# wildsonbbl/gnnepcsaft

Hardware: AMD Instinct MI355X
Metric: molecular graphs/sec (fwd+bwd) (higher is better)
Workload: dtype f32; 1 GPU; BASELINE configs[1]: PNA hidden=128 L=6 towers=1 pre=2 post=4, 4096 graphs/GPU (81920 atoms, 163840 directed bonds), fwd+loss+bwd incl. CSR packing; graphs_per_gpu=4096, parallelism=dp1, hip_graph=False, launch=auto, grad_allreduce_bytes=0, grad_exchange=none (1 rank)

## Files before the change

gnnepcsaft_amd/_lib.py:

```python
from __future__ import annotations

import ctypes as C
from pathlib import Path
from typing import Dict, Optional

import torch

_LIB_PATH = Path(__file__).resolve().parent / "libgnnepcsaft_hip.so"

ABI_VERSION = 7
GNX_OK, GNX_E_INVALID, GNX_E_HIP, GNX_E_RANGE, GNX_E_WORKSPACE = 0, -1, -2, -3, -4
OPT_GEMM_SPLIT, OPT_WGRAD_WGS, OPT_EMBED_BWD_MFMA, OPT_STD_BWD_CENTERED, OPT_GEMM_PIPE, OPT_WGRAD_PIPE, OPT_GEMM_AS, \
    OPT_GEMM_WS_FAST, OPT_GEMM_TILE_ROWS, OPT_GEMM_MID = range(10)
GEMM_RELU, GEMM_ACCUMULATE, GEMM_B_TRANS, GEMM_SPLIT_ONLY, GEMM_PRESPLIT = 1, 2, 4, 8, 16
GEMM_KERNEL_NAMES = ("none", "k_gemm<vec>", "k_gemm<generic>", "k_gemm_ws", "k_gemm_ws3", "k_gemm_ws3<fast,8>",
                     "k_gemm_ws3<fast,4>", "k_gemm3", "k_gemm3p<96>", "k_gemm3p<128>", "k_gemm_as3", "k_gemm_mid",
                     "k_gemm_small_batched")
WGRAD_KERNEL_NAMES = ("none", "k_gemm_wgrad<true,true>", "k_gemm_wgrad<false,true>", "k_gemm_wgrad3<true>",
                      "k_gemm_wgrad3p_grouped")
POOL_ADD, POOL_MEAN, POOL_MAX = 0, 1, 2
K_NONE, K_PNA_AGG_FWD, K_PNA_AGG_BWD, K_GEMM_WS, K_GEMM_WGRAD, K_GINE_AGG_FWD, K_GINE_AGG_BWD, K_EDGE_COMBINE_FWD, \
    K_EDGE_COMBINE_BWD, K_BN_FWD, K_BN_BWD, K_GEMM_TILED, K_GEMM_SMALL, K_GEMM_WGRAD_BATCHED, K_KEY_SEGMENT_SUM, \
    K_EMBED, K_PNA_EDGE_FWD, K_PNA_EDGE_BWD, K_ATTN_FWD, K_ATTN_BWD, K_PCSAFT_RHO, K_PCSAFT_VP, \
    K_PCSAFT_MIX_STATE, K_PCSAFT_MIX_RHO, K_PCSAFT_MIX_LNPHI_STATE, K_PCSAFT_MIX_LNPHI = range(26)
K_COUNT = 26
KERNEL_GROUPS = {K_PNA_AGG_FWD: "pna_aggregate_fwd", K_PNA_AGG_BWD: "pna_aggregate_bwd", K_GEMM_WS: "gemm_weights_stationary",
                 K_GEMM_WGRAD: "weight_gradient", K_GINE_AGG_FWD: "gine_aggregate_fwd", K_GINE_AGG_BWD: "gine_aggregate_bwd",
                 K_EDGE_COMBINE_FWD: "edge_combine_fwd", K_EDGE_COMBINE_BWD: "edge_combine_bwd", K_BN_FWD: "batchnorm_fwd",
                 K_BN_BWD: "batchnorm_bwd", K_GEMM_TILED: "gemm_tiled", K_GEMM_SMALL: "gemm_small",
                 K_GEMM_WGRAD_BATCHED: "weight_gradient_batched", K_KEY_SEGMENT_SUM: "key_segment_sum", K_EMBED: "embedding",
                 K_PNA_EDGE_FWD: "pna_edge_fused_fwd", K_PNA_EDGE_BWD: "pna_edge_fused_bwd",
                 K_ATTN_FWD: "transformer_attn_fwd", K_ATTN_BWD: "transformer_attn_bwd",
                 K_PCSAFT_RHO: "pcsaft_density", K_PCSAFT_VP: "pcsaft_vapor_pressure",
                 K_PCSAFT_MIX_STATE: "pcsaft_mix_state", K_PCSAFT_MIX_RHO: "pcsaft_mix_density",
                 K_PCSAFT_MIX_LNPHI_STATE: "pcsaft_mix_lnphi_state", K_PCSAFT_MIX_LNPHI: "pcsaft_mix_lnphi"}


class GnxError(RuntimeError):
    def __init__(self, status: int, msg: str):
        super().__init__(f"gnx status {status}: {msg}")
        self.status = status


class GemmSeg(C.Structure):
    _fields_ = [("a", C.c_void_p), ("lda", C.c_int64), ("rowscale", C.c_void_p), ("b", C.c_void_p),
                ("ldb", C.c_int64), ("k", C.c_int32), ("_pad", C.c_int32)]


class GemmPlanInfo(C.Structure):
    _fields_ = [("kernel", C.c_int32), ("tile_rows", C.c_int32), ("grid_x", C.c_uint32), ("grid_y", C.c_uint32),
                ("block", C.c_uint32), ("runs_split", C.c_int32), ("image_bytes", C.c_size_t)]


class WgradGroupedPlanInfo(C.Structure):
    _fields_ = [("kernel", C.c_int32), ("ranges", C.c_int32), ("chunks_per_range", C.c_int32), ("grid_x", C.c_uint32),
                ("grid_y", C.c_uint32), ("grid_z", C.c_uint32), ("block", C.c_uint32)]


class WgradProb(C.Structure):
    _fields_ = [("dC", C.c_void_p), ("lddc", C.c_int64), ("A", C.c_void_p), ("lda", C.c_int64),
                ("rowscale", C.c_void_p), ("dW", C.c_void_p), ("lddw", C.c_int64), ("dbias", C.c_void_p),
                ("M", C.c_int64), ("N", C.c_int32), ("K", C.c_int32)]


_vp, _i32, _i64, _f32, _sz = C.c_void_p, C.c_int32, C.c_int64, C.c_float, C.c_size_t

PNA_MAX_LAYERS, PNA_MAX_TOWERS = 8, 8
PNA_BWD_DEFER_SMALL, PNA_BWD_LAST_OF_PASS = 1, 2


class PnaFwdArgs(C.Structure):
    _fields_ = [("N", _i64), ("E", _i64), ("T", _i32), ("F", _i32), ("pre_layers", _i32), ("post_layers", _i32),
                ("D", _i32), ("merged", _i32),
                ("rowptr", _vp), ("src", _vp), ("dst", _vp), ("code", _vp), ("dperm", _vp), ("tiles", _vp), ("ntiles", _vp),
                ("max_tiles", _i64), ("x", _vp), ("Te", _vp), ("weff", _vp * PNA_MAX_TOWERS), ("Wm", _vp), ("bm", _vp),
                ("params", C.POINTER(_vp)), ("P", _vp), ("Q", _vp), ("A", _vp), ("hs", _vp * PNA_MAX_LAYERS),
                ("zs", _vp * PNA_MAX_LAYERS), ("ws", _vp), ("ws_bytes", _sz), ("out", _vp), ("etile_info", _vp),
                ("etile_w", _i32), ("tile_rows", _i32)]


class PnaBwdArgs(C.Structure):
    _fields_ = [("N", _i64), ("E", _i64), ("T", _i32), ("F", _i32), ("pre_layers", _i32), ("post_layers", _i32),
                ("R", _i32), ("D", _i32), ("avg_deg_log", _f32), ("merged", _i32), ("acc_first", _i32),
                ("use_side_streams", _i32), ("n_h", _i32), ("n_z", _i32),
                ("rowptr", _vp), ("colptr", _vp), ("cpos", _vp), ("code", _vp), ("code_pos", _vp), ("dperm", _vp),
                ("tiles", _vp), ("ntiles", _vp), ("chunks", _vp), ("nchunks", _vp),
                ("max_tiles", _i64), ("max_chunks", _i64),
                ("x", _vp), ("BE", _vp), ("EE", _vp), ("A", _vp),
                ("hs", _vp * PNA_MAX_LAYERS), ("zs", _vp * PNA_MAX_LAYERS), ("weff", _vp * PNA_MAX_TOWERS), ("Wm", _vp),
                ("params", C.POINTER(_vp)), ("grads", C.POINTER(_vp)), ("dout", _vp),
                ("gbuf", _vp * PNA_MAX_LAYERS), ("dA", _vp), ("gebuf", _vp * PNA_MAX_LAYERS), ("dP", _vp), ("dQ", _vp),
                ("dTe", _vp), ("dEE", _vp), ("dWm", _vp), ("dbm", _vp), ("dWeff", _vp), ("ws", _vp), ("ws_bytes", _sz),
                ("acc_buf", _vp), ("dx", _vp), ("flags", _i32), ("etile_w", _i32), ("etile_info", _vp)]


PACK_MAX_AVG = 4
PACK_CLASSES, PACK_CODE_INDEX, PACK_EDGE_TILES, PACK_TILED_SCAN = 1, 2, 4, 256


class PackBatchArgs(C.Structure):
    _fields_ = [("edge_index", _vp), ("edge_attr", _vp), ("batch", _vp), ("N", _i64), ("E", _i64), ("B", _i64),
                ("K", _i32), ("bond_dims", _i32 * 16), ("max_degree", _i32), ("R", _i32), ("n_avg", _i32),
                ("avg_deg_log", _f32 * PACK_MAX_AVG), ("tile_rows", _i32 * 3), ("edge_tile_w", _i32),
                ("parts", C.c_uint32), ("_pad", _i32),
                ("rowptr", _vp), ("perm", _vp), ("src", _vp), ("dst", _vp), ("colptr", _vp), ("cpos", _vp),
                ("code", _vp), ("graph_ptr", _vp), ("amp", _vp * PACK_MAX_AVG), ("att", _vp * PACK_MAX_AVG),
                ("dperm", _vp), ("cls_ptr", _vp), ("tiles", _vp * 3), ("ntiles", _vp * 3), ("code_pos", _vp),
                ("code_ptr", _vp), ("edge_tiles", _vp), ("ws", _vp), ("ws_bytes", _sz)]


class GemmImage(C.Structure):
    _fields_ = [("image_bytes", C.c_uint64), ("classes", _i32), ("Npad", _i32), ("Kpad", _i32), ("koff", _i32 * 5),
                ("frag", _i32), ("bt", _i32)]


class PnaLayerImages(C.Structure):
    _fields_ = [("post0", _vp * PNA_MAX_TOWERS), ("dA", _vp * PNA_MAX_TOWERS), ("dx", _vp * PNA_MAX_TOWERS),
                ("post0_rec", GemmImage * PNA_MAX_TOWERS), ("dA_rec", GemmImage * PNA_MAX_TOWERS),
                ("dx_rec", GemmImage * PNA_MAX_TOWERS)]


class PnaFinishArgs(C.Structure):
    _fields_ = [("L", _i32), ("T", _i32), ("F", _i32), ("pre_layers", _i32), ("post_layers", _i32), ("R", _i32), ("D", _i32),
                ("merged", _i32), ("use_side_streams", _i32), ("_pad", _i32),
                ("BE", _vp), ("acc_buf", _vp), ("ones", _vp), ("avg_deg_log", C.POINTER(_f32)),
                ("params", C.POINTER(_vp)), ("grads", C.POINTER(_vp)), ("EE", C.POINTER(_vp)), ("dTe", C.POINTER(_vp)),
                ("dEE", C.POINTER(_vp)), ("dWm", C.POINTER(_vp)), ("dbm", C.POINTER(_vp)), ("dWeff", C.POINTER(_vp))]


class SmallProb(C.Structure):
    _fields_ = [("A", _vp), ("lda", _i64), ("B", _vp), ("ldb", _i64), ("bias", _vp), ("C", _vp), ("ldc", _i64),
                ("M", _i32), ("N", _i32), ("K", _i32), ("flags", _i32)]


SB_A_TRANS, SB_B_TRANS, SB_ACCUMULATE, SB_ATOMIC, SB_RELU = 1, 2, 4, 8, 16

SIGNATURES = {
    "gnx_create": (_i32, [C.POINTER(_vp), _i32]),
    "gnx_destroy": (_i32, [_vp]),
    "gnx_set_stream": (_i32, [_vp, _vp]),
    "gnx_last_error": (C.c_char_p, []),
    "gnx_abi_version": (_i32, []),
    "gnx_set_option": (_i32, [_vp, _i32, _i32]),
    "gnx_get_option": (_i32, [_vp, _i32, C.POINTER(_i32)]),
    "gnx_prof_begin": (_i32, [_vp, C.c_uint32]),
    "gnx_prof_read": (_i32, [_vp, _i32, C.POINTER(_i64), C.POINTER(C.c_double), C.POINTER(C.c_double),
                             C.POINTER(C.c_double), C.POINTER(C.c_double)]),
    "gnx_prof_end": (_i32, [_vp]),
    "gnx_pack_csr_workspace_bytes": (_sz, [_i64, _i64]),
    "gnx_pack_csr": (_i32, [_vp, _vp, _i64, _i64, _vp, _vp, _vp, _vp, _vp, _vp, _vp, _sz]),
    "gnx_feature_code": (_i32, [_vp, _vp, _i64, _i32, C.POINTER(_i32), _vp, _vp, _vp, _sz]),
    "gnx_graph_ptr": (_i32, [_vp, _vp, _i64, _i64, _vp, _vp, _sz]),
    "gnx_degree_scalers": (_i32, [_vp, _vp, _i64, _f32, _vp, _vp]),
    "gnx_embed_sum_fwd": (_i32, [_vp, _vp, _i64, _i32, C.POINTER(_i32), _vp, _i32, _vp]),
    "gnx_table_scatter_workspace_bytes": (_sz, [_i64, _i32, _i32]),
    "gnx_embed_sum_bwd": (_i32, [_vp, _vp, _i64, _i32, C.POINTER(_i32), _i32, _vp, _i32, _vp, _vp, _sz]),
    "gnx_check_range": (_i32, [_vp]),
    "gnx_collate_ptr": (_i32, [_vp, _vp, _vp, _i64, _vp, _i64, _vp, _vp]),
    "gnx_collate_gather": (_i32, [_vp, _vp, _vp, _i64, _vp, _vp, _vp, _i64, _vp, _i64, _vp, _vp, _i64, _i64, _vp, _vp,
                                  _vp, _vp]),
    "gnx_collate_rows": (_i32, [_vp, _vp, _i64, _vp, _i64, _i32, _i32, _vp]),
    "gnx_gemm_workspace_bytes": (_sz, [_vp, _i32, C.POINTER(GemmSeg), C.POINTER(_i64), _i32, _i64, _i32, _vp, _i32,
                                       _i32]),
    "gnx_gemm": (_i32, [_vp, _i32, C.POINTER(GemmSeg), _i64, _i32, _vp, _vp, _i64, _vp, _i64, _i32, _vp, _sz]),
    "gnx_gemm_wgrad": (_i32, [_vp, _vp, _i64, _vp, _i64, _vp, _i64, _i32, _i32, _vp, _i64, _vp]),
    "gnx_gemm_wgrad_batched": (_i32, [_vp, _i32, C.POINTER(WgradProb)]),
    "gnx_degree_max": (_i32, [_vp, _vp, _i64, C.POINTER(_i32)]),
    "gnx_degree_classes_workspace_bytes": (_sz, [_i64, _i32]),
    "gnx_degree_classes": (_i32, [_vp, _vp, _i64, _i32, _vp, _vp, _vp, _sz]),
    "gnx_class_tiles": (_i32, [_vp, _vp, _i32, _i32, _vp, _vp]),
    "gnx_gemm_grouped": (_i32, [_vp, _i32, C.POINTER(GemmSeg), C.POINTER(_i64), _i32, _i64, _i32, _vp, _vp, _i64, _vp,
                                _i64, _i32, _vp, _vp, _vp, _i64, _vp, _sz]),
    "gnx_gemm_tile_rows": (_i32, [_vp, _i64, _i32]),
    "gnx_gemm_grouped_rows": (_i32, [_vp, _i32, C.POINTER(GemmSeg), C.POINTER(_i64), _i32, _i64, _i32, _vp, _vp, _i64, _vp,
                                     _i64, _i32, _vp, _vp, _vp, _i64, _vp, _sz, _i32]),
    "gnx_gemm_plan": (_i32, [_vp, _i32, C.POINTER(GemmSeg), C.POINTER(_i64), _i32, _i64, _i32, _vp, _vp, _i64, _vp, _i64, _i32,
                             _vp, _vp, _vp, _i64, _vp, _sz, _i32, C.POINTER(GemmPlanInfo)]),
    "gnx_gemm_wgrad_grouped": (_i32, [_vp, _vp, _i64, _vp, _i64, _i64, _i32, _i32, _vp, _i64, _i64, _vp, _vp, _vp,
                                      _i64]),
    "gnx_gemm_wgrad_grouped_plan": (_i32, [_vp, _i64, _i64, _vp, _vp, _i64, _i32, _i32, _i64,
                                           C.POINTER(WgradGroupedPlanInfo)]),
    "gnx_pna_weff": (_i32, [_vp, _vp, _i64, _i32, _i32, _f32, _vp]),
    "gnx_pna_weff_bwd": (_i32, [_vp, _vp, _i32, _i32, _f32, _vp, _i64]),
    "gnx_group_by_small_key": (_i32, [_vp, _vp, _i64, _i32, _vp, _vp, _vp, _sz]),
    "gnx_key_segment_sum": (_i32, [_vp, _vp, _vp, _vp, _i64, _i32, _vp]),
    "gnx_edge_combine_fwd": (_i32, [_vp, _vp, _vp, _vp, _vp, _vp, _vp, _i64, _i32, _i32, _vp]),
    "gnx_edge_combine_bwd": (_i32, [_vp, _vp, _vp, _vp, _vp, _vp, _i64, _i64, _i32, _i32, _vp, _vp, _vp, _vp, _sz]),
    "gnx_pna_aggregate_fwd": (_i32, [_vp, _vp, _vp, _i64, _i64, _i32, _i32, _vp]),
    "gnx_pna_aggregate_bwd": (_i32, [_vp, _vp, _vp, _vp, _vp, _i64, _i64, _i32, _i32, _vp]),
    "gnx_edge_tiles_count": (_i32, [_i64, _i32]),
    "gnx_edge_tiles": (_i32, [_vp, _vp, _i64, _i64, _i32, _vp]),
    "gnx_pack_batch_workspace_bytes": (_sz, [_i64, _i64, _i32, _i32]),
    "gnx_pack_batch": (_i32, [_vp, C.POINTER(PackBatchArgs)]),
    "gnx_pack_batch_scan_chunk": (_i64, []),
    "gnx_pack_batch_scan_bound": (_i64, []),
    "gnx_pna_edge_fwd": (_i32, [_vp, _vp, _vp, _vp, _vp, _vp, _vp, _vp, _vp, _i32, _i64, _i64, _i32, _i32, C.POINTER(_vp),
                                C.POINTER(_vp), _vp, _vp, _vp]),
    "gnx_pna_edge_bwd": (_i32, [_vp, _vp, _vp, _vp, _vp, _vp, _i32, _i64, _i64, _i32, _i32, _i32, C.POINTER(_vp), _vp, _vp,
                                _vp]),
    "gnx_gine_aggregate_fwd": (_i32, [_vp, _vp, _vp, _vp, _vp, _vp, _i64, _i64, _i32, _f32, _vp]),
    "gnx_gine_aggregate_bwd": (_i32, [_vp, _vp, _vp, _vp, _vp, _vp, _vp, _vp, _vp, _vp, _i64, _i64, _i32, _i32, _f32,
                                      _vp, _vp]),
    "gnx_gine_dle": (_i32, [_vp, _vp, _vp, _vp, _vp, _vp, _vp, _vp, _i64, _i32, _i32, _vp]),
    "gnx_transformer_attn_fwd": (_i32, [_vp, _vp, _vp, _vp, _vp, _vp, _i64, _i64, _i32, _i32, _f32, C.c_uint64,
                                        C.c_uint64, _vp, _vp, _vp]),
    "gnx_transformer_attn_bwd": (_i32, [_vp, _vp, _vp, _vp, _vp, _vp, _vp, _vp, _vp, _vp, _vp, _vp, _i64, _i64, _i32,
                                        _i32, _i32, _f32, C.c_uint64, C.c_uint64, _vp, _vp, _vp]),
    "gnx_transformer_attn_dle": (_i32, [_vp, _vp, _vp, _vp, _vp, _vp, _vp, _i64, _i32, _i32, _i32, _vp]),
    "gnx_pcsaft_density": (_i32, [_vp, _vp, _i64, _vp, _vp, _vp, _i64, _vp, _vp]),
    "gnx_pcsaft_vapor_pressure": (_i32, [_vp, _vp, _i64, _vp, _vp, _i64, _vp, _vp, _vp, _vp]),
    "gnx_pcsaft_mix_state": (_i32, [_vp, _vp, _i64, _vp, _vp, _vp, _i64, _i32, _vp, _vp, _vp, _vp, _i64, _vp, _vp, _vp,
                                    _vp]),
    "gnx_pcsaft_mix_density": (_i32, [_vp, _vp, _i64, _vp, _vp, _vp, _i64, _i32, _vp, _vp, _vp, _vp, _i64, _vp, _vp]),
    "gnx_pcsaft_mix_lnphi_state": (_i32, [_vp, _vp, _i64, _vp, _vp, _vp, _i64, _i32, _vp, _vp, _vp, _vp, _i64, _vp, _vp,
                                          _vp]),
    "gnx_pcsaft_mix_lnphi": (_i32, [_vp, _vp, _i64, _vp, _vp, _vp, _i64, _i32, _vp, _vp, _vp, _vp, _i64, _vp, _vp, _vp,
                                    _vp]),
    "gnx_pcsaft_mix_bubble": (_i32, [_vp, _vp, _i64, _vp, _vp, _vp, _i64, _i32, _vp, _vp, _vp, _i64, _vp, _vp, _vp, _vp,
                                     _vp]),
    "gnx_pcsaft_mix_dew": (_i32, [_vp, _vp, _i64, _vp, _vp, _vp, _i64, _i32, _vp, _vp, _vp, _i64, _vp, _vp, _vp, _vp,
                                  _vp]),
    "gnx_pcsaft_mix_bubble_t": (_i32, [_vp, _vp, _i64, _vp, _vp, _vp, _i64, _i32, _vp, _vp, _vp, _vp, _i64, _vp, _vp, _vp,
                                       _vp, _vp]),
    "gnx_pcsaft_mix_dew_t": (_i32, [_vp, _vp, _i64, _vp, _vp, _vp, _i64, _i32, _vp, _vp, _vp, _vp, _i64, _vp, _vp, _vp,
                                    _vp, _vp]),
    "gnx_pcsaft_mix_flash": (_i32, [_vp, _vp, _i64, _vp, _vp, _vp, _i64, _i32, _vp, _vp, _vp, _vp, _i64, _vp, _vp, _vp, _vp,
                                    _vp, _vp]),
    "gnx_pcsaft_mix_stability": (_i32, [_vp, _vp, _i64, _vp, _vp, _vp, _i64, _i32, _vp, _vp, _vp, _vp, _vp, _i64, _vp, _vp,
                                        _vp, _vp, _vp]),
    "gnx_pcsaft_mix_lle": (_i32, [_vp, _vp, _i64, _vp, _vp, _vp, _i64, _i32, _vp, _vp, _vp, _vp, _vp, _i64, _vp, _vp, _vp,
                                  _vp, _vp, _vp]),
    "gnx_segment_pool_fwd": (_i32, [_vp, _vp, _vp, _i64, _i32, _i32, _vp]),
    "gnx_segment_pool_bwd": (_i32, [_vp, _vp, _vp, _vp, _vp, _i64, _i32, _i32, _vp]),
    "gnx_batchnorm_workspace_bytes": (_sz, [_i64, _i32]),
    "gnx_batchnorm_fwd": (_i32, [_vp, _vp, _i64, _i32, _vp, _vp, _vp, _vp, _vp, _f32, _f32, _i32, _i32, _vp, _vp, _vp,
                                 _vp, _sz]),
    "gnx_batchnorm_bwd": (_i32, [_vp, _vp, _vp, _vp, _i64, _i32, _vp, _vp, _vp, _i32, _vp, _vp, _vp, _vp, _sz]),
    "gnx_batchnorm_bwd_x": (_i32, [_vp, _vp, _vp, _i64, _i32, _vp, _vp, _vp, _vp, _i32, _vp, _vp, _vp, _vp, _sz]),
    "gnx_dropout": (_i32, [_vp, _vp, _i64, _f32, C.c_uint64, C.c_uint64, _vp]),
    "gnx_huber_ape": (_i32, [_vp, _vp, _vp, _i64, _f32, _vp, _vp]),
    "gnx_adamw_amsgrad": (_i32, [_vp, _vp, _vp, _vp, _vp, _vp, _i64, _f32, _f32, _f32, _f32, _f32, _i64]),
    "gnx_sgd": (_i32, [_vp, _vp, _vp, _i64, _f32]),
    "gnx_pna_weight_only": (_i32, [_vp, _vp, _i32, _i32, _i32, _i32, _i32, _i32, _f32, C.POINTER(_vp), _i32, _vp, _vp,
                                   C.POINTER(_vp), _vp, _vp]),
    "gnx_pna_conv_fwd": (_i32, [_vp, C.POINTER(PnaFwdArgs)]),
    "gnx_pna_split_all_bytes": (_sz, [_vp, _i32, _i32, _i32, _i32, _i32, _i32, _i64, _i32]),
    "gnx_pna_split_all": (_i32, [_vp, _i32, _i32, _i32, _i32, _i32, _i32, _i64, _i32, C.POINTER(_vp), C.POINTER(_vp), _vp, _sz,
                                 C.POINTER(PnaLayerImages)]),
    "gnx_gemm_split_counts": (_i32, [_vp, C.POINTER(_i64), C.POINTER(_i64)]),
    "gnx_pna_conv_fwd_images": (_i32, [_vp, C.POINTER(PnaFwdArgs), C.POINTER(PnaLayerImages)]),
    "gnx_pna_conv_bwd_images": (_i32, [_vp, C.POINTER(PnaBwdArgs), C.POINTER(PnaLayerImages)]),
    "gnx_pna_weight_only_all": (_i32, [_vp, _i32, _vp, _i32, _i32, _i32, _i32, _i32, _i32, C.POINTER(_f32), C.POINTER(_vp),
                                       _i32, C.POINTER(_vp), C.POINTER(_vp), C.POINTER(_vp), C.POINTER(_vp), C.POINTER(_vp)]),
    "gnx_pna_stack_finish": (_i32, [_vp, C.POINTER(PnaFinishArgs)]),
    "gnx_gemm_small_batched": (_i32, [_vp, _i32, C.POINTER(SmallProb)]),
    "gnx_pna_weff_batched": (_i32, [_vp, _i32, C.POINTER(_vp), _i64, _i32, _i32, C.POINTER(_f32), C.POINTER(_vp)]),
    "gnx_pna_weff_bwd_batched": (_i32, [_vp, _i32, C.POINTER(_vp), _i32, _i32, C.POINTER(_f32), C.POINTER(_vp), _i64]),
    "gnx_pna_conv_bwd_workspace_bytes": (_sz, [_i32, _i32, _i32]),
    "gnx_pna_conv_bwd": (_i32, [_vp, C.POINTER(PnaBwdArgs)]),
    "gnx_fill": (_i32, [_vp, _vp, _i64, _f32]),
    "gnx_scale": (_i32, [_vp, _vp, _i64, _f32]),
    "gnx_axpy": (_i32, [_vp, _vp, _vp, _i64, _f32]),
    "gnx_side_stream": (_i32, [_vp, C.POINTER(_vp)]),
    "gnx_side_begin": (_i32, [_vp]),
    "gnx_side_end": (_i32, [_vp]),
    "gnx_side_join": (_i32, [_vp]),
    "gnx_side_stream_n": (_i32, [_vp, _i32, C.POINTER(_vp)]),
    "gnx_side_begin_n": (_i32, [_vp, _i32]),
    "gnx_side_join_n": (_i32, [_vp, _i32]),
    "gnx_clip_rows": (_i32, [_vp, _vp, _i64, _i32, _vp, _vp, _vp]),
}

_lib: Optional[C.CDLL] = None
_handles: Dict[int, int] = {}


def lib_path() -> Path:
    return _LIB_PATH


def load() -> C.CDLL:
    global _lib
    if _lib is not None:
        return _lib
    if not _LIB_PATH.exists():
        raise ImportError(f"{_LIB_PATH} is missing: build it with `python -m gnnepcsaft_amd.build` "
                          "(hipcc --offload-arch=gfx950). There is no CPU fallback.")
    lib = C.CDLL(str(_LIB_PATH))
    for name, (res, args) in SIGNATURES.items():
        fn = getattr(lib, name)
        fn.restype = res
        fn.argtypes = args
    if lib.gnx_abi_version() != ABI_VERSION:
        raise ImportError(f"ABI version mismatch: library {lib.gnx_abi_version()} != binding {ABI_VERSION}")
    _lib = lib
    return lib


def last_error() -> str:
    return load().gnx_last_error().decode(errors="replace")


def check(status: int) -> None:
    if status != GNX_OK:
        raise GnxError(status, last_error())


_bound_stream: dict = {}
try:
    _raw_stream = torch._C._cuda_getCurrentRawStream
except AttributeError:
    def _raw_stream(idx: int) -> int:
        return torch.cuda.current_stream(idx).cuda_stream


def handle(device: torch.device) -> int:
    if device.type != "cuda":
        raise GnxError(GNX_E_INVALID, f"gnnepcsaft_amd kernels need a HIP device tensor, got {device}; there is no CPU "
                                      "fallback")
    idx = device.index if device.index is not None else torch.cuda.current_device()
    lib = load()
    h = _handles.get(idx)
    if h is None:
        out = _vp()
        check(lib.gnx_create(C.byref(out), idx))
        h = out.value
        _handles[idx] = h
    stream = _raw_stream(idx)
    if _bound_stream.get(idx) != stream:
        check(lib.gnx_set_stream(h, stream))
        _bound_stream[idx] = stream
    return h
```

gnnepcsaft_amd/csrc/gnx_aggregate.hip:

```cpp
#include "gnx_common.hpp"

#include <cmath>
#include <cstdlib>

int32_t gnx_code_scatter_add(gnx_handle* h, const int32_t* code, int64_t E, int R, const float* g, int H,
                             float* dtable, void* ws, size_t ws_bytes);

template <int VEC>
struct vec_t;
template <>
struct vec_t<4> {
  typedef f32x4 type;
};
template <>
struct vec_t<1> {
  typedef float type;
};

template <int VEC>
__device__ __forceinline__ void vload(float (&r)[VEC], const float* p) {
  if constexpr (VEC == 4) {
    f32x4 v = *reinterpret_cast<const f32x4*>(p);
    r[0] = v.x;
    r[1] = v.y;
    r[2] = v.z;
    r[3] = v.w;
  } else {
    r[0] = p[0];
  }
}
template <int VEC>
__device__ __forceinline__ void vstore(float* p, const float (&r)[VEC]) {
  if constexpr (VEC == 4) {
    f32x4 v = {r[0], r[1], r[2], r[3]};
    *reinterpret_cast<f32x4*>(p) = v;
  } else {
    p[0] = r[0];
  }
}

__device__ __forceinline__ float relu_keep_nan(float r) { return (r < 0.f) ? 0.f : r; }
__device__ __forceinline__ float max_keep_nan(float s, float a) { return (a > s || a != a) ? a : s; }

#define STD_VAR_MIN 1e-5f
#define STD_MASK_AT 0.0031622776601683794f

template <int VEC>
__global__ void __launch_bounds__(256) k_pna_agg_fwd(const float* __restrict__ m, const int* __restrict__ rowptr,
                                                     int64_t N, int T, int F, float* __restrict__ A) {
  const int H = T * F;
  const int G = H / VEC;
  int64_t t = (int64_t)blockIdx.x * blockDim.x + threadIdx.x;
  if (t >= N * G) return;
  int64_t n = t / G;
  int c = (int)(t % G) * VEC;
  int p0 = rowptr[n], p1 = rowptr[n + 1];
  float s[VEC], s2[VEC], mn[VEC], mx[VEC];
#pragma unroll
  for (int v = 0; v < VEC; ++v) {
    s[v] = 0.f;
    s2[v] = 0.f;
    mn[v] = INFINITY;
    mx[v] = -INFINITY;
  }
  const float* mp = m + (int64_t)p0 * H + c;
  int p = p0;
  for (; p + 1 < p1; p += 2, mp += 2 * (int64_t)H) {
    float a[VEC], b[VEC];
    vload<VEC>(a, mp);
    vload<VEC>(b, mp + H);
#pragma unroll
    for (int v = 0; v < VEC; ++v) {
      s[v] = __fadd_rn(__fadd_rn(s[v], a[v]), b[v]);
      s2[v] = __fadd_rn(__fadd_rn(s2[v], __fmul_rn(a[v], a[v])), __fmul_rn(b[v], b[v]));
      mn[v] = fminf(mn[v], fminf(a[v], b[v]));
      mx[v] = fmaxf(mx[v], fmaxf(a[v], b[v]));
    }
  }
  if (p < p1) {
    float a[VEC];
    vload<VEC>(a, mp);
#pragma unroll
    for (int v = 0; v < VEC; ++v) {
      s[v] = __fadd_rn(s[v], a[v]);
      s2[v] = __fadd_rn(s2[v], __fmul_rn(a[v], a[v]));
      mn[v] = fminf(mn[v], a[v]);
      mx[v] = fmaxf(mx[v], a[v]);
    }
  }
  const int d = p1 - p0;
  const float cnt = (float)(d > 0 ? d : 1);
  float mean[VEC], sd[VEC];
#pragma unroll
  for (int v = 0; v < VEC; ++v) {
    mean[v] = __fdiv_rn(s[v], cnt);
    float mean2 = __fdiv_rn(s2[v], cnt);
    float var = __fsub_rn(mean2, __fmul_rn(mean[v], mean[v]));
    float o = __fsqrt_rn(fmaxf(var, STD_VAR_MIN));
    sd[v] = (o <= STD_MASK_AT) ? 0.f : o;
    if (d == 0) {
      mn[v] = 0.f;
      mx[v] = 0.f;
    }
  }
  int tw = c / F, f = c % F;
  float* o = A + (n * T + tw) * (int64_t)(4 * F) + f;
  vstore<VEC>(o, mean);
  vstore<VEC>(o + F, mn);
  vstore<VEC>(o + 2 * F, mx);
  vstore<VEC>(o + 3 * F, sd);
}

extern "C" int32_t gnx_pna_aggregate_fwd(gnx_handle* h, const float* m, const int32_t* rowptr, int64_t N, int64_t E,
                                         int32_t T, int32_t F, float* A) {
  GNX_CHECK_ARG(h && rowptr && T > 0 && F > 0 && N >= 0 && E >= 0, "gnx_pna_aggregate_fwd: bad argument");
  GNX_CHECK_ARG(N == 0 || A, "gnx_pna_aggregate_fwd: A is NULL");
  if (N == 0) return GNX_OK;
  gnx_prof_scope prof(h, GNX_K_PNA_AGG_FWD, 4.0 * E * T * F + 4.0 * E + 16.0 * N * T * F, 0.0, 0.0, true);
  if (F % 4 == 0) {
    int64_t th = N * (T * F / 4);
    GNX_LAUNCH_TIMED(prof, k_pna_agg_fwd<4>, dim3((unsigned)gnx_cdiv(th, 256)), dim3(256), 0, h->stream, m, rowptr, N,
                     (int)T, (int)F, A);
  } else {
    int64_t th = N * (T * F);
    GNX_LAUNCH_TIMED(prof, k_pna_agg_fwd<1>, dim3((unsigned)gnx_cdiv(th, 256)), dim3(256), 0, h->stream, m, rowptr, N,
                     (int)T, (int)F, A);
  }
  GNX_LAUNCH_CHECK();
  return GNX_OK;
}

template <int VEC>
__global__ void __launch_bounds__(256) k_pna_agg_bwd_rc(const float* __restrict__ dA, const float* __restrict__ m,
                                                        const int* __restrict__ rowptr, int64_t N, int T, int F,
                                                        float* __restrict__ dm, int centered) {
  const int H = T * F;
  const int G = H / VEC;
  int64_t t = (int64_t)blockIdx.x * blockDim.x + threadIdx.x;
  if (t >= N * G) return;
  int64_t n = t / G;
  int c = (int)(t % G) * VEC;
  int p0 = rowptr[n], p1 = rowptr[n + 1];
  if (p1 <= p0) return;
  int tw = c / F, f = c % F;
  int64_t ao = (n * T + tw) * (int64_t)(4 * F) + f;
  float gmean[VEC], gmn[VEC], gmx[VEC], gsd[VEC];
  vload<VEC>(gmean, dA + ao);
  vload<VEC>(gmn, dA + ao + F);
  vload<VEC>(gmx, dA + ao + 2 * F);
  vload<VEC>(gsd, dA + ao + 3 * F);
  float s[VEC], s2[VEC], mn[VEC], mx[VEC];
#pragma unroll
  for (int v = 0; v < VEC; ++v) {
    s[v] = 0.f;
    s2[v] = 0.f;
    mn[v] = INFINITY;
    mx[v] = -INFINITY;
  }
  if (p1 - p0 <= 4) {
    const int deg = p1 - p0;
    float a[4][VEC];
#pragma unroll
    for (int e = 0; e < 4; ++e) vload<VEC>(a[e], m + (int64_t)(p0 + (e < deg ? e : 0)) * H + c);
#pragma unroll
    for (int e = 0; e < 4; ++e)
      if (e < deg) {
#pragma unroll
        for (int v = 0; v < VEC; ++v) {
          s[v] = __fadd_rn(s[v], a[e][v]);
          s2[v] = __fadd_rn(s2[v], __fmul_rn(a[e][v], a[e][v]));
          mn[v] = fminf(mn[v], a[e][v]);
          mx[v] = fmaxf(mx[v], a[e][v]);
        }
      }
    const float cnt = (float)deg;
    float mean[VEC], sd[VEC], nmn[VEC], nmx[VEC], c2[VEC];
#pragma unroll
    for (int v = 0; v < VEC; ++v) {
      c2[v] = 0.f;
      mean[v] = __fdiv_rn(s[v], cnt);
      float mean2 = __fdiv_rn(s2[v], cnt);
      float var = __fsub_rn(mean2, __fmul_rn(mean[v], mean[v]));
      float o = __fsqrt_rn(fmaxf(var, STD_VAR_MIN));
      sd[v] = (o <= STD_MASK_AT) ? 0.f : o;
      nmn[v] = (mn[v] == 0.f) ? 1.f : 0.f;
      nmx[v] = (mx[v] == 0.f) ? 1.f : 0.f;
    }
#pragma unroll
    for (int e = 0; e < 4; ++e)
      if (e < deg) {
#pragma unroll
        for (int v = 0; v < VEC; ++v) {
          nmn[v] += (a[e][v] == mn[v]) ? 1.f : 0.f;
          nmx[v] += (a[e][v] == mx[v]) ? 1.f : 0.f;
          const float dv = a[e][v] - mean[v];
          c2[v] = fmaf(dv, dv, c2[v]);
        }
      }
    float k_mean[VEC], k_mn[VEC], k_mx[VEC], k_sd[VEC];
#pragma unroll
    for (int v = 0; v < VEC; ++v) {
      k_mean[v] = gmean[v] / cnt;
      k_mn[v] = gmn[v] / nmn[v];
      k_mx[v] = gmx[v] / nmx[v];
      const float sdiv = (centered && c2[v] > 0.f) ? sqrtf(c2[v] / cnt) : sd[v];
      k_sd[v] = (sd[v] > 0.f) ? gsd[v] / (cnt * sdiv) : 0.f;
    }
    float* dp = dm + (int64_t)p0 * H + c;
#pragma unroll
    for (int e = 0; e < 4; ++e)
      if (e < deg) {
        float o[VEC];
#pragma unroll
        for (int v = 0; v < VEC; ++v) {
          float r = k_mean[v] + k_sd[v] * (a[e][v] - mean[v]);
          r += (a[e][v] == mn[v]) ? k_mn[v] : 0.f;
          r += (a[e][v] == mx[v]) ? k_mx[v] : 0.f;
          o[v] = r;
        }
        vstore<VEC>(dp + (int64_t)e * H, o);
      }
    return;
  }
  const float* mp = m + (int64_t)p0 * H + c;
  for (int p = p0; p < p1; ++p, mp += H) {
    float a[VEC];
    vload<VEC>(a, mp);
#pragma unroll
    for (int v = 0; v < VEC; ++v) {
      s[v] = __fadd_rn(s[v], a[v]);
      s2[v] = __fadd_rn(s2[v], __fmul_rn(a[v], a[v]));
      mn[v] = fminf(mn[v], a[v]);
      mx[v] = fmaxf(mx[v], a[v]);
    }
  }
  const float cnt = (float)(p1 - p0);
  float mean[VEC], sd[VEC], nmn[VEC], nmx[VEC], c2[VEC];
#pragma unroll
  for (int v = 0; v < VEC; ++v) {
    c2[v] = 0.f;
    mean[v] = __fdiv_rn(s[v], cnt);
    float mean2 = __fdiv_rn(s2[v], cnt);
    float var = __fsub_rn(mean2, __fmul_rn(mean[v], mean[v]));
    float o = __fsqrt_rn(fmaxf(var, STD_VAR_MIN));
    sd[v] = (o <= STD_MASK_AT) ? 0.f : o;
    nmn[v] = (mn[v] == 0.f) ? 1.f : 0.f;
    nmx[v] = (mx[v] == 0.f) ? 1.f : 0.f;
  }
  mp = m + (int64_t)p0 * H + c;
  for (int p = p0; p < p1; ++p, mp += H) {
    float a[VEC];
    vload<VEC>(a, mp);
#pragma unroll
    for (int v = 0; v < VEC; ++v) {
      nmn[v] += (a[v] == mn[v]) ? 1.f : 0.f;
      nmx[v] += (a[v] == mx[v]) ? 1.f : 0.f;
      const float dv = a[v] - mean[v];
      c2[v] = fmaf(dv, dv, c2[v]);
    }
  }
  float k_mean[VEC], k_mn[VEC], k_mx[VEC], k_sd[VEC];
#pragma unroll
  for (int v = 0; v < VEC; ++v) {
    k_mean[v] = gmean[v] / cnt;
    k_mn[v] = gmn[v] / nmn[v];
    k_mx[v] = gmx[v] / nmx[v];
    const float sdiv = (centered && c2[v] > 0.f) ? sqrtf(c2[v] / cnt) : sd[v];
    k_sd[v] = (sd[v] > 0.f) ? gsd[v] / (cnt * sdiv) : 0.f;
  }
  mp = m + (int64_t)p0 * H + c;
  float* dp = dm + (int64_t)p0 * H + c;
  for (int p = p0; p < p1; ++p, mp += H, dp += H) {
    float a[VEC], o[VEC];
    vload<VEC>(a, mp);
#pragma unroll
    for (int v = 0; v < VEC; ++v) {
      float r = k_mean[v] + k_sd[v] * (a[v] - mean[v]);
      r += (a[v] == mn[v]) ? k_mn[v] : 0.f;
      r += (a[v] == mx[v]) ? k_mx[v] : 0.f;
      o[v] = r;
    }
    vstore<VEC>(dp, o);
  }
}

extern "C" int32_t gnx_pna_aggregate_bwd(gnx_handle* h, const float* dA, const float* m, const float* A,
                                         const int32_t* rowptr, int64_t N, int64_t E, int32_t T, int32_t F, float* dm) {
  GNX_CHECK_ARG(h && rowptr && T > 0 && F > 0 && N >= 0 && E >= 0, "gnx_pna_aggregate_bwd: bad argument");
  GNX_CHECK_ARG(N == 0 || (dA && A), "gnx_pna_aggregate_bwd: NULL argument");
  if (N == 0) return GNX_OK;
  gnx_prof_scope prof(h, GNX_K_PNA_AGG_BWD, 16.0 * N * T * F + 8.0 * E * T * F + 4.0 * E, 0.0, 0.0, true);
  if (F % 4 == 0)
    GNX_LAUNCH_TIMED(prof, k_pna_agg_bwd_rc<4>, dim3((unsigned)gnx_cdiv(N * (T * F / 4), 256)), dim3(256), 0, h->stream, dA, m,
                     rowptr, N, (int)T, (int)F, dm, h->opt[GNX_OPT_STD_BWD_CENTERED]);
  else
    GNX_LAUNCH_TIMED(prof, k_pna_agg_bwd_rc<1>, dim3((unsigned)gnx_cdiv(N * (int64_t)(T * F), 256)), dim3(256), 0, h->stream, dA,
                     m, rowptr, N, (int)T, (int)F, dm, h->opt[GNX_OPT_STD_BWD_CENTERED]);
  GNX_LAUNCH_CHECK();
  return GNX_OK;
}

template <int VEC>
__global__ void __launch_bounds__(256) k_edge_combine_fwd(const float* __restrict__ P, const float* __restrict__ Q,
                                                          const float* __restrict__ Te, const int* __restrict__ src,
                                                          const int* __restrict__ dst, const int* __restrict__ code,
                                                          int64_t E, int H, int relu, float* __restrict__ h1) {
  const int G = H / VEC;
  int64_t t = (int64_t)blockIdx.x * blockDim.x + threadIdx.x;
  if (t >= E * G) return;
  int64_t p = t / G;
  int c = (int)(t % G) * VEC;
  float a[VEC], b[VEC], e[VEC], o[VEC];
  vload<VEC>(a, P + (int64_t)dst[p] * H + c);
  vload<VEC>(b, Q + (int64_t)src[p] * H + c);
  vload<VEC>(e, Te + (int64_t)code[p] * H + c);
#pragma unroll
  for (int v = 0; v < VEC; ++v) {
    float r = (a[v] + b[v]) + e[v];
    o[v] = relu ? relu_keep_nan(r) : r;
  }
  vstore<VEC>(h1 + p * H + c, o);
}

extern "C" int32_t gnx_edge_combine_fwd(gnx_handle* h, const float* P, const float* Q, const float* Te,
                                        const int32_t* src, const int32_t* dst, const int32_t* code, int64_t E,
                                        int32_t H, int32_t relu, float* h1) {
  GNX_CHECK_ARG(h && H > 0 && E >= 0, "gnx_edge_combine_fwd: bad argument");
  if (E == 0) return GNX_OK;
  GNX_CHECK_ARG(P && Q && Te && src && dst && code && h1, "gnx_edge_combine_fwd: NULL argument");
  gnx_prof_scope prof(h, GNX_K_EDGE_COMBINE_FWD, 12.0 * E * H + 12.0 * E);
  if (H % 4 == 0)
    hipLaunchKernelGGL(k_edge_combine_fwd<4>, dim3((unsigned)gnx_cdiv(E * (H / 4), 256)), dim3(256), 0, h->stream, P, Q,
                       Te, src, dst, code, E, (int)H, (int)relu, h1);
  else
    hipLaunchKernelGGL(k_edge_combine_fwd<1>, dim3((unsigned)gnx_cdiv(E * H, 256)), dim3(256), 0, h->stream, P, Q, Te,
                       src, dst, code, E, (int)H, (int)relu, h1);
  GNX_LAUNCH_CHECK();
  return GNX_OK;
}

template <int VEC>
__global__ void __launch_bounds__(256) k_edge_combine_bwd(const float* __restrict__ g, const int* __restrict__ rowptr,
                                                          const int* __restrict__ colptr, const int* __restrict__ cpos,
                                                          int64_t N, int H, float* __restrict__ dP,
                                                          float* __restrict__ dQ) {
  const int G = H / VEC;
  int64_t t = (int64_t)blockIdx.x * blockDim.x + threadIdx.x;
  if (t >= N * G) return;
  int64_t n = t / G;
  int c = (int)(t % G) * VEC;
  float s[VEC], q[VEC];
#pragma unroll
  for (int v = 0; v < VEC; ++v) {
    s[v] = 0.f;
    q[v] = 0.f;
  }
  if (dP != nullptr) {
    int p0 = rowptr[n], p1 = rowptr[n + 1];
    for (int p = p0; p < p1; ++p) {
      float a[VEC];
      vload<VEC>(a, g + (int64_t)p * H + c);
#pragma unroll
      for (int v = 0; v < VEC; ++v) s[v] += a[v];
    }
  }
  int c0 = colptr[n], c1 = colptr[n + 1];
  for (int k = c0; k < c1; ++k) {
    float a[VEC];
    vload<VEC>(a, g + (int64_t)cpos[k] * H + c);
#pragma unroll
    for (int v = 0; v < VEC; ++v) q[v] += a[v];
  }
  if (dP != nullptr) vstore<VEC>(dP + n * H + c, s);
  vstore<VEC>(dQ + n * H + c, q);
}

extern "C" int32_t gnx_edge_combine_bwd(gnx_handle* h, const float* g, const int32_t* rowptr, const int32_t* colptr,
                                        const int32_t* cpos, const int32_t* code, int64_t N, int64_t E, int32_t H,
                                        int32_t R, float* dP, float* dQ, float* dTe, void* ws, size_t ws_bytes) {
  GNX_CHECK_ARG(h && H > 0 && N >= 0 && E >= 0, "gnx_edge_combine_bwd: bad argument");
  if (N == 0) return GNX_OK;
  GNX_CHECK_ARG(rowptr && colptr && dQ && (E == 0 || (g && cpos)), "gnx_edge_combine_bwd: NULL argument");
  gnx_prof_scope prof(h, GNX_K_EDGE_COMBINE_BWD, 4.0 * E * H + (dP ? 8.0 : 4.0) * N * H + 4.0 * E + 8.0 * N);
  if (H % 4 == 0)
    hipLaunchKernelGGL(k_edge_combine_bwd<4>, dim3((unsigned)gnx_cdiv(N * (H / 4), 256)), dim3(256), 0, h->stream, g,
                       rowptr, colptr, cpos, N, (int)H, dP, dQ);
  else
    hipLaunchKernelGGL(k_edge_combine_bwd<1>, dim3((unsigned)gnx_cdiv(N * H, 256)), dim3(256), 0, h->stream, g, rowptr,
                       colptr, cpos, N, (int)H, dP, dQ);
  GNX_LAUNCH_CHECK();
  if (dTe != nullptr && E > 0) {
    GNX_CHECK_ARG(code && R > 0, "gnx_edge_combine_bwd: code/R missing for dTe");
    return gnx_code_scatter_add(h, code, E, R, g, H, dTe, ws, ws_bytes);
  }
  return GNX_OK;
}


#define SEG_CHUNK 128

template <int VEC>
__global__ void __launch_bounds__(256) k_key_segment_sum(const float* __restrict__ g, const int* __restrict__ pos,
                                                         const int* __restrict__ key, int64_t E, int H,
                                                         float* __restrict__ dtable) {
  const int G = H / VEC;
  const int lanes = 256 / G > 0 ? 256 / G : 1;
  const int cg = threadIdx.x % G, rl = threadIdx.x / G;
  if (rl >= lanes) return;
  const int c = cg * VEC;
  const int64_t i0 = (int64_t)blockIdx.x * SEG_CHUNK;
  int64_t i1 = i0 + SEG_CHUNK;
  if (i1 > E) i1 = E;
  const int64_t per = (i1 - i0 + lanes - 1) / lanes;
  int64_t a = i0 + (int64_t)rl * per, b = a + per;
  if (b > i1) b = i1;
  if (a >= b) return;
  float acc[VEC];
#pragma unroll
  for (int v = 0; v < VEC; ++v) acc[v] = 0.f;
  int cur = key[pos[a]];
  constexpr int UN = 4;
  for (int64_t i = a; i < b; i += UN) {
    int p[UN], k[UN];
    float r[UN][VEC];
#pragma unroll
    for (int j = 0; j < UN; ++j) p[j] = pos[(i + j < b) ? i + j : b - 1];
#pragma unroll
    for (int j = 0; j < UN; ++j) k[j] = key[p[j]];
#pragma unroll
    for (int j = 0; j < UN; ++j) vload<VEC>(r[j], g + (int64_t)p[j] * H + c);
#pragma unroll
    for (int j = 0; j < UN; ++j) {
      if (i + j < b) {
        if (k[j] != cur) {
#pragma unroll
          for (int v = 0; v < VEC; ++v) atomicAdd(&dtable[(int64_t)cur * H + c + v], acc[v]);
// ... 366 lines not shown
```

gnnepcsaft_amd/csrc/gnx_api.hip:

```cpp
#include "gnx_common.hpp"

#include <cstdlib>
#include <cstring>

static thread_local char g_err[512] = "";

void gnx_set_error(const char* fmt, ...) {
  va_list ap;
  va_start(ap, fmt);
  vsnprintf(g_err, sizeof(g_err), fmt, ap);
  va_end(ap);
}

extern "C" const char* gnx_last_error(void) { return g_err; }
extern "C" int32_t gnx_abi_version(void) { return GNX_ABI_VERSION; }

extern "C" int32_t gnx_create(gnx_handle** out, int32_t device) {
  GNX_CHECK_ARG(out != nullptr, "gnx_create: out is NULL");
  int count = 0;
  GNX_HIP(hipGetDeviceCount(&count));
  GNX_CHECK_ARG(device >= 0 && device < count, "gnx_create: device %d not in [0,%d)", device, count);
  GNX_HIP(hipSetDevice(device));
  gnx_handle* h = new gnx_handle();
  h->device = device;
  {
    hipDeviceProp_t prop;
    if (hipGetDeviceProperties(&prop, device) == hipSuccess) h->num_cus = prop.multiProcessorCount;
  }
  hipError_t e = hipMalloc(&h->d_flag, 256);
  if (e == hipSuccess) e = hipMalloc(&h->d_scratch, 4096);
  if (e == hipSuccess) e = hipMemset(h->d_flag, 0, 256);
  if (e == hipSuccess) e = hipMalloc(&h->d_zero, 256);
  if (e == hipSuccess) e = hipMemset(h->d_zero, 0, 256);
  if (e != hipSuccess) {
    gnx_set_error("gnx_create: %s", hipGetErrorString(e));
    delete h;
    return GNX_E_HIP;
  }
  static const struct {
    int id;
    const char* env;
    int def;
  } opts[] = {{GNX_OPT_GEMM_SPLIT, "GNX_GEMM_SPLIT", 1},         {GNX_OPT_WGRAD_WGS, "GNX_WGRAD_WGS", 0},
              {GNX_OPT_EMBED_BWD_MFMA, "GNX_EMBED_BWD_MFMA", 1}, {GNX_OPT_STD_BWD_CENTERED, "GNX_STD_BWD_CENTERED", 1},
              {GNX_OPT_GEMM_PIPE, "GNX_GEMM_PIPE", 1},           {GNX_OPT_WGRAD_PIPE, "GNX_WGRAD_PIPE", 1},
              {GNX_OPT_GEMM_AS, "GNX_GEMM_AS", 1},               {GNX_OPT_GEMM_WS_FAST, "GNX_GEMM_WS_FAST", 2},
              {GNX_OPT_GEMM_TILE_ROWS, "GNX_GEMM_TILE_ROWS", 0}, {GNX_OPT_GEMM_MID, "GNX_GEMM_MID", 1}};
  for (const auto& o : opts) {
    const char* e = getenv(o.env);
    h->opt[o.id] = e ? atoi(e) : o.def;
  }
  *out = h;
  return GNX_OK;
}

extern "C" int32_t gnx_set_option(gnx_handle* h, int32_t opt, int32_t value) {
  GNX_CHECK_ARG(h != nullptr && opt >= 0 && opt < GNX_OPT_COUNT, "gnx_set_option: bad handle or option %d", opt);
  h->opt[opt] = value;
  return GNX_OK;
}

extern "C" int32_t gnx_get_option(gnx_handle* h, int32_t opt, int32_t* value) {
  GNX_CHECK_ARG(h != nullptr && value != nullptr && opt >= 0 && opt < GNX_OPT_COUNT, "gnx_get_option: bad argument");
  *value = h->opt[opt];
  return GNX_OK;
}

extern "C" int32_t gnx_destroy(gnx_handle* h) {
  if (!h) return GNX_OK;
  for (hipEvent_t e : h->ev) (void)hipEventDestroy(e);
  (void)hipFree(h->d_flag);
  (void)hipFree(h->d_scratch);
  (void)hipFree(h->d_zero);
  for (int i = 0; i < gnx_handle::kSideStreams; ++i) {
    if (h->side_fork[i]) (void)hipEventDestroy(h->side_fork[i]);
    if (h->side_done[i]) (void)hipEventDestroy(h->side_done[i]);
    if (h->side[i]) (void)hipStreamDestroy(h->side[i]);
  }
  delete h;
  return GNX_OK;
}

extern "C" int32_t gnx_set_stream(gnx_handle* h, void* hip_stream) {
  GNX_CHECK_ARG(h != nullptr, "gnx_set_stream: handle is NULL");
  GNX_CHECK_ARG(!h->on_side, "gnx_set_stream: between gnx_side_begin and gnx_side_end");
  h->stream = reinterpret_cast<hipStream_t>(hip_stream);
  return GNX_OK;
}

static int32_t side_ensure(gnx_handle* h, int which) {
  GNX_CHECK_ARG(h != nullptr, "gnx_side_*: handle is NULL");
  GNX_CHECK_ARG(which >= 0 && which < gnx_handle::kSideStreams, "gnx_side_*: stream %d not in [0,%d)", which,
                gnx_handle::kSideStreams);
  if (h->side[which] == nullptr) {
    GNX_HIP(hipSetDevice(h->device));
    GNX_HIP(hipStreamCreateWithFlags(&h->side[which], hipStreamNonBlocking));
    GNX_HIP(hipEventCreateWithFlags(&h->side_fork[which], hipEventDisableTiming));
    GNX_HIP(hipEventCreateWithFlags(&h->side_done[which], hipEventDisableTiming));
  }
  return GNX_OK;
}

extern "C" int32_t gnx_side_begin_n(gnx_handle* h, int32_t which) {
  const int32_t st = side_ensure(h, which);
  if (st != GNX_OK) return st;
  GNX_CHECK_ARG(!h->on_side, "gnx_side_begin: already on a side stream");
  GNX_HIP(hipEventRecord(h->side_fork[which], h->stream));
  GNX_HIP(hipStreamWaitEvent(h->side[which], h->side_fork[which], 0));
  h->main_saved = h->stream;
  h->stream = h->side[which];
  h->on_side = true;
  return GNX_OK;
}

extern "C" int32_t gnx_side_begin(gnx_handle* h) { return gnx_side_begin_n(h, 0); }

extern "C" int32_t gnx_side_stream_n(gnx_handle* h, int32_t which, void** hip_stream) {
  GNX_CHECK_ARG(hip_stream != nullptr, "gnx_side_stream: NULL argument");
  const int32_t st = side_ensure(h, which);
  if (st != GNX_OK) return st;
  *hip_stream = reinterpret_cast<void*>(h->side[which]);
  return GNX_OK;
}

extern "C" int32_t gnx_side_stream(gnx_handle* h, void** hip_stream) { return gnx_side_stream_n(h, 0, hip_stream); }

extern "C" int32_t gnx_side_end(gnx_handle* h) {
  GNX_CHECK_ARG(h != nullptr, "gnx_side_end: handle is NULL");
  if (h->on_side) {
    h->stream = h->main_saved;
    h->on_side = false;
  }
  return GNX_OK;
}

extern "C" int32_t gnx_side_join_n(gnx_handle* h, int32_t which) {
  GNX_CHECK_ARG(h != nullptr, "gnx_side_join: handle is NULL");
  GNX_CHECK_ARG(which >= 0 && which < gnx_handle::kSideStreams, "gnx_side_join: bad stream %d", which);
  GNX_CHECK_ARG(!h->on_side, "gnx_side_join: between gnx_side_begin and gnx_side_end");
  if (h->side[which] == nullptr) return GNX_OK;
  GNX_HIP(hipEventRecord(h->side_done[which], h->side[which]));
  GNX_HIP(hipStreamWaitEvent(h->stream, h->side_done[which], 0));
  return GNX_OK;
}

extern "C" int32_t gnx_side_join(gnx_handle* h) { return gnx_side_join_n(h, 0); }

int32_t gnx_read_flag(gnx_handle* h, int* value) {
  int v = 0;
  GNX_HIP(hipMemcpyAsync(&v, h->d_flag, sizeof(int), hipMemcpyDeviceToHost, h->stream));
  GNX_HIP(hipStreamSynchronize(h->stream));
  if (v != 0) GNX_HIP(hipMemsetAsync(h->d_flag, 0, sizeof(int), h->stream));
  *value = v;
  return GNX_OK;
}

extern "C" int32_t gnx_check_range(gnx_handle* h) {
  GNX_CHECK_ARG(h != nullptr, "gnx_check_range: handle is NULL");
  int v = 0;
  int32_t st = gnx_read_flag(h, &v);
  if (st != GNX_OK) return st;
  if (v != 0) {
    gnx_set_error("integer input out of range:%s%s%s%s%s%s%s", (v & 32) ? " an in-degree (or bond code) exceeds the caller's hint;" : "",
                  (v & 1) ? " edge_index holds a node id outside [0,N);" : "",
                  (v & 2) ? " edge/node feature outside its vocabulary;" : "",
                  (v & 4) ? " batch holds a graph id outside [0,B);" : "", (v & 8) ? " batch is not sorted;" : "",
                  (v & 16) ? " embedding index outside its table;" : "",
                  (v & 128) ? " batch index outside the device dataset;" : "");
    return GNX_E_RANGE;
  }
  return GNX_OK;
}

extern "C" int32_t gnx_prof_begin(gnx_handle* h, uint32_t kernel_mask) {
  GNX_CHECK_ARG(h != nullptr, "gnx_prof_begin: handle is NULL");
  GNX_CHECK_ARG((kernel_mask >> GNX_K_COUNT) == 0, "gnx_prof_begin: bad kernel mask 0x%x", kernel_mask);
  h->prof_mask = kernel_mask & ~1u;
  h->ev_used = 0;
  return GNX_OK;
}

extern "C" int32_t gnx_prof_read(gnx_handle* h, int32_t kid, int64_t* launches, double* total_ms, double* alg_bytes,
                                 double* alg_flops, double* mfma_bf16_flops) {
  GNX_CHECK_ARG(h != nullptr && launches != nullptr && total_ms != nullptr, "gnx_prof_read: NULL argument");
  GNX_CHECK_ARG(kid > 0 && kid < GNX_K_COUNT, "gnx_prof_read: bad kernel id %d", kid);
  GNX_HIP(hipStreamSynchronize(h->stream));
  double tot = 0.0, w[3] = {0.0, 0.0, 0.0};
  int64_t n = 0;
  for (size_t i = 0; i + 1 < h->ev_used; i += 2) {
    if (h->ev_kid[i / 2] != kid) continue;
    float ms = 0.f;
    GNX_HIP(hipEventElapsedTime(&ms, h->ev[i], h->ev[i + 1]));
    tot += ms;
    for (int q = 0; q < 3; ++q) w[q] += h->ev_work[3 * (i / 2) + q];
    ++n;
  }
  *launches = n;
  *total_ms = tot;
  if (alg_bytes) *alg_bytes = w[0];
  if (alg_flops) *alg_flops = w[1];
// ... 106 lines not shown
```

gnnepcsaft_amd/csrc/gnx_gemm.hip:

```cpp
#include "gnx_gemm_plan.hpp"
#include "gnx_split.hpp"

#include <cstdlib>
#include <type_traits>

#define MAX_SEGS 4

enum { EPI_PLAIN = 0, EPI_ACCUM = 1, EPI_MASK = 2 };

template <typename F>
static auto epi_dispatch(bool bt, int epi, F&& f) {
  auto with_bt = [&](auto BT) {
    if (epi == EPI_MASK) return f(BT, std::integral_constant<int, EPI_MASK>{});
    if (epi == EPI_ACCUM) return f(BT, std::integral_constant<int, EPI_ACCUM>{});
    return f(BT, std::integral_constant<int, EPI_PLAIN>{});
  };
  return bt ? with_bt(std::true_type{}) : with_bt(std::false_type{});
}

struct seg_dev {
  const float* a;
  const float* rs;
  const float* b;
  int64_t lda;
  int64_t ldb;
  int64_t cls_stride;
  int k;
  int vec_a;
  int vec_b;
};

struct gemm_args {
  seg_dev seg[MAX_SEGS];
  int nseg;
  int64_t M;
  int N;
  const float* bias;
  const float* mask;
  int64_t ldmask;
  float* C;
  int64_t ldc;
  int relu;
  const int* row_index;
  const int* tile_info;
  const int* ntiles;
  int ny;
  const __bf16* bsplit;
  int Npad, Kpad;
  int koff[MAX_SEGS];
  int steps;
};

template <int EPI>
__device__ __forceinline__ void epilogue_tile(const f32x16& acc, const int (&rows)[16], int gc, int N, float bv,
                                              int relu, const float* __restrict__ mask, int64_t ldmask,
                                              float* __restrict__ C, int64_t ldc) {
  const bool col_ok = gc < N;
  const int gcc = col_ok ? gc : 0;
  float extra[16];
  if constexpr (EPI != EPI_PLAIN) {
#pragma unroll
    for (int r = 0; r < 16; ++r) {
      const int64_t gr = rows[r] < 0 ? 0 : rows[r];
      extra[r] = (EPI == EPI_MASK) ? mask[gr * ldmask + gcc] : C[gr * ldc + gcc];
    }
  }
#pragma unroll
  for (int r = 0; r < 16; ++r) {
    float v = acc[r] + bv;
    if constexpr (EPI == EPI_ACCUM) v += extra[r];
    v = relu ? fmaxf(v, 0.f) : v;
    if constexpr (EPI == EPI_MASK) v = (extra[r] > 0.f) ? v : 0.f;
    if (col_ok && rows[r] >= 0) C[(int64_t)rows[r] * ldc + gc] = v;
  }
}

template <bool B_TRANS, int EPI, bool VEC>
__global__ void __launch_bounds__(256, 2) k_gemm(gemm_args g) {
  __shared__ __attribute__((aligned(16))) float As[BM * LDK];
  __shared__ __attribute__((aligned(16))) float Bs[B_TRANS ? BN * LDK : BK * LDN];
  __shared__ int rid[BM];

  const int tid = threadIdx.x;
  const int lane = tid & 63;
  const int wave = tid >> 6;
  const int wm = wave >> 1, wn = wave & 1;
  const int li = lane & 31, lh = lane >> 5;
  const int n0 = blockIdx.y * BN;
  int cls = 0;
  if (g.tile_info != nullptr) {
    if ((int)blockIdx.x >= g.ntiles[0]) return;
    const int p0 = g.tile_info[3 * blockIdx.x], pr = g.tile_info[3 * blockIdx.x + 1];
    cls = g.tile_info[3 * blockIdx.x + 2];
    if (tid < BM) rid[tid] = (tid < pr) ? g.row_index[p0 + tid] : -1;
  } else {
    const int64_t m0 = (int64_t)blockIdx.x * BM;
    if (tid < BM) rid[tid] = (m0 + tid < g.M) ? (int)(m0 + tid) : -1;
  }
  __syncthreads();

  f32x16 acc[2][2];
#pragma unroll
  for (int i = 0; i < 2; ++i)
#pragma unroll
    for (int j = 0; j < 2; ++j)
#pragma unroll
      for (int r = 0; r < 16; ++r) acc[i][j][r] = 0.f;

  f32x4 ra[4], rb[4];

  const int lr = tid >> 3;
  const int lk = (tid & 7) * 4;
  const int br = tid >> 5;
  const int bc = (tid & 31) * 4;
  int grow[4];
#pragma unroll
  for (int i = 0; i < 4; ++i) grow[i] = rid[lr + 32 * i];
  int okmask = 0;
  float rsv[4] = {1.f, 1.f, 1.f, 1.f};

  auto load_tile = [&](const seg_dev& s, int k0) {
    const float* sb = s.b + (int64_t)cls * s.cls_stride;
    if constexpr (VEC) {
      const int kcol = k0 + lk;
      const bool k_ok = kcol < s.k;
      const int kc = k_ok ? kcol : 0;
      okmask = 0;
#pragma unroll
      for (int i = 0; i < 4; ++i) {
        const int64_t row = grow[i] >= 0 ? grow[i] : 0;
        ra[i] = *reinterpret_cast<const f32x4*>(s.a + row * s.lda + kc);
        rsv[i] = *(s.rs != nullptr ? s.rs + row : &c_one);
        okmask |= (k_ok && grow[i] >= 0) ? (1 << i) : 0;
      }
      if (B_TRANS) {
#pragma unroll
        for (int i = 0; i < 4; ++i) {
          const int gn = n0 + lr + 32 * i;
          rb[i] = *reinterpret_cast<const f32x4*>(sb + (int64_t)(gn < g.N ? gn : 0) * s.ldb + kc);
          okmask |= (k_ok && gn < g.N) ? (16 << i) : 0;
        }
      } else {
        const int nn = n0 + bc;
        const bool n_ok = nn < g.N;
        const int nc = n_ok ? nn : 0;
#pragma unroll
        for (int i = 0; i < 4; ++i) {
          const int kr = k0 + br + 8 * i;
          rb[i] = *reinterpret_cast<const f32x4*>(sb + (int64_t)(kr < s.k ? kr : 0) * s.ldb + nc);
          okmask |= (n_ok && kr < s.k) ? (16 << i) : 0;
        }
      }
      return;
// ... 1189 lines not shown
  const bool k_ok = k4 < s.k;
  int grow[8];
#pragma unroll
  for (int q = 0; q < 8; ++q) {
    const int r = lr + 8 * q;
    const int idx = p0 + (r < pr ? r : pr - 1);
    grow[q] = grouped ? g.row_index[idx] : idx;
  }
  int my_row = 0;
  if (tid < AS_BM) {
    const int idx = p0 + (tid < pr ? tid : pr - 1);
    my_row = grouped ? g.row_index[idx] : idx;
  }
  f32x4 ra[8];
#pragma unroll
  for (int q = 0; q < 8; ++q) ra[q] = *reinterpret_cast<const f32x4*>(s.a + (int64_t)grow[q] * s.lda + (k_ok ? k4 : 0));

  const int total_kt = NT * 4;
  const __bf16* const bbase = g.bsplit + ((int64_t)cls * NT * 4 * 3) * (BN * BK) + (wave * 64 + lane) * 8;
  bf16x8 bq[2][2][3];
  auto load_b = [&](int slot, int sl, int j) {
    const __bf16* p = bbase + (int64_t)(j < total_kt ? j : total_kt - 1) * (3 * BN * BK);
#pragma unroll
    for (int pc = 0; pc < 3; ++pc) bq[slot][sl][pc] = *reinterpret_cast<const bf16x8*>(p + ((sl * 3 + pc) * 4 * 64) * 8);
  };
  load_b(0, 0, 0);
  load_b(0, 1, 0);
  AS_AT(0);

  typedef __attribute__((ext_vector_type(2))) float f32x2;
  if (tid < AS_BM) {
    roff[tid] = (unsigned)my_row * (unsigned)g.ldc;
    moff[tid] = (unsigned)my_row * (unsigned)g.ldmask;
  }
#pragma unroll
  for (int q = 0; q < 8; q += 2) {
    float xa[8];
#pragma unroll
    for (int j = 0; j < 4; ++j) {
      xa[j] = k_ok ? ra[q][j] : 0.f;
      xa[4 + j] = k_ok ? ra[q + 1][j] : 0.f;
    }
    bf16x8 pc[3];
    split3(xa, pc[0], pc[1], pc[2]);
#pragma unroll
    for (int p = 0; p < 3; ++p) {
      const f32x4 w = *reinterpret_cast<const f32x4*>(&pc[p]);
      unsigned char* qa = A3 + p * AS_PIECE + (lr + 8 * q) * AS_LDA + k4 * 2;
      *reinterpret_cast<f32x2*>(qa) = f32x2{w.x, w.y};
      *reinterpret_cast<f32x2*>(qa + 8 * AS_LDA) = f32x2{w.z, w.w};
    }
  }
  load_b(1, 0, 1);
  load_b(1, 1, 1);
  AS_AT(1);
  __syncthreads();
  AS_AT(2);

  int afrag = li * AS_LDA + 16 * lh;
  bf16x8 af[2][2][3];
  auto read_a = [&](int slot, int off, int ks) {
    const unsigned char* base = A3 + off;
#pragma unroll
    for (int mi = 0; mi < 2; ++mi)
#pragma unroll
      for (int p = 0; p < 3; ++p)
        af[slot][mi][p] = *reinterpret_cast<const bf16x8*>(base + p * AS_PIECE + mi * 32 * AS_LDA + ks * 32);
  };
  read_a(0, afrag, 0);

  const int qj = li & 3;
  const unsigned lc = (unsigned)(wave * 32 + (li >> 2) * 4);
  unsigned ro[2][4], mo[2][4];
#pragma unroll
  for (int mi = 0; mi < 2; ++mi)
#pragma unroll
    for (int gq = 0; gq < 4; ++gq) {
      ro[mi][gq] = roff[mi * 32 + 8 * gq + 4 * lh + qj] + lc;
      mo[mi][gq] = moff[mi * 32 + 8 * gq + 4 * lh + qj] + lc;
    }
  const float* const bias_p = g.bias != nullptr ? g.bias : c_zero4;
  const int bias_on = g.bias != nullptr ? 1 : 0;
  auto bias_at = [&](int nt_) { return *reinterpret_cast<const f32x4*>(bias_p + (bias_on ? nt_ * BN + (int)lc : 0)); };
  f32x4 bv = bias_at(0);
  const float floor_v = g.relu ? 0.f : -__builtin_inff();
  asm volatile("" ::"v"(bv));
  auto quad_swap = [&](float& x, float& y, auto CTRL, bool hi) {
    const float send = hi ? x : y;
    const float got = __builtin_bit_cast(float, __builtin_amdgcn_mov_dpp(__builtin_bit_cast(int, send), decltype(CTRL)::value, 0xf, 0xf, true));
    x = hi ? got : x;
    y = hi ? y : got;
  };
  using XOR1 = std::integral_constant<int, 0xB1>;
  using XOR2 = std::integral_constant<int, 0x4E>;

  for (int nt = 0; nt < NT; ++nt) {
    asm volatile("" : "+v"(afrag));
    f32x16 acc[2];
#pragma unroll
    for (int mi = 0; mi < 2; ++mi)
#pragma unroll
      for (int r = 0; r < 16; ++r) acc[mi][r] = 0.f;
    const f32x4 bv_next = bias_at(nt + 1 < NT ? nt + 1 : nt);
#pragma unroll
    for (int ks = 0; ks < 8; ++ks) {
      const int kt = ks >> 1, sl = ks & 1;
      read_a((ks + 1) & 1, afrag, (ks + 1) & 7);
      __builtin_amdgcn_sched_barrier(0);
#pragma unroll
      for (int mi = 0; mi < 2; ++mi) mfma_3x3(acc[mi], af[ks & 1][mi], bq[kt & 1][sl]);
      load_b(kt & 1, sl, nt * 4 + kt + 2);
      __builtin_amdgcn_sched_barrier(0);
    }
    asm volatile("" ::"v"(bv_next));
    AS_AT(3);
    float* const cbase = g.C + nt * BN;
    const float* const mbase = (EPI == EPI_MASK ? g.mask : g.C) + nt * BN;
    f32x4 extra[2][4];
    if constexpr (EPI != EPI_PLAIN) {
#pragma unroll
      for (int mi = 0; mi < 2; ++mi)
#pragma unroll
        for (int gq = 0; gq < 4; ++gq)
          extra[mi][gq] = *reinterpret_cast<const f32x4*>(mbase + (EPI == EPI_MASK ? mo[mi][gq] : ro[mi][gq]));
    }
#pragma unroll
    for (int mi = 0; mi < 2; ++mi)
#pragma unroll
      for (int gq = 0; gq < 4; ++gq) {
        float c0 = acc[mi][4 * gq], c1 = acc[mi][4 * gq + 1], c2 = acc[mi][4 * gq + 2], c3 = acc[mi][4 * gq + 3];
        quad_swap(c0, c1, XOR1{}, (qj & 1) != 0);
        quad_swap(c2, c3, XOR1{}, (qj & 1) != 0);
        quad_swap(c0, c2, XOR2{}, (qj & 2) != 0);
        quad_swap(c1, c3, XOR2{}, (qj & 2) != 0);
        f32x4 v = {c0 + bv.x, c1 + bv.y, c2 + bv.z, c3 + bv.w};
        if constexpr (EPI == EPI_ACCUM) v += extra[mi][gq];
#pragma unroll
        for (int e = 0; e < 4; ++e) v[e] = fmaxf(v[e], floor_v);
        if constexpr (EPI == EPI_MASK)
#pragma unroll
          for (int e = 0; e < 4; ++e) v[e] = (extra[mi][gq][e] > 0.f) ? v[e] : 0.f;
        *reinterpret_cast<f32x4*>(cbase + ro[mi][gq]) = v;
      }
    bv = bv_next;
    AS_AT(4);
  }
#ifdef AS_STAMP
  if (tid == 0 && as_stamp_buf != nullptr) {
    for (int i = 0; i < 5; ++i) as_stamp_buf[(size_t)blockIdx.x * 8 + i] = tacc[i];
    as_stamp_buf[(size_t)blockIdx.x * 8 + 5] = tstart;
    as_stamp_buf[(size_t)blockIdx.x * 8 + 6] = clock64();
  }
#endif
}

#define MID_T 16
#define MID_KC 128
#define MID_LD (MID_KC + 4)

template <bool B_TRANS, int EPI>
__global__ void __launch_bounds__(256) k_gemm_mid(gemm_args g) {
  __shared__ __attribute__((aligned(16))) float As[MID_T][MID_LD];
  __shared__ __attribute__((aligned(16))) float Bs[MID_T][MID_LD];
  __shared__ int rid[MID_T];
  const int tid = threadIdx.x;
  const int tx = tid & 15, ty = tid >> 4;
  const int n0 = blockIdx.y * MID_T;
  int cls = 0;
  if (g.tile_info != nullptr) {
    const int t = blockIdx.x >> 3, sub = blockIdx.x & 7;
    if (t >= g.ntiles[0]) return;
    const int p0 = g.tile_info[3 * t] + MID_T * sub, pr = g.tile_info[3 * t + 1] - MID_T * sub;
    cls = g.tile_info[3 * t + 2];
    if (pr <= 0) return;
    if (tid < MID_T) rid[tid] = tid < pr ? g.row_index[p0 + tid] : -1;
  } else {
    const int64_t m0 = (int64_t)blockIdx.x * MID_T;
    if (tid < MID_T) rid[tid] = (m0 + tid < g.M) ? (int)(m0 + tid) : -1;
  }
  __syncthreads();

  f32x4 ra[2], rb[2];
  auto fetch = [&](int si, int k0) {
    const seg_dev& s = g.seg[si];
    const float* __restrict__ sb = s.b + (int64_t)cls * s.cls_stride;
    const bool va = s.vec_a && (s.k % 4 == 0), vb = s.vec_b && (B_TRANS ? (s.k % 4 == 0) : (g.N % 4 == 0));
    const int kc = (s.k - k0) < MID_KC ? (s.k - k0) : MID_KC;
#pragma unroll
    for (int j = 0; j < 2; ++j) {
      const int gi = tid + 256 * j, r = gi >> 5, k4 = (gi & 31) * 4;
      const int row = rid[r];
      f32x4 v = {0.f, 0.f, 0.f, 0.f};
      if (row >= 0 && k4 < kc) {
        const float* ap = s.a + (int64_t)row * s.lda + k0 + k4;
        if (va) {
          v = *reinterpret_cast<const f32x4*>(ap);
        } else {
#pragma unroll
          for (int e = 0; e < 4; ++e) v[e] = (k4 + e < kc) ? ap[e] : 0.f;
        }
        if (s.rs != nullptr) {
          const float rs = s.rs[row];
#pragma unroll
          for (int e = 0; e < 4; ++e) v[e] = rs * v[e];
        }
      }
      ra[j] = v;
    }
    if (B_TRANS) {
#pragma unroll
      for (int j = 0; j < 2; ++j) {
        const int gi = tid + 256 * j, r = gi >> 5, k4 = (gi & 31) * 4;
        f32x4 v = {0.f, 0.f, 0.f, 0.f};
        if (n0 + r < g.N && k4 < kc) {
          const float* bp = sb + (int64_t)(n0 + r) * s.ldb + k0 + k4;
          if (vb) {
            v = *reinterpret_cast<const f32x4*>(bp);
          } else {
#pragma unroll
            for (int e = 0; e < 4; ++e) v[e] = (k4 + e < kc) ? bp[e] : 0.f;
          }
        }
        rb[j] = v;
      }
    } else {
#pragma unroll
      for (int j = 0; j < 2; ++j) {
        const int gi = tid + 256 * j, k = gi >> 2, c4 = (gi & 3) * 4;
        f32x4 v = {0.f, 0.f, 0.f, 0.f};
        if (k < kc && n0 + c4 < g.N) {
          const float* bp = sb + (int64_t)(k0 + k) * s.ldb + n0 + c4;
          if (vb) {
            v = *reinterpret_cast<const f32x4*>(bp);
          } else {
#pragma unroll
            for (int e = 0; e < 4; ++e) v[e] = (n0 + c4 + e < g.N) ? bp[e] : 0.f;
          }
        }
        rb[j] = v;
      }
    }
  };
  auto stage = [&]() {
#pragma unroll
    for (int j = 0; j < 2; ++j) {
      const int gi = tid + 256 * j;
      *reinterpret_cast<f32x4*>(&As[gi >> 5][(gi & 31) * 4]) = ra[j];
      if (B_TRANS) {
        *reinterpret_cast<f32x4*>(&Bs[gi >> 5][(gi & 31) * 4]) = rb[j];
      } else {
        const int k = gi >> 2, c4 = (gi & 3) * 4;
#pragma unroll
        for (int e = 0; e < 4; ++e) Bs[c4 + e][k] = rb[j][e];
      }
    }
  };

  float acc = 0.f;
  int si = 0, k0 = 0;
  fetch(0, 0);
  while (true) {
    stage();
    __syncthreads();
    const int kc = (g.seg[si].k - k0) < MID_KC ? (g.seg[si].k - k0) : MID_KC;
    int sn = si, kn = k0 + MID_KC;
    if (kn >= g.seg[si].k) {
      ++sn;
      kn = 0;
    }
    const bool more = sn < g.nseg;
    if (more) fetch(sn, kn);
    const int kend = (kc + 3) & ~3;
    for (int k = 0; k < kend; k += 4) {
      const f32x4 a = *reinterpret_cast<const f32x4*>(&As[ty][k]);
      const f32x4 b = *reinterpret_cast<const f32x4*>(&Bs[tx][k]);
      acc = fmaf(a.x, b.x, acc);
      acc = fmaf(a.y, b.y, acc);
      acc = fmaf(a.z, b.z, acc);
      acc = fmaf(a.w, b.w, acc);
    }
    if (!more) break;
    __syncthreads();
    si = sn;
    k0 = kn;
  }
  const int gm = rid[ty], gn = n0 + tx;
  if (gm >= 0 && gn < g.N) {
    float v = acc + (g.bias != nullptr ? g.bias[gn] : 0.f);
    float* cp = g.C + (int64_t)gm * g.ldc + gn;
    if constexpr (EPI == EPI_ACCUM) v += *cp;
    v = g.relu ? fmaxf(v, 0.f) : v;
    if constexpr (EPI == EPI_MASK) v = (g.mask[(int64_t)gm * g.ldmask + gn] > 0.f) ? v : 0.f;
    *cp = v;
  }
}

#define SM_T 16
#define SM_KC 128

struct small_batch_args {
  gnx_small_prob p[GNX_SMALL_BATCH];
  int n;
};

__global__ void __launch_bounds__(256) k_gemm_small_batched(small_batch_args b) {
  __shared__ float As[SM_T][SM_KC + 1];
// ... 141 lines not shown

  gnx_prof_scope prof(h, p.prof_id, p.bytes, p.flops, p.mfma);
  if (p.run_split) {
    const dim3 gs((unsigned)gnx_cdiv((int64_t)sa.D * sa.Npad * (sa.Kpad / 8), 256));
    if (p.bt)
      hipLaunchKernelGGL(k_split_weights<true>, gs, dim3(256), 0, h->stream, sa);
    else
      hipLaunchKernelGGL(k_split_weights<false>, gs, dim3(256), 0, h->stream, sa);
    ++h->split_launches;
  }
  if (p.stop_after_split || p.kernel == GNX_GEMM_KERNEL_NONE) {
    GNX_LAUNCH_CHECK();
    return GNX_OK;
  }
  const dim3 grid(p.grid_x, p.grid_y), block(p.block);
#define GEMM_CASE(KIND, COND, KERNEL, ARGS, LDS_LIMIT)                                               \
  case KIND:                                                                                         \
    if constexpr (COND) {                                                                            \
      if constexpr ((LDS_LIMIT) > 0)                                                                 \
        if (const hipError_t e = gnx_raise_lds_limit<&KERNEL>(LDS_LIMIT); e != hipSuccess) return e; \
      hipLaunchKernelGGL((KERNEL), grid, block, p.lds, h->stream, ARGS);                             \
    }                                                                                                \
    return hipSuccess
  const hipError_t lds_limit = epi_dispatch(p.bt, p.epi, [&](auto BT, auto EPI) -> hipError_t {
    constexpr bool no_rmw = EPI != EPI_ACCUM;
    switch (p.kernel) {
      GEMM_CASE(GNX_GEMM_KERNEL_WS, true, (k_gemm_ws<BT, EPI>), w, 160 * 1024);
      GEMM_CASE(GNX_GEMM_KERNEL_WS3, true, (k_gemm_ws3<BT, EPI, false, 8>), w, 160 * 1024);
      GEMM_CASE(GNX_GEMM_KERNEL_WS3_FAST8, no_rmw, (k_gemm_ws3<BT, EPI, true, 8>), w, 160 * 1024);
      GEMM_CASE(GNX_GEMM_KERNEL_WS3_FAST4, no_rmw, (k_gemm_ws3<BT, EPI, true, 4>), w, 64 * 1024);
      GEMM_CASE(GNX_GEMM_KERNEL_MID, true, (k_gemm_mid<BT, EPI>), g, 0);
      GEMM_CASE(GNX_GEMM_KERNEL_AS3, true, (k_gemm_as3<EPI>), g, (int)AS_LDS);
      GEMM_CASE(GNX_GEMM_KERNEL_GEMM3P_96, true, (k_gemm3p<EPI, 3>), g, 0);
      GEMM_CASE(GNX_GEMM_KERNEL_GEMM3P_128, true, (k_gemm3p<EPI, 4>), g, 0);
      GEMM_CASE(GNX_GEMM_KERNEL_GEMM3, true, (k_gemm3<EPI>), g, 0);
      GEMM_CASE(GNX_GEMM_KERNEL_TILED_VEC, true, (k_gemm<BT, EPI, true>), g, 0);
      GEMM_CASE(GNX_GEMM_KERNEL_TILED_GENERIC, true, (k_gemm<BT, EPI, false>), g, 0);
      default: {
        small_batch_args b;
        for (int i = 0; i < GNX_SMALL_BATCH; ++i)
          b.p[i] = {w.A, w.lda, w.B, w.ldb, bias, C, ldc, (int32_t)M, N, w.K,
                    (p.bt ? GNX_SB_B_TRANS : 0) | (relu ? GNX_SB_RELU : 0) | ((flags & GNX_GEMM_ACCUMULATE) ? GNX_SB_ACCUMULATE : 0)};
        b.n = 1;
        hipLaunchKernelGGL(k_gemm_small_batched, grid, block, 0, h->stream, b);
        return hipSuccess;
      }
    }
  });
#undef GEMM_CASE
  GNX_HIP(lds_limit);
  GNX_LAUNCH_CHECK();
  return GNX_OK;
}

int32_t gnx_split_weights_batched(gnx_handle* h, int32_t n, const gemm_split_problem* probs) {
  GNX_CHECK_ARG(h && (n == 0 || probs) && n >= 0, "gnx_split_weights_batched: bad argument");
  double bytes = 0.0;
  for (int i = 0; i < n; ++i) {
    const gemm_split_problem& q = probs[i];
    GNX_CHECK_ARG(q.nseg >= 1 && q.nseg <= MAX_SEGS && q.N > 0 && q.classes >= 1 && q.out && aligned16(q.out),
                  "gnx_split_weights_batched: problem %d: bad shape or image address", i);
    for (int s = 0; s < q.nseg; ++s)
      GNX_CHECK_ARG(q.b[s] && q.k[s] > 0 && q.ldb[s] > 0 && q.ldb[s] <= INT32_MAX,
                    "gnx_split_weights_batched: problem %d, segment %d: NULL weights, k <= 0 or ldb out of range", i, s);
  }
  for (int i0 = 0; i0 < n; i0 += SPLIT_MAX_BATCH) {
    split_batch_args b = {};
    b.n = n - i0 < SPLIT_MAX_BATCH ? n - i0 : SPLIT_MAX_BATCH;
    int64_t widest = 0;
    for (int i = 0; i < b.n; ++i) {
      const gemm_split_problem& q = probs[i0 + i];
      split_batch_prob& d = b.p[i];
      int64_t kpad = 0;
      for (int s = 0; s < q.nseg; ++s) {
        d.seg[s] = split_batch_seg{q.b[s], q.cls_stride[s], (int32_t)q.ldb[s], q.k[s]};
        kpad += plan_kpad(q.k[s]);
      }
      d.out = reinterpret_cast<__bf16*>(q.out);
      d.N = q.N;
      d.D = q.classes;
      d.nseg = q.nseg;
      d.layout = (q.bt ? 1 : 0) | (q.frag ? 2 : 0);
      const int64_t items = (int64_t)q.classes * (gnx_cdiv(q.N, BN) * BN) * (kpad / 8);
      widest = items > widest ? items : widest;
      bytes += 6.0 * items * 8 + 4.0 * q.classes * q.N * kpad;
    }
    gnx_prof_scope prof(h, GNX_K_GEMM_TILED, bytes, 0.0, 0.0);
    hipLaunchKernelGGL(k_split_weights_batched, dim3((unsigned)gnx_cdiv(widest, 256), (unsigned)b.n), dim3(256), 0, h->stream, b);
    ++h->split_batched_launches;
    bytes = 0.0;
  }
  GNX_LAUNCH_CHECK();
  return GNX_OK;
}

extern "C" int32_t gnx_gemm(gnx_handle* h, int32_t nseg, const gnx_gemm_seg* segs, int64_t M, int32_t N,
                            const float* bias, const float* mask, int64_t ldmask, float* C, int64_t ldc, int32_t flags,
                            void* ws, size_t ws_bytes) {
  return gemm_launch(h, nseg, segs, nullptr, 1, M, N, bias, mask, ldmask, C, ldc, flags, nullptr, nullptr, nullptr, 0,
                     ws, ws_bytes);
}

extern "C" size_t gnx_gemm_workspace_bytes(gnx_handle* h, int32_t nseg, const gnx_gemm_seg* segs,
                                           const int64_t* cls_strides, int32_t num_classes, int64_t M, int32_t N,
                                           const float* mask, int32_t flags, int32_t grouped) {
  if (h == nullptr || segs == nullptr || nseg < 1 || nseg > MAX_SEGS || M < 0 || N <= 0) return 0;
  static const int32_t a_table = 0;
  return gemm_plan_of(nseg, segs, cls_strides, num_classes, M, N, nullptr, mask, N, nullptr, N, flags, grouped ? &a_table : nullptr,
                      1, nullptr, 0, h->opt, h->num_cus)
      .image_bytes;
}

extern "C" int32_t gnx_gemm_split_counts(gnx_handle* h, int64_t* per_call, int64_t* batched) {
  GNX_CHECK_ARG(h && per_call && batched, "gnx_gemm_split_counts: NULL argument");
  *per_call = h->split_launches;
  *batched = h->split_batched_launches;
  return GNX_OK;
}

extern "C" int32_t gnx_gemm_tile_rows(gnx_handle* h, int64_t M, int32_t N) {
  if (h == nullptr || M <= 0 || N <= 0) return 128;
  return gemm_plan_tile_rows(M, N, h->opt[GNX_OPT_GEMM_TILE_ROWS], h->num_cus > 0 ? h->num_cus : 256);
}

extern "C" int32_t gnx_gemm_plan(gnx_handle* h, int32_t nseg, const gnx_gemm_seg* segs, const int64_t* cls_strides,
                                 int32_t num_classes, int64_t M, int32_t N, const float* bias, const float* mask, int64_t ldmask,
                                 float* C, int64_t ldc, int32_t flags, const int32_t* row_index, const int32_t* tile_info,
                                 const int32_t* ntiles, int64_t max_tiles, void* ws, size_t ws_bytes, int32_t tile_rows,
                                 gnx_gemm_plan_info* out) {
  GNX_CHECK_ARG(out, "gnx_gemm_plan: NULL argument");
  const bool grouped = cls_strides || row_index || tile_info || ntiles;
  GNX_CHECK_ARG(!grouped || (cls_strides && row_index && tile_info && ntiles && max_tiles > 0 && num_classes >= 1 && num_classes <= 4096),
                "gnx_gemm_plan: grouped call with a NULL array, max_tiles <= 0 or num_classes not in [1,4096]");
  const int32_t st = gemm_check(h, nseg, segs, M, N, mask, ldmask, C, ldc, flags, tile_rows);
  if (st != GNX_OK) return st;
  (void)ws_bytes;
  const gemm_plan p = gemm_plan_of(nseg, segs, cls_strides, grouped ? num_classes : 1, M, N, bias, mask, ldmask, C, ldc, flags,
                                   tile_info, max_tiles, ws, tile_rows, h->opt, h->num_cus);
  *out = gnx_gemm_plan_info{p.kernel, p.tile_rows, p.grid_x, p.grid_y, p.block, p.run_split ? 1 : 0, p.image_bytes};
  return GNX_OK;
}

extern "C" int32_t gnx_gemm_grouped(gnx_handle* h, int32_t nseg, const gnx_gemm_seg* segs, const int64_t* cls_strides,
                                    int32_t num_classes, int64_t M, int32_t N, const float* bias, const float* mask,
                                    int64_t ldmask, float* C, int64_t ldc, int32_t flags, const int32_t* row_index,
                                    const int32_t* tile_info, const int32_t* ntiles, int64_t max_tiles, void* ws,
                                    size_t ws_bytes) {
  GNX_CHECK_ARG(cls_strides && row_index && tile_info && ntiles && max_tiles > 0, "gnx_gemm_grouped: NULL argument");
  GNX_CHECK_ARG(num_classes >= 1 && num_classes <= 4096, "gnx_gemm_grouped: num_classes=%d not in [1,4096]", num_classes);
  return gemm_launch(h, nseg, segs, cls_strides, num_classes, M, N, bias, mask, ldmask, C, ldc, flags, row_index,
                     tile_info, ntiles, max_tiles, ws, ws_bytes);
}

extern "C" int32_t gnx_gemm_grouped_rows(gnx_handle* h, int32_t nseg, const gnx_gemm_seg* segs, const int64_t* cls_strides,
                                         int32_t num_classes, int64_t M, int32_t N, const float* bias, const float* mask,
                                         int64_t ldmask, float* C, int64_t ldc, int32_t flags, const int32_t* row_index,
                                         const int32_t* tile_info, const int32_t* ntiles, int64_t max_tiles, void* ws,
                                         size_t ws_bytes, int32_t tile_rows) {
  GNX_CHECK_ARG(cls_strides && row_index && tile_info && ntiles && max_tiles > 0, "gnx_gemm_grouped_rows: NULL argument");
  GNX_CHECK_ARG(num_classes >= 1 && num_classes <= 4096, "gnx_gemm_grouped_rows: num_classes=%d not in [1,4096]", num_classes);
  GNX_CHECK_ARG(tile_rows == 96 || tile_rows == 128, "gnx_gemm_grouped_rows: tile_rows=%d not in {96, 128}", tile_rows);
  return gemm_launch(h, nseg, segs, cls_strides, num_classes, M, N, bias, mask, ldmask, C, ldc, flags, row_index,
                     tile_info, ntiles, max_tiles, ws, ws_bytes, tile_rows);
}
```

gnnepcsaft_amd/csrc/gnx_gemm_plan.hpp:

```cpp
#pragma once
#include <cstddef>
#include <cstdint>

#include "gnx.h"

constexpr int PLAN_MAX_SEGS = 4;
constexpr int PLAN_BM = 128, PLAN_BN = 128, PLAN_BK = 32;
constexpr int PLAN_WS_BM = 64;
constexpr size_t PLAN_WS_LDS = 4 * (128 * 132 + 2 * 64 * 132);
constexpr size_t PLAN_WS3_LDS8 = 2 * 3 * 64 * 272;
constexpr size_t PLAN_WS3_LDS4 = 64 * 1024;
constexpr int PLAN_G3P_MIN_KTILES = 8;
constexpr size_t plan_g3p_lds(int mi) { return (size_t)(2 * 3 * 32 * mi * 80 + 2 * 32 * mi * 4); }
constexpr int PLAN_AS_BM = 64;
constexpr size_t PLAN_AS_LDS = 3 * 64 * 272 + 2 * 64 * 4;
constexpr int PLAN_PATCH = 16;
constexpr int PLAN_WGS_PER_CU = 2;
constexpr int64_t PLAN_SPLIT_MIN_ROWS = 4096, PLAN_WS_MIN_ROWS = 8192;

enum { PLAN_EPI_PLAIN = 0, PLAN_EPI_ACCUM = 1, PLAN_EPI_MASK = 2 };

struct gemm_plan {
  int kernel = GNX_GEMM_KERNEL_NONE;
  bool bt = false;
// ... 154 lines not shown
  r.classes = p.classes;
  r.Npad = p.Npad;
  r.Kpad = p.Kpad;
  for (int s = 0; s <= PLAN_MAX_SEGS; ++s) r.koff[s] = p.koff[s];
  r.frag = p.frag;
  r.bt = p.bt ? 1 : 0;
  return r;
}
static inline bool gemm_image_equal(const gnx_gemm_image& a, const gnx_gemm_image& b) {
  bool eq = a.image_bytes == b.image_bytes && a.classes == b.classes && a.Npad == b.Npad && a.Kpad == b.Kpad && a.frag == b.frag &&
            a.bt == b.bt;
  for (int s = 0; s <= PLAN_MAX_SEGS; ++s) eq = eq && a.koff[s] == b.koff[s];
  return eq;
}

struct gemm_split_problem {
  const float* b[PLAN_MAX_SEGS];
  int64_t ldb[PLAN_MAX_SEGS], cls_stride[PLAN_MAX_SEGS];
  int32_t k[PLAN_MAX_SEGS];
  int32_t nseg, N, classes, frag, bt;
  void* out;
};
static inline gemm_split_problem gemm_split_problem_of(const gemm_plan& p, int32_t nseg, const gnx_gemm_seg* segs,
                                                       const int64_t* cls_strides, int32_t N, void* out) {
  gemm_split_problem q = {};
  for (int s = 0; s < nseg; ++s) {
    q.b[s] = segs[s].b;
    q.ldb[s] = segs[s].ldb;
    q.cls_stride[s] = cls_strides ? cls_strides[s] : 0;
    q.k[s] = segs[s].k;
  }
  q.nseg = nseg;
  q.N = N;
  q.classes = p.classes;
  q.frag = p.frag;
  q.bt = p.bt ? 1 : 0;
  q.out = out;
  return q;
}

struct pna_product {
  int32_t nseg = 0;
  gnx_gemm_seg seg[3] = {};
  int64_t stride[3] = {0, 0, 0};
  bool grouped = false;
  int32_t classes = 1, N = 0, flags = 0, tile_rows = 0;
  const float* bias = nullptr;
  float* C = nullptr;
  int64_t ldc = 0;
};

static inline gnx_gemm_seg pna_seg(const float* a, int64_t lda, const float* b, int64_t ldb, int32_t k) {
  gnx_gemm_seg s;
  s.a = a;
  s.lda = lda;
  s.rowscale = nullptr;
  s.b = b;
  s.ldb = ldb;
  s.k = k;
  s._pad = 0;
  return s;
}

static inline float* pna_stand_in() { return reinterpret_cast<float*>(static_cast<uintptr_t>(1) << 20); }

static inline pna_product pna_post0_product(const float* const* P, const float* weff_t, int T, int F, int pre, int post, int D,
                                            int t, const float* x, const float* A, float* z0, int tile_rows) {
  const int H = T * F, k = 4 + t * 2 * (pre + post) + 2 * pre;
  pna_product q;
  q.nseg = 2;
  q.seg[0] = pna_seg(x + t * F, H, P[k], 13 * F, F);
  q.seg[1] = pna_seg(A + (int64_t)t * 4 * F, (int64_t)T * 4 * F, weff_t, 4 * F, 4 * F);
  q.stride[1] = (int64_t)4 * F * F;
  q.grouped = true;
  q.classes = D;
  q.N = F;
  q.flags = GNX_GEMM_B_TRANS | (post > 1 ? GNX_GEMM_RELU : 0);
  q.tile_rows = tile_rows == 96 ? 96 : 128;
  q.bias = P[k + 1];
  q.C = z0 + t * F;
  q.ldc = H;
  return q;
}

static inline pna_product pna_dA_product(const float* weff_t, int T, int F, int D, int t, const float* g, float* dA) {
  pna_product q;
  q.nseg = 1;
  q.seg[0] = pna_seg(g + t * F, (int64_t)T * F, weff_t, 4 * F, F);
  q.stride[0] = (int64_t)4 * F * F;
  q.grouped = true;
  q.classes = D;
  q.N = 4 * F;
  q.C = dA + (int64_t)t * 4 * F;
  q.ldc = (int64_t)T * 4 * F;
  return q;
}

static inline pna_product pna_dx_product(const float* const* P, int T, int F, int pre, int post, int t, const float* g_post0,
                                         const float* dP, const float* dQ, float* dx) {
  const int H = T * F, k0 = 4 + t * 2 * (pre + post), kp = k0 + 2 * pre;
  pna_product q;
  q.nseg = 3;
  q.seg[0] = pna_seg(g_post0 + t * F, H, P[kp], 13 * F, F);
  q.seg[1] = pna_seg(dP + t * F, H, P[k0], 3 * F, F);
  q.seg[2] = pna_seg(dQ + t * F, H, P[k0] + F, 3 * F, F);
  q.N = F;
  q.C = dx + t * F;
  q.ldc = H;
  return q;
}

static inline gemm_plan pna_product_plan(const pna_product& q, int64_t M, int32_t extra_flags, const void* ws, int64_t max_tiles,
                                         const int* opt, int num_cus) {
  static const int32_t a_table = 0;
  return gemm_plan_of(q.nseg, q.seg, q.grouped ? q.stride : nullptr, q.grouped ? q.classes : 1, M, q.N, q.bias, nullptr, 0, q.C,
                      q.ldc, q.flags | extra_flags, q.grouped ? &a_table : nullptr, max_tiles, ws, q.grouped ? q.tile_rows : 0, opt,
                      num_cus);
}

static inline size_t pna_images_layout(int L, int T, int F, int pre, int post, int D, int64_t N, int tile_rows,
                                       const float* const* params, const float* const* weff, const int* opt, int num_cus,
                                       void* slab, gnx_pna_layer_images* out, gemm_split_problem* probs, int* nprobs) {
  const int np = 4 + T * 2 * (pre + post);
  const uintptr_t base = reinterpret_cast<uintptr_t>(slab);
  float* const act = pna_stand_in();
  size_t off = 0;
  int n = 0;
  for (int l = 0; l < L; ++l) {
    const float* const* P = params + (size_t)l * np;
    gnx_pna_layer_images li = {};
    for (int t = 0; t < T; ++t) {
      const float* w = weff[(size_t)l * T + t];
      const pna_product prod[3] = {pna_post0_product(P, w, T, F, pre, post, D, t, act, act, act, tile_rows),
                                   pna_dA_product(w, T, F, D, t, act, act), pna_dx_product(P, T, F, pre, post, t, act, act, act, act)};
      void** const ptr[3] = {&li.post0[t], &li.dA[t], &li.dx[t]};
      gnx_gemm_image* const rec[3] = {&li.post0_rec[t], &li.dA_rec[t], &li.dx_rec[t]};
      for (int i = 0; i < 3; ++i) {
        const pna_product& q = prod[i];
        const gemm_plan p = pna_product_plan(q, N, GNX_GEMM_SPLIT_ONLY, act, 1, opt, num_cus);
        if (!p.images || !p.run_split) continue;
        *rec[i] = gemm_image_of(p);
        void* const image = reinterpret_cast<void*>(base + off);
        *ptr[i] = image;
        if (probs) probs[n] = gemm_split_problem_of(p, q.nseg, q.seg, q.grouped ? q.stride : nullptr, q.N, image);
        ++n;
        off += p.image_bytes;
      }
    }
    if (out) out[l] = li;
  }
  if (nprobs) *nprobs = n;
  return off;
}
```

gnnepcsaft_amd/csrc/gnx_layer.hip:

```cpp
#include "gnx_common.hpp"
#include "gnx_gemm_plan.hpp"

#include <algorithm>
#include <vector>

namespace {

inline gnx_gemm_seg seg(const float* a, int64_t lda, const float* b, int64_t ldb, int32_t k) { return pna_seg(a, lda, b, ldb, k); }

inline bool a16(const void* p) { return (reinterpret_cast<uintptr_t>(p) & 15) == 0; }

struct WgradQueue {
  std::vector<gnx_wgrad_prob> q;
  void add(const float* dC, int64_t lddc, const float* A, int64_t lda, int64_t M, int32_t N, int32_t K, float* dW,
           int64_t lddw, float* dbias) {
    if (M <= 0) return;
    gnx_wgrad_prob p;
    p.dC = dC;
    p.lddc = lddc;
    p.A = A;
    p.lda = lda;
    p.rowscale = nullptr;
    p.dW = dW;
    p.lddw = lddw;
    p.dbias = dbias;
    p.M = M;
    p.N = N;
    p.K = K;
    q.push_back(p);
  }
  int32_t flush(gnx_handle* h) {
    std::stable_sort(q.begin(), q.end(), [](const gnx_wgrad_prob& a, const gnx_wgrad_prob& b) { return a.M > b.M; });
    for (size_t i = 0; i < q.size(); i += 8) {
      const int32_t n = (int32_t)std::min<size_t>(8, q.size() - i);
      const int32_t st = gnx_gemm_wgrad_batched(h, n, q.data() + i);
      if (st != GNX_OK) return st;
    }
    q.clear();
    return GNX_OK;
  }
};

#define GNX_TRY(call)                 \
  do {                                \
    const int32_t st_ = (call);       \
    if (st_ != GNX_OK) return st_;    \
  } while (0)

template <class F>
int32_t on_side(gnx_handle* h, int which, bool enabled, F body) {
  if (!enabled) return body();
  GNX_TRY(gnx_side_begin_n(h, which));
  const int32_t st = body();
  (void)gnx_side_end(h);
  return st;
}

struct class_tiles {
  const int32_t *dperm, *tiles, *ntiles;
  int64_t max_tiles;
};

int32_t run_product(gnx_handle* h, const pna_product& q, int64_t M, const class_tiles& ct, int32_t extra_flags, void* ws,
                    size_t ws_bytes) {
  if (!q.grouped) return gnx_gemm(h, q.nseg, q.seg, M, q.N, q.bias, nullptr, 0, q.C, q.ldc, q.flags | extra_flags, ws, ws_bytes);
  if (q.tile_rows)
    return gnx_gemm_grouped_rows(h, q.nseg, q.seg, q.stride, q.classes, M, q.N, q.bias, nullptr, 0, q.C, q.ldc, q.flags | extra_flags,
                                 ct.dperm, ct.tiles, ct.ntiles, ct.max_tiles, ws, ws_bytes, q.tile_rows);
  return gnx_gemm_grouped(h, q.nseg, q.seg, q.stride, q.classes, M, q.N, q.bias, nullptr, 0, q.C, q.ldc, q.flags | extra_flags, ct.dperm,
                          ct.tiles, ct.ntiles, ct.max_tiles, ws, ws_bytes);
}

int32_t run_with_image(gnx_handle* h, const pna_product& q, int64_t M, const class_tiles& ct, void* image,
                       const gnx_gemm_image* rec, void* scratch, size_t scratch_bytes) {
  if (image != nullptr && rec != nullptr && rec->image_bytes > 0) {
    const gemm_plan p = pna_product_plan(q, M, GNX_GEMM_PRESPLIT, image, ct.max_tiles, h->opt, h->num_cus);
    if (p.images && gemm_image_equal(gemm_image_of(p), *rec))
      return run_product(h, q, M, ct, GNX_GEMM_PRESPLIT, image, (size_t)rec->image_bytes);
  }
  return run_product(h, q, M, ct, 0, scratch, scratch_bytes);
}

}

static size_t align256(size_t v) { return (v + 255) / 256 * 256; }

extern "C" size_t gnx_pna_conv_bwd_workspace_bytes(int32_t T, int32_t F, int32_t D) {
  const int64_t H = (int64_t)T * F;
  const size_t grouped = gemm_plan_image_bytes(D, 4 * (int64_t)F, plan_kpad(F));
  const size_t dx = gemm_plan_image_bytes(1, F, 3 * plan_kpad(F));
  const size_t lin = gemm_plan_image_bytes(1, H, plan_kpad(H));
  const size_t post0 = gemm_plan_image_bytes(D, F, plan_kpad(F) + plan_kpad(4 * (int64_t)F));
  return align256(std::max(std::max(grouped, post0), std::max(dx, lin)) + 256);
}

extern "C" int32_t gnx_pna_conv_bwd(gnx_handle* h, const gnx_pna_bwd_args* a) { return gnx_pna_conv_bwd_images(h, a, nullptr); }

extern "C" int32_t gnx_pna_conv_bwd_images(gnx_handle* h, const gnx_pna_bwd_args* a, const gnx_pna_layer_images* im) {
  GNX_CHECK_ARG(h && a, "gnx_pna_conv_bwd: NULL argument");
  const int T = a->T, F = a->F, pre = a->pre_layers, post = a->post_layers, R = a->R, D = a->D;
  const int64_t N = a->N, E = a->E;
  const int H = T * F;
  GNX_CHECK_ARG(T >= 1 && F >= 1 && pre >= 1 && pre <= GNX_PNA_MAX_LAYERS && post >= 1 && post <= GNX_PNA_MAX_LAYERS &&
                    T <= GNX_PNA_MAX_TOWERS && D >= 1 && R >= 1,
                "gnx_pna_conv_bwd: bad layer shape T=%d F=%d pre=%d post=%d D=%d R=%d", T, F, pre, post, D, R);
  GNX_CHECK_ARG(a->params && a->grads && a->dout && a->x && a->A && a->dx && a->acc_buf, "gnx_pna_conv_bwd: NULL array");
  const bool side = a->use_side_streams != 0;
  const int per = 2 * (pre + post);
  auto pidx = [&](int t, bool is_pre, int i) { return 4 + t * per + 2 * (is_pre ? i : pre + i); };
  const float* const* P = a->params;
  float* const* G = a->grads;
  const float* lin_w = P[2];
  WgradQueue wq;

  const class_tiles ct = {a->dperm, a->tiles, a->ntiles, a->max_tiles};

  int gi = 0;
  float* g = a->gbuf[gi];
  const float* z_last = a->zs[a->n_z - 1];
  int last_hidden;
  const bool tail = (a->flags & GNX_PNA_BWD_LAST_OF_PASS) != 0;
  const bool defer = (a->flags & GNX_PNA_BWD_DEFER_SMALL) != 0;
  std::vector<std::function<int32_t()>> class_wgrads;
  if (a->merged) {
    if (!defer) {
      GNX_TRY(gnx_fill(h, a->dWm, (int64_t)H * H, 0.f));
      GNX_TRY(gnx_fill(h, a->dbm, H, 0.f));
    }
    wq.add(a->dout, H, z_last, H, N, H, H, a->dWm, H, a->dbm);
    gnx_gemm_seg s = seg(a->dout, H, a->Wm, H, H);
    GNX_TRY(gnx_gemm(h, 1, &s, N, H, nullptr, z_last, H, g, H, 0, a->ws, a->ws_bytes));
    last_hidden = post - 2;
  } else {
    wq.add(a->dout, H, z_last, H, N, H, H, G[2], H, G[3]);
    gnx_gemm_seg s = seg(a->dout, H, lin_w, H, H);
    GNX_TRY(gnx_gemm(h, 1, &s, N, H, nullptr, nullptr, 0, g, H, 0, a->ws, a->ws_bytes));
    last_hidden = post - 1;
  }
  for (int i = last_hidden; i >= 1; --i) {
    const float* a_prev = a->zs[i - 1];
    for (int t = 0; t < T; ++t) {
      const int k = pidx(t, false, i);
      wq.add(g + t * F, H, a_prev + t * F, H, N, F, F, G[k], F, G[k + 1]);
      gnx_gemm_seg s = seg(g + t * F, H, P[k], F, F);
      GNX_TRY(gnx_gemm(h, 1, &s, N, F, nullptr, a_prev + t * F, H, a->gbuf[gi + 1] + t * F, H, 0, a->ws, a->ws_bytes));
    }
    g = a->gbuf[++gi];
  }
  for (int t = 0; t < T; ++t) {
    const int k = pidx(t, false, 0);
    const float* gt = g + t * F;
    const float* At = a->A + (int64_t)t * 4 * F;
    float* dWp = G[k];
    wq.add(gt, H, a->x + t * F, H, N, F, F, dWp, 13 * F, G[k + 1]);
    float* dWeff = a->dWeff + (int64_t)t * D * F * 4 * F;
    if (!defer) GNX_TRY(gnx_fill(h, dWeff, (int64_t)D * F * 4 * F, 0.f));
    auto class_wgrad = [&, gt, At, dWeff, dWp]() -> int32_t {
      GNX_TRY(gnx_gemm_wgrad_grouped(h, gt, H, At, (int64_t)T * 4 * F, N, F, 4 * F, dWeff, 4 * F, (int64_t)F * 4 * F, a->dperm,
                                     a->chunks, a->nchunks, a->max_chunks));
      return defer ? GNX_OK : gnx_pna_weff_bwd(h, dWeff, F, D, a->avg_deg_log, dWp, 13 * F);
    };
    if (side)
      class_wgrads.push_back(class_wgrad);
    else
      GNX_TRY(class_wgrad());
    GNX_TRY(run_with_image(h, pna_dA_product(a->weff[t], T, F, D, t, g, a->dA), N, ct, im ? im->dA[t] : nullptr,
                           im ? &im->dA_rec[t] : nullptr, a->ws, a->ws_bytes));
  }
  const float* g_post0 = g;
  int ei = 0;
  float* ge = a->gebuf[ei];
  GNX_TRY(gnx_pna_aggregate_bwd(h, a->dA, a->hs[a->n_h - 1], a->A, a->rowptr, N, E, T, F, ge));
  for (auto& fn : class_wgrads) GNX_TRY(on_side(h, 0, side, fn));
  bool fused_bwd = pre == 2 && a->etile_info != nullptr && E > 0 && F % 4 == 0 && F <= 128 &&
                   R <= 64 && a16(ge) && a16(a->hs[0]) && a16(a->gebuf[1]) && a16(a->dP) && a16(a->dTe);
  for (int t = 0; t < T && fused_bwd; ++t) fused_bwd = a16(P[pidx(t, true, 1)]);
  if (fused_bwd) {
    const float* W1[GNX_PNA_MAX_TOWERS];
    for (int t = 0; t < T; ++t) {
      const int k = pidx(t, true, 1);
      W1[t] = P[k];
      wq.add(ge + t * F, H, a->hs[0] + t * F, H, E, F, F, G[k], F, G[k + 1]);
    }
    if (!defer) GNX_TRY(gnx_fill(h, a->dTe, (int64_t)R * H, 0.f));
    GNX_TRY(gnx_pna_edge_bwd(h, ge, a->hs[0], a->code, a->rowptr, a->etile_info, a->etile_w, N, E, T, F, R, W1, a->gebuf[1], a->dP,
                             a->dTe));
    ge = a->gebuf[++ei];
    GNX_TRY(gnx_edge_combine_bwd(h, ge, a->rowptr, a->colptr, a->cpos, a->code, N, E, H, 0, nullptr, a->dQ, nullptr, nullptr, 0));
  } else {
    for (int i = pre - 1; i >= 1; --i) {
      const float* h_prev = a->hs[i - 1];
      for (int t = 0; t < T; ++t) {
        const int k = pidx(t, true, i);
        wq.add(ge + t * F, H, h_prev + t * F, H, E, F, F, G[k], F, G[k + 1]);
        gnx_gemm_seg s = seg(ge + t * F, H, P[k], F, F);
        GNX_TRY(gnx_gemm(h, 1, &s, E, F, nullptr, h_prev + t * F, H, a->gebuf[ei + 1] + t * F, H, 0, a->ws, a->ws_bytes));
      }
      ge = a->gebuf[++ei];
    }
    GNX_TRY(gnx_edge_combine_bwd(h, ge, a->rowptr, a->colptr, a->cpos, a->code, N, E, H, 0, a->dP, a->dQ, nullptr, nullptr, 0));
  }
  for (int t = 0; t < T; ++t) {
    float* dW0 = G[pidx(t, true, 0)];
    wq.add(a->dP + t * F, H, a->x + t * F, H, N, F, F, dW0, 3 * F, nullptr);
    wq.add(a->dQ + t * F, H, a->x + t * F, H, N, F, F, dW0 + F, 3 * F, nullptr);
  }
  auto flush_batched = [&]() -> int32_t {
    const int wgs_saved = h->opt[GNX_OPT_WGRAD_WGS];
    if (tail && wgs_saved == 0) h->opt[GNX_OPT_WGRAD_WGS] = h->num_cus > 0 ? h->num_cus : 256;
    const int32_t fst = wq.flush(h);
    h->opt[GNX_OPT_WGRAD_WGS] = wgs_saved;
    return fst;
  };
  const bool flush_before_dx = side && !tail;
  if (flush_before_dx) GNX_TRY(on_side(h, 0, side, flush_batched));
  for (int t = 0; t < T; ++t)
    GNX_TRY(run_with_image(h, pna_dx_product(P, T, F, pre, post, t, g_post0, a->dP, a->dQ, a->dx), N, ct, im ? im->dx[t] : nullptr,
                           im ? &im->dx_rec[t] : nullptr, a->ws, a->ws_bytes));
  GNX_TRY(on_side(h, 1, side, [&]() -> int32_t {
    if (!fused_bwd) {
      if (!defer) GNX_TRY(gnx_fill(h, a->dTe, (int64_t)R * H, 0.f));
      if (E > 0) GNX_TRY(gnx_key_segment_sum(h, ge, a->code_pos, a->code, E, H, a->dTe));
    }
    if (defer) return GNX_OK;
    for (int t = 0; t < T; ++t) {
      const int k0 = pidx(t, true, 0);
      GNX_TRY(gnx_gemm_wgrad(h, a->dTe + t * F, H, a->EE, F, nullptr, R, F, F, G[k0] + 2 * F, 3 * F, G[k0 + 1]));
      gnx_gemm_seg s = seg(a->dTe + t * F, H, P[k0] + 2 * F, 3 * F, F);
      GNX_TRY(gnx_gemm(h, 1, &s, R, F, nullptr, nullptr, 0, a->dEE, F, t > 0 ? GNX_GEMM_ACCUMULATE : 0, nullptr, 0));
    }
    GNX_TRY(gnx_gemm_wgrad(h, a->dEE, F, a->BE, H, nullptr, R, F, H, G[0], H, G[1]));
    if (a->acc_first) GNX_TRY(gnx_fill(h, a->acc_buf, (int64_t)R * H, 0.f));
    gnx_gemm_seg s = seg(a->dEE, F, P[0], H, F);
    return gnx_gemm(h, 1, &s, R, H, nullptr, nullptr, 0, a->acc_buf, H, GNX_GEMM_ACCUMULATE, nullptr, 0);
  }));
  GNX_TRY(on_side(h, 0, side, [&]() -> int32_t {
    if (!flush_before_dx) GNX_TRY(flush_batched());
    if (!a->merged || defer) return GNX_OK;
    const float* dbm = a->dbm;
    for (int t = 0; t < T; ++t) {
      const int k = pidx(t, false, post - 1);
      const float* Wt = P[k];
      const float* bt = P[k + 1];
      gnx_gemm_seg s1 = seg(a->dWm + t * F, H, Wt, F, F);
      GNX_TRY(gnx_gemm(h, 1, &s1, H, F, nullptr, nullptr, 0, G[2] + t * F, H, GNX_GEMM_ACCUMULATE | GNX_GEMM_B_TRANS, nullptr, 0));
      gnx_gemm_seg s2 = seg(dbm, 1, bt, 1, 1);
      GNX_TRY(gnx_gemm(h, 1, &s2, H, F, nullptr, nullptr, 0, G[2] + t * F, H, GNX_GEMM_ACCUMULATE | GNX_GEMM_B_TRANS, nullptr, 0));
      GNX_TRY(gnx_gemm_wgrad(h, lin_w + t * F, H, a->dWm + t * F, H, nullptr, H, F, F, G[k], F, nullptr));
      gnx_gemm_seg s3 = seg(dbm, H, lin_w + t * F, H, H);
      GNX_TRY(gnx_gemm(h, 1, &s3, 1, F, nullptr, nullptr, 0, G[k + 1], F, GNX_GEMM_ACCUMULATE, nullptr, 0));
    }
    return gnx_axpy(h, G[3], dbm, H, 1.0f);
  }));
  return GNX_OK;
}

struct weff_batch_args {
  const float* W[GNX_SMALL_BATCH];
  float* out[GNX_SMALL_BATCH];
  float avg_log[GNX_SMALL_BATCH];
  int64_t ldw;
  int F, D;
};

#define WEFF_BLOCK 256
#define WEFF_CLS (WEFF_BLOCK / 4 + 2)
__global__ void __launch_bounds__(WEFF_BLOCK) k_pna_weff_batched(weff_batch_args a) {
  __shared__ float s_amp[WEFF_CLS], s_att[WEFF_CLS];
  const int b = blockIdx.y;
  const int F = a.F;
  const int64_t first = (int64_t)blockIdx.x * WEFF_BLOCK;
  int64_t i = first + threadIdx.x;
  int64_t per = (int64_t)F * 4 * F;
  const int d0 = (int)(first / per);
  if (threadIdx.x < WEFF_CLS) {
    const double dd = (double)(d0 + (int)threadIdx.x), avg = (double)a.avg_log[b];
    s_amp[threadIdx.x] = (float)(log(dd + 1.0) / avg);
    s_att[threadIdx.x] = (float)(avg / log(fmax(dd, 1.0) + 1.0));
  }
  __syncthreads();
  if (i >= per * a.D) return;
  int d = (int)(i / per);
  int o = (int)((i % per) / (4 * F)), j = (int)(i % (4 * F));
  const float amp = s_amp[d - d0], att = s_att[d - d0];
  const float* w = a.W[b] + (int64_t)o * a.ldw;
  a.out[b][i] = w[F + j] + amp * w[5 * F + j] + att * w[9 * F + j];
}

struct weff_bwd_batch_args {
  const float* dWeff[GNX_SMALL_BATCH];
  float* dW[GNX_SMALL_BATCH];
  float avg_log[GNX_SMALL_BATCH];
  int64_t lddw;
  int F, D;
};

__global__ void k_pna_weff_bwd_batched(weff_bwd_batch_args a) {
  const int b = blockIdx.y;
  const int F = a.F;
  int64_t i = (int64_t)blockIdx.x * blockDim.x + threadIdx.x;
  int64_t per = (int64_t)F * 4 * F;
  if (i >= per) return;
  int o = (int)(i / (4 * F)), j = (int)(i % (4 * F));
  float s1 = 0.f, s2 = 0.f, s3 = 0.f;
  const float avg_log = a.avg_log[b];
  const float* dWeff = a.dWeff[b];
  for (int d = 0; d < a.D; ++d) {
    float dd = (float)d;
    float amp = logf(dd + 1.0f) / avg_log;
    float att = avg_log / logf(fmaxf(dd, 1.0f) + 1.0f);
    float v = dWeff[(int64_t)d * per + i];
    s1 += v;
    s2 += amp * v;
    s3 += att * v;
  }
  float* w = a.dW[b] + (int64_t)o * a.lddw;
  w[F + j] += s1;
  w[5 * F + j] += s2;
  w[9 * F + j] += s3;
}

extern "C" int32_t gnx_pna_weff_bwd_batched(gnx_handle* h, int32_t n, const float* const* dWeff, int32_t F, int32_t D,
                                            const float* avg_deg_log, float* const* dW, int64_t lddw) {
  GNX_CHECK_ARG(h && dWeff && dW && avg_deg_log && n >= 0 && F > 0 && D > 0 && lddw >= 13 * F,
                "gnx_pna_weff_bwd_batched: bad argument");
// ... 298 lines not shown
```

gnnepcsaft_amd/ops.py:

```python
from __future__ import annotations

import ctypes as C
import threading
from typing import List, Optional, Sequence, Tuple

import torch

from . import _lib
from ._lib import GemmSeg, check, handle

_I32 = C.c_int32


def _f32(t: torch.Tensor, name: str) -> torch.Tensor:
    if t.dtype != torch.float32:
        raise _lib.GnxError(_lib.GNX_E_INVALID, f"{name}: expected float32, got {t.dtype}")
    return t


def _mat(t: torch.Tensor, name: str) -> Tuple[int, int]:
    if t.dtype is not torch.float32:
        raise _lib.GnxError(_lib.GNX_E_INVALID, f"{name}: expected float32, got {t.dtype}")
    shape, strides = t.shape, t.stride()
    if len(shape) != 2 or (shape[1] > 1 and strides[1] != 1):
# ... 683 lines not shown

def run_on_second_side_stream(ref: torch.Tensor, tensors, fn) -> None:
    _run_on_side(ref, tensors, fn, which=1)


def gemm_wgrad_inline(dC: torch.Tensor, A: torch.Tensor, dW: torch.Tensor, dbias: Optional[torch.Tensor] = None) -> None:
    _gemm_wgrad_launch(dC, A, dW, None, dbias)


def axpy_(y: torch.Tensor, x: torch.Tensor, alpha: float = 1.0) -> torch.Tensor:
    if y.numel() != x.numel() or not (y.is_contiguous() and x.is_contiguous()):
        raise _lib.GnxError(_lib.GNX_E_INVALID, "axpy_: need contiguous tensors of equal size")
    check(_lib.load().gnx_axpy(handle(y.device), _f32(y, "y").data_ptr(), _f32(x, "x").data_ptr(), y.numel(),
                               float(alpha)))
    return y


def gemm_wgrad(dC: torch.Tensor, A: torch.Tensor, dW: torch.Tensor, *, rowscale: Optional[torch.Tensor] = None,
               dbias: Optional[torch.Tensor] = None) -> None:
    if dC.size(0) == 0:
        return
    _run_on_side(dC, (dC, A, rowscale, dW, dbias), lambda: _gemm_wgrad_launch(dC, A, dW, rowscale, dbias))


def pna_post0_wgrad_classes(g: torch.Tensor, A: torch.Tensor, dc: "DegreeClasses", F: int, avg_deg_log: float,
                            dW: torch.Tensor) -> None:
    if g.size(0) == 0:
        return
    dWeff = zeros(dc.D, F, 4 * F, device=g.device)

    def run():
        gemm_wgrad_grouped(g, A, dWeff, dc)
        pna_weff_bwd(dWeff, F, dc.D, avg_deg_log, dW)

    _run_on_side(g, (g, A, dWeff, dW), run)


def _gemm_wgrad_launch(dC, A, dW, rowscale, dbias) -> None:
    M, N = dC.shape
    xp, ldx = _mat(dC, "dC")
    ap, lda = _mat(A, "A")
    wp, ldw = _mat(dW, "dW")
    K = A.size(1)
    if A.size(0) != M or dW.size(0) != N or dW.size(1) != K:
        raise _lib.GnxError(_lib.GNX_E_INVALID, f"wgrad shapes dC {tuple(dC.shape)} A {tuple(A.shape)} "
                                                f"dW {tuple(dW.shape)}")
    check(_lib.load().gnx_gemm_wgrad(handle(dW.device), xp, ldx, ap, lda, _ptr(rowscale), M, N, K, wp, ldw,
                                     _ptr(dbias)))


def edge_combine_fwd(P: torch.Tensor, Q: torch.Tensor, Te: torch.Tensor, g: GraphPack, relu: bool) -> torch.Tensor:
    H = P.size(1)
    h1 = torch.empty(g.E, H, dtype=torch.float32, device=P.device)
    check(_lib.load().gnx_edge_combine_fwd(handle(P.device), P.data_ptr(), Q.data_ptr(), Te.data_ptr(),
                                           g.src.data_ptr(), g.dst.data_ptr(), g.code.data_ptr(), g.E, H, int(relu),
                                           h1.data_ptr()))
    return h1


def edge_combine_bwd_pq(gr: torch.Tensor, g: GraphPack) -> Tuple[torch.Tensor, torch.Tensor]:
    H = gr.size(1)
    dP = torch.empty(g.N, H, dtype=torch.float32, device=gr.device)
    dQ = torch.empty(g.N, H, dtype=torch.float32, device=gr.device)
    check(_lib.load().gnx_edge_combine_bwd(handle(gr.device), gr.data_ptr(), g.rowptr.data_ptr(), g.colptr.data_ptr(),
                                           g.cpos.data_ptr(), g.code.data_ptr(), g.N, g.E, H, 0, dP.data_ptr(),
                                           dQ.data_ptr(), None, None, 0))
    return dP, dQ


def bond_table_grad(gr: torch.Tensor, g: GraphPack, R: int, pos: Optional[torch.Tensor]) -> torch.Tensor:
    H = gr.size(1)
    dTe = zeros(R, H, device=gr.device)
    lib = _lib.load()
    if g.E == 0:
        return dTe
    if pos is not None:
        check(lib.gnx_key_segment_sum(handle(gr.device), gr.data_ptr(), pos.data_ptr(), g.code.data_ptr(), g.E, H,
                                      dTe.data_ptr()))
        return dTe
    nbytes = lib.gnx_table_scatter_workspace_bytes(g.E, R, H)
    ws = torch.empty(max(nbytes, 1), dtype=torch.uint8, device=gr.device)
    tmp = torch.empty(2, g.N, H, dtype=torch.float32, device=gr.device)
    check(lib.gnx_edge_combine_bwd(handle(gr.device), gr.data_ptr(), g.rowptr.data_ptr(), g.colptr.data_ptr(),
                                   g.cpos.data_ptr(), g.code.data_ptr(), g.N, g.E, H, R, tmp[0].data_ptr(),
                                   tmp[1].data_ptr(), dTe.data_ptr(), ws.data_ptr(), nbytes))
    return dTe


def bond_code_index(g: GraphPack, R: int, H: int) -> Optional[torch.Tensor]:
    return g.code_index(R) if ((H % 4 == 0 and H <= 1024) or H <= 256) and g.E > 0 else None


def edge_combine_bwd(gr: torch.Tensor, g: GraphPack, R: int) -> Tuple[torch.Tensor, torch.Tensor, torch.Tensor]:
    dP, dQ = edge_combine_bwd_pq(gr, g)
    return dP, dQ, bond_table_grad(gr, g, R, bond_code_index(g, R, gr.size(1)))


def pna_edge_fwd(P: torch.Tensor, Q: torch.Tensor, Te: torch.Tensor, g: GraphPack, T: int, F: int,
                 weights: Sequence[torch.Tensor], biases: Sequence[torch.Tensor], max_degree: int,
                 keep: bool = True) -> Tuple[Optional[torch.Tensor], Optional[torch.Tensor], torch.Tensor]:
    H = T * F
    tiles = g.edge_tiles(max_degree)
    if tiles is None and g.E > 0:
        raise _lib.GnxError(_lib.GNX_E_INVALID, f"pna_edge_fwd: in-degree bound {max_degree} too large for edge tiles")
    dev = P.device
    h1 = torch.empty(g.E, H, dtype=torch.float32, device=dev) if keep else None
    m = torch.empty(g.E, H, dtype=torch.float32, device=dev) if keep else None
    A = torch.empty(g.N, T * 4 * F, dtype=torch.float32, device=dev)
    warr = (C.c_void_p * T)(*[_f32(w, "W1").data_ptr() for w in weights])
    barr = (C.c_void_p * T)(*[_f32(b, "b1").data_ptr() for b in biases])
    for w in weights:
        if tuple(w.shape) != (F, F) or not w.is_contiguous():
            raise _lib.GnxError(_lib.GNX_E_INVALID, f"pna_edge_fwd: pre-layer 1 weight must be contiguous [{F},{F}]")
    info, w_ = tiles if tiles is not None else (None, 1)
    check(_lib.load().gnx_pna_edge_fwd(handle(dev), P.data_ptr(), Q.data_ptr(), Te.data_ptr(), g.src.data_ptr(),
                                       g.dst.data_ptr(), g.code.data_ptr(), g.rowptr.data_ptr(), _ptr(info), w_, g.N, g.E,
                                       T, F, C.cast(warr, C.POINTER(C.c_void_p)), C.cast(barr, C.POINTER(C.c_void_p)),
                                       _ptr(h1), _ptr(m), A.data_ptr()))
    return h1, m, A


def pna_edge_bwd(ge: torch.Tensor, h1: torch.Tensor, g: GraphPack, T: int, F: int, R: int,
                 weights: Sequence[torch.Tensor], max_degree: int) -> Tuple[torch.Tensor, torch.Tensor, torch.Tensor]:
    H = T * F
    tiles = g.edge_tiles(max_degree)
    if tiles is None and g.E > 0:
        raise _lib.GnxError(_lib.GNX_E_INVALID, f"pna_edge_bwd: in-degree bound {max_degree} too large for edge tiles")
    dev = ge.device
    gh1 = torch.empty(g.E, H, dtype=torch.float32, device=dev)
    dP = torch.empty(g.N, H, dtype=torch.float32, device=dev)
    dTe = zeros(R, H, device=dev)
    warr = (C.c_void_p * T)(*[_f32(w, "W1").data_ptr() for w in weights])
    info, w_ = tiles if tiles is not None else (None, 1)
    check(_lib.load().gnx_pna_edge_bwd(handle(dev), _f32(ge, "ge").contiguous().data_ptr(), _f32(h1, "h1").contiguous().data_ptr(),
                                       g.code.data_ptr(), g.rowptr.data_ptr(), _ptr(info), w_, g.N, g.E, T, F, R,
                                       C.cast(warr, C.POINTER(C.c_void_p)), gh1.data_ptr(), dP.data_ptr(), dTe.data_ptr()))
    return gh1, dP, dTe


def pna_aggregate_fwd(m: torch.Tensor, g: GraphPack, T: int, F: int) -> torch.Tensor:
    A = torch.empty(g.N, T * 4 * F, dtype=torch.float32, device=m.device)
    check(_lib.load().gnx_pna_aggregate_fwd(handle(m.device), m.data_ptr(), g.rowptr.data_ptr(), g.N, g.E, T, F,
                                            A.data_ptr()))
    return A


def pna_aggregate_bwd(dA: torch.Tensor, m: torch.Tensor, A: torch.Tensor, g: GraphPack, T: int, F: int) -> torch.Tensor:
    dm = torch.empty_like(m)
    check(_lib.load().gnx_pna_aggregate_bwd(handle(m.device), dA.data_ptr(), m.data_ptr(), A.data_ptr(),
                                            g.rowptr.data_ptr(), g.N, g.E, T, F, dm.data_ptr()))
    return dm


def gine_aggregate_fwd(x: torch.Tensor, Le: torch.Tensor, g: GraphPack, eps: float) -> torch.Tensor:
    out = torch.empty_like(x)
    check(_lib.load().gnx_gine_aggregate_fwd(handle(x.device), x.data_ptr(), Le.data_ptr(), g.rowptr.data_ptr(),
                                             g.src.data_ptr(), g.code.data_ptr(), g.N, g.E, x.size(1), float(eps),
                                             out.data_ptr()))
    return out


def gine_aggregate_bwd(dout: torch.Tensor, x: torch.Tensor, Le: torch.Tensor, g: GraphPack,
                       eps: float, want_dle: bool = True) -> Tuple[torch.Tensor, Optional[torch.Tensor]]:
    dx = torch.empty_like(x)
    dLe = zeros(*Le.shape, device=Le.device) if want_dle else None
    pos = g.code_index(Le.size(0)) if (g.E > 0 and want_dle) else None
    check(_lib.load().gnx_gine_aggregate_bwd(handle(x.device), dout.data_ptr(), x.data_ptr(), Le.data_ptr(),
                                             g.colptr.data_ptr(), g.cpos.data_ptr(), g.src.data_ptr(),
                                             g.dst.data_ptr(), g.code.data_ptr(), _ptr(pos), g.N, g.E, x.size(1),
                                             Le.size(0), float(eps), dx.data_ptr(), _ptr(dLe)))
    return dx, dLe


def gine_dle(dout: torch.Tensor, x: torch.Tensor, Le: torch.Tensor, g: GraphPack, pos: Optional[torch.Tensor]) -> torch.Tensor:
    dLe = zeros(*Le.shape, device=Le.device)
    check(_lib.load().gnx_gine_dle(handle(x.device), dout.data_ptr(), x.data_ptr(), Le.data_ptr(), g.src.data_ptr(),
                                   g.dst.data_ptr(), g.code.data_ptr(), _ptr(pos), g.E, x.size(1), Le.size(0),
                                   dLe.data_ptr()))
    return dLe


def transformer_attn_fwd(qkvs: torch.Tensor, Le: torch.Tensor, g: GraphPack, heads: int, p: float = 0.0,
                         seed: int = 0, offset: int = 0, want_mask: bool = False
                         ) -> Tuple[torch.Tensor, torch.Tensor, Optional[torch.Tensor]]:
    qkvs = _f32(qkvs, "qkvs").contiguous()
    Le = _f32(Le, "Le").contiguous()
    N, H = qkvs.size(0), qkvs.size(1) // 4
    if qkvs.size(1) != 4 * H or Le.size(1) != H or heads <= 0 or H % heads != 0:
        raise _lib.GnxError(_lib.GNX_E_INVALID, f"transformer_attn_fwd: qkvs {tuple(qkvs.shape)} Le {tuple(Le.shape)} "
                                                f"heads {heads}")
    dev = qkvs.device
    out = torch.empty(N, H, dtype=torch.float32, device=dev)
    alpha = torch.empty(g.E, heads, dtype=torch.float32, device=dev)
    keep = torch.empty(g.E, heads, dtype=torch.uint8, device=dev) if want_mask else None
    check(_lib.load().gnx_transformer_attn_fwd(handle(dev), qkvs.data_ptr(), Le.data_ptr(), g.rowptr.data_ptr(),
                                               g.src.data_ptr(), g.code.data_ptr(), N, g.E, int(heads), H // int(heads),
                                               float(p), int(seed) & (2 ** 64 - 1), int(offset) & (2 ** 64 - 1),
                                               out.data_ptr(), alpha.data_ptr(), _ptr(keep)))
    return out, alpha, keep


def transformer_attn_bwd(dout: torch.Tensor, qkvs: torch.Tensor, Le: torch.Tensor, alpha: torch.Tensor, g: GraphPack,
                         heads: int, p: float = 0.0, seed: int = 0, offset: int = 0, want_dle: bool = True
                         ) -> Tuple[torch.Tensor, torch.Tensor, Optional[torch.Tensor]]:
    dout = _f32(dout, "dout").contiguous()
    N, H = dout.shape
    dev = dout.device
    dqkv = torch.empty(N, 3 * H, dtype=torch.float32, device=dev)
    scratch = torch.empty(2, g.E, heads, dtype=torch.float32, device=dev)
    dLe = zeros(*Le.shape, device=dev) if want_dle else None
    pos = g.code_index(Le.size(0)) if (want_dle and g.E > 0) else None
    if want_dle and g.E > 0 and pos is None:
        raise _lib.GnxError(_lib.GNX_E_INVALID, f"transformer_attn_bwd: {Le.size(0)} bond codes exceed the inverted index")
    check(_lib.load().gnx_transformer_attn_bwd(handle(dev), dout.data_ptr(), qkvs.data_ptr(), Le.data_ptr(),
                                               alpha.data_ptr(), g.rowptr.data_ptr(), g.src.data_ptr(), g.dst.data_ptr(),
                                               g.code.data_ptr(), g.colptr.data_ptr(), g.cpos.data_ptr(), _ptr(pos), N,
                                               g.E, int(heads), H // int(heads), Le.size(0), float(p),
                                               int(seed) & (2 ** 64 - 1), int(offset) & (2 ** 64 - 1), dqkv.data_ptr(),
                                               scratch.data_ptr(), _ptr(dLe)))
    return dqkv, scratch, dLe


def transformer_attn_dle(dout: torch.Tensor, qkvs: torch.Tensor, scratch: torch.Tensor, Le: torch.Tensor, g: GraphPack,
                         heads: int, pos: Optional[torch.Tensor]) -> torch.Tensor:
    R, H = Le.shape
    dLe = zeros(R, H, device=dout.device)
    if g.E == 0:
        return dLe
    if pos is None:
        raise _lib.GnxError(_lib.GNX_E_INVALID, f"transformer_attn_dle: {R} bond codes exceed the inverted index")
    check(_lib.load().gnx_transformer_attn_dle(handle(dout.device), dout.data_ptr(), qkvs.data_ptr(), scratch.data_ptr(),
                                               g.dst.data_ptr(), g.code.data_ptr(), pos.data_ptr(), g.E, int(heads),
                                               H // int(heads), R, dLe.data_ptr()))
    return dLe


def _f64_on(t: torch.Tensor, name: str, dev: torch.device) -> torch.Tensor:
    if t.dtype != torch.float64 or t.device != dev:
        raise _lib.GnxError(_lib.GNX_E_INVALID, f"{name}: expected float64 on {dev}, got {t.dtype} on {t.device}")
    return t.contiguous()


def _pcsaft_args(params: torch.Tensor, owner: torch.Tensor, T: torch.Tensor, name: str):
    dev = params.device
    params = _f64_on(params, f"{name}: params", dev)
    if params.dim() != 2 or params.size(1) != 9:
        raise _lib.GnxError(_lib.GNX_E_INVALID, f"{name}: params must be [B, 9], got {tuple(params.shape)}")
    if owner.dtype != torch.int64 or owner.device != dev or owner.dim() != 1:
        raise _lib.GnxError(_lib.GNX_E_INVALID, f"{name}: owner must be a 1-D int64 tensor on {dev}")
    T = _f64_on(T, f"{name}: T", dev)
    if T.shape != owner.shape:
        raise _lib.GnxError(_lib.GNX_E_INVALID, f"{name}: T {tuple(T.shape)} and owner {tuple(owner.shape)} differ")
    return params, owner.contiguous(), T


_F64, _ST = torch.float64, torch.int32


def _pcsaft_outs(out, specs, dev: torch.device, name: str):
    if out is None:
        return tuple(None if s is None else torch.empty(s[0], dtype=s[1], device=dev) for s in specs)
    if len(out) != len(specs):
        raise _lib.GnxError(_lib.GNX_E_INVALID, f"{name}: out must hold {len(specs)} tensors, got {len(out)}")
    for t, s in zip(out, specs):
        if t is not None and (s is None or tuple(t.shape) != s[0] or t.dtype != s[1] or t.device != dev
                              or not t.is_contiguous()):
            raise _lib.GnxError(_lib.GNX_E_INVALID, f"{name}: out does not match the outputs of this call")
    return tuple(out)


def _pcsaft_density(params, owner, T, P, out=None):
    params, owner, T = _pcsaft_args(params, owner, T, "pcsaft_density")
    P = _f64_on(P, "pcsaft_density: P", params.device)
    if P.shape != T.shape:
        raise _lib.GnxError(_lib.GNX_E_INVALID, f"pcsaft_density: P {tuple(P.shape)} and T {tuple(T.shape)} differ")
    n, dev = T.numel(), params.device
    rho, status = _pcsaft_outs(out, [((n,), _F64), ((n,), _ST)], dev, "pcsaft_density")
    check(_lib.load().gnx_pcsaft_density(handle(dev), params.data_ptr(), params.size(0), owner.data_ptr(),
                                         T.data_ptr(), P.data_ptr(), n, rho.data_ptr(), status.data_ptr()))
    return rho, status


def pcsaft_density(params: torch.Tensor, owner: torch.Tensor, T: torch.Tensor, P: torch.Tensor
                   ) -> Tuple[torch.Tensor, torch.Tensor]:
    return _pcsaft_density(params, owner, T, P)


def _pcsaft_vapor_pressure(params, owner, T, out=None):
    params, owner, T = _pcsaft_args(params, owner, T, "pcsaft_vapor_pressure")
    n, dev = T.numel(), params.device
    out = _pcsaft_outs(out, [((n,), _F64)] * 3 + [((n,), _ST)], dev, "pcsaft_vapor_pressure")
    check(_lib.load().gnx_pcsaft_vapor_pressure(handle(dev), params.data_ptr(), params.size(0), owner.data_ptr(),
                                                T.data_ptr(), n, *map(_ptr, out)))
    return out


def pcsaft_vapor_pressure(params: torch.Tensor, owner: torch.Tensor, T: torch.Tensor
                          ) -> Tuple[torch.Tensor, torch.Tensor, torch.Tensor, torch.Tensor]:
    return _pcsaft_vapor_pressure(params, owner, T)


_PCSAFT_MIX = {"pcsaft_mix_state": ("gnx_pcsaft_mix_state", (0, 0, 0)),
               "pcsaft_mix_density": ("gnx_pcsaft_mix_density", (0,)),
               "pcsaft_mix_lnphi_state": ("gnx_pcsaft_mix_lnphi_state", (1, 0)),
               "pcsaft_mix_lnphi": ("gnx_pcsaft_mix_lnphi", (0, 1, 1)),
               "pcsaft_mix_bubble": ("gnx_pcsaft_mix_bubble", (0, 1, 0, 0)),
# ... 272 lines not shown
```

include/gnx.h:

```cpp
#ifndef GNX_H_
#define GNX_H_

#include <stddef.h>
#include <stdint.h>

#ifdef __cplusplus
extern "C" {
#endif

#define GNX_ABI_VERSION 7

enum {
  GNX_OK = 0,
  GNX_E_INVALID = -1,
  GNX_E_HIP = -2,
  GNX_E_RANGE = -3,
  GNX_E_WORKSPACE = -4
};

typedef struct gnx_handle gnx_handle;

int32_t gnx_create(gnx_handle** out, int32_t device);
int32_t gnx_destroy(gnx_handle* h);
int32_t gnx_set_stream(gnx_handle* h, void* hip_stream);
const char* gnx_last_error(void);
int32_t gnx_abi_version(void);

enum {
  GNX_OPT_GEMM_SPLIT = 0,
  GNX_OPT_WGRAD_WGS = 1,
  GNX_OPT_EMBED_BWD_MFMA = 2,
  GNX_OPT_STD_BWD_CENTERED = 3,
  GNX_OPT_GEMM_PIPE = 4,
  GNX_OPT_WGRAD_PIPE = 5,
  GNX_OPT_GEMM_AS = 6,
  GNX_OPT_GEMM_WS_FAST = 7,
  GNX_OPT_GEMM_TILE_ROWS = 8,
  GNX_OPT_GEMM_MID = 9,
  GNX_OPT_COUNT = 10
};
int32_t gnx_set_option(gnx_handle* h, int32_t opt, int32_t value);
int32_t gnx_get_option(gnx_handle* h, int32_t opt, int32_t* value);

enum {
  GNX_K_NONE = 0,
  GNX_K_PNA_AGG_FWD = 1,
  GNX_K_PNA_AGG_BWD = 2,
  GNX_K_GEMM_WS = 3,
  GNX_K_GEMM_WGRAD = 4,
  GNX_K_GINE_AGG_FWD = 5,
  GNX_K_GINE_AGG_BWD = 6,
  GNX_K_EDGE_COMBINE_FWD = 7,
  GNX_K_EDGE_COMBINE_BWD = 8,
  GNX_K_BN_FWD = 9,
  GNX_K_BN_BWD = 10,
  GNX_K_GEMM_TILED = 11,
  GNX_K_GEMM_SMALL = 12,
  GNX_K_GEMM_WGRAD_BATCHED = 13,
  GNX_K_KEY_SEGMENT_SUM = 14,
  GNX_K_EMBED = 15,
  GNX_K_PNA_EDGE_FWD = 16,
  GNX_K_PNA_EDGE_BWD = 17,
  GNX_K_ATTN_FWD = 18,
  GNX_K_ATTN_BWD = 19,
  GNX_K_PCSAFT_RHO = 20,
  GNX_K_PCSAFT_VP = 21,
  GNX_K_PCSAFT_MIX_STATE = 22,
  GNX_K_PCSAFT_MIX_RHO = 23,
  GNX_K_PCSAFT_MIX_LNPHI_STATE = 24,
  GNX_K_PCSAFT_MIX_LNPHI = 25,
  GNX_K_COUNT = 26
};
int32_t gnx_prof_begin(gnx_handle* h, uint32_t kernel_mask);
int32_t gnx_prof_read(gnx_handle* h, int32_t kid, int64_t* launches, double* total_ms, double* alg_bytes,
                      double* alg_flops, double* mfma_bf16_flops);
int32_t gnx_prof_end(gnx_handle* h);

size_t gnx_pack_csr_workspace_bytes(int64_t N, int64_t E);
int32_t gnx_pack_csr(gnx_handle* h, const int64_t* edge_index, int64_t E, int64_t N, int32_t* rowptr, int32_t* perm,
                     int32_t* src, int32_t* dst, int32_t* colptr, int32_t* cpos, void* ws, size_t ws_bytes);
int32_t gnx_feature_code(gnx_handle* h, const int64_t* feat, int64_t rows, int32_t K, const int32_t* dims,
                         const int32_t* perm, int32_t* code, void* ws, size_t ws_bytes);
int32_t gnx_graph_ptr(gnx_handle* h, const int64_t* batch, int64_t N, int64_t B, int32_t* graph_ptr, void* ws,
                      size_t ws_bytes);
int32_t gnx_degree_scalers(gnx_handle* h, const int32_t* rowptr, int64_t N, float avg_deg_log, float* amp, float* att);

int32_t gnx_collate_ptr(gnx_handle* h, const int64_t* node_ptr, const int64_t* edge_ptr, int64_t G, const int64_t* idx,
                        int64_t B, int64_t* out_ptr, int64_t* out_eptr);
int32_t gnx_collate_gather(gnx_handle* h, const int64_t* node_ptr, const int64_t* edge_ptr, int64_t G, const int64_t* x,
                           const int64_t* edge_index, const int64_t* edge_attr, int64_t E_src, const int64_t* idx,
                           int64_t B, const int64_t* out_ptr, const int64_t* out_eptr, int64_t N, int64_t E,
                           int64_t* x_out, int64_t* edge_index_out, int64_t* edge_attr_out, int64_t* batch_out);
int32_t gnx_collate_rows(gnx_handle* h, const void* src, int64_t G, const int64_t* idx, int64_t B, int32_t elem_bytes,
                         int32_t K, void* dst);

int32_t gnx_embed_sum_fwd(gnx_handle* h, const int64_t* idx, int64_t N, int32_t K, const int32_t* offsets,
                          const float* table, int32_t H, float* out);
size_t gnx_table_scatter_workspace_bytes(int64_t rows, int32_t R, int32_t H);
int32_t gnx_embed_sum_bwd(gnx_handle* h, const int64_t* idx, int64_t N, int32_t K, const int32_t* offsets,
                          int32_t R, const float* dout, int32_t H, float* dtable, void* ws, size_t ws_bytes);
int32_t gnx_check_range(gnx_handle* h);

typedef struct {
  const float* a;
  int64_t lda;
  const float* rowscale;
  const float* b;
  int64_t ldb;
  int32_t k;
  int32_t _pad;
} gnx_gemm_seg;

enum {
  GNX_GEMM_RELU = 1,
  GNX_GEMM_ACCUMULATE = 2,
  GNX_GEMM_B_TRANS = 4,
  GNX_GEMM_SPLIT_ONLY = 8,
  GNX_GEMM_PRESPLIT = 16
};
size_t gnx_gemm_workspace_bytes(gnx_handle* h, int32_t nseg, const gnx_gemm_seg* segs, const int64_t* cls_strides,
                                int32_t num_classes, int64_t M, int32_t N, const float* mask, int32_t flags,
                                int32_t grouped);
int32_t gnx_gemm(gnx_handle* h, int32_t nseg, const gnx_gemm_seg* segs, int64_t M, int32_t N, const float* bias,
                 const float* mask, int64_t ldmask, float* C, int64_t ldc, int32_t flags, void* ws, size_t ws_bytes);
int32_t gnx_gemm_wgrad(gnx_handle* h, const float* dC, int64_t lddc, const float* A, int64_t lda,
                       const float* rowscale, int64_t M, int32_t N, int32_t K, float* dW, int64_t lddw, float* dbias);

typedef struct {
  const float* dC;
  int64_t lddc;
  const float* A;
  int64_t lda;
  const float* rowscale;
  float* dW;
  int64_t lddw;
  float* dbias;
  int64_t M;
  int32_t N, K;
} gnx_wgrad_prob;
int32_t gnx_gemm_wgrad_batched(gnx_handle* h, int32_t nprob, const gnx_wgrad_prob* probs);

enum { GNX_SB_A_TRANS = 1, GNX_SB_B_TRANS = 2, GNX_SB_ACCUMULATE = 4, GNX_SB_ATOMIC = 8, GNX_SB_RELU = 16 };
#define GNX_SMALL_BATCH 32
typedef struct {
  const float* A;
  int64_t lda;
  const float* B;
  int64_t ldb;
  const float* bias;
  float* C;
  int64_t ldc;
  int32_t M, N, K;
  int32_t flags;
} gnx_small_prob;
int32_t gnx_gemm_small_batched(gnx_handle* h, int32_t nprob, const gnx_small_prob* probs);

int32_t gnx_degree_max(gnx_handle* h, const int32_t* rowptr, int64_t N, int32_t* max_degree_host);
size_t gnx_degree_classes_workspace_bytes(int64_t N, int32_t D);
int32_t gnx_degree_classes(gnx_handle* h, const int32_t* rowptr, int64_t N, int32_t D, int32_t* dperm,
                           int32_t* cls_ptr, void* ws, size_t ws_bytes);
int32_t gnx_class_tiles(gnx_handle* h, const int32_t* cls_ptr, int32_t D, int32_t tile_rows, int32_t* tile_info,
                        int32_t* ntiles);
int32_t gnx_gemm_grouped(gnx_handle* h, int32_t nseg, const gnx_gemm_seg* segs, const int64_t* cls_strides,
                         int32_t num_classes, int64_t M, int32_t N, const float* bias, const float* mask,
                         int64_t ldmask, float* C, int64_t ldc, int32_t flags, const int32_t* row_index,
                         const int32_t* tile_info, const int32_t* ntiles, int64_t max_tiles, void* ws, size_t ws_bytes);
int32_t gnx_gemm_tile_rows(gnx_handle* h, int64_t M, int32_t N);
int32_t gnx_gemm_grouped_rows(gnx_handle* h, int32_t nseg, const gnx_gemm_seg* segs, const int64_t* cls_strides,
                              int32_t num_classes, int64_t M, int32_t N, const float* bias, const float* mask,
                              int64_t ldmask, float* C, int64_t ldc, int32_t flags, const int32_t* row_index,
                              const int32_t* tile_info, const int32_t* ntiles, int64_t max_tiles, void* ws,
                              size_t ws_bytes, int32_t tile_rows);
enum {
  GNX_GEMM_KERNEL_NONE = 0,
  GNX_GEMM_KERNEL_TILED_VEC = 1,
  GNX_GEMM_KERNEL_TILED_GENERIC = 2,
  GNX_GEMM_KERNEL_WS = 3,
  GNX_GEMM_KERNEL_WS3 = 4,
  GNX_GEMM_KERNEL_WS3_FAST8 = 5,
  GNX_GEMM_KERNEL_WS3_FAST4 = 6,
  GNX_GEMM_KERNEL_GEMM3 = 7,
  GNX_GEMM_KERNEL_GEMM3P_96 = 8,
  GNX_GEMM_KERNEL_GEMM3P_128 = 9,
  GNX_GEMM_KERNEL_AS3 = 10,
  GNX_GEMM_KERNEL_MID = 11,
  GNX_GEMM_KERNEL_SMALL = 12,
  GNX_GEMM_KERNEL_COUNT = 13
};
typedef struct {
  int32_t kernel;
  int32_t tile_rows;
  uint32_t grid_x, grid_y, block;
// ... 155 lines not shown
int32_t gnx_pcsaft_mix_dew_t(gnx_handle* h, const double* params, int64_t B, const int64_t* mix_comp,
                             const double* mix_kij, const double* mix_eab, int64_t M, int32_t nc, const int64_t* owner,
                             const double* P, const double* y, const double* T0, int64_t n, double* T, double* x,
                             double* rho_l, double* rho_v, int32_t* status);
int32_t gnx_pcsaft_mix_flash(gnx_handle* h, const double* params, int64_t B, const int64_t* mix_comp,
                             const double* mix_kij, const double* mix_eab, int64_t M, int32_t nc, const int64_t* owner,
                             const double* T, const double* P, const double* z, int64_t n, double* beta, double* x,
                             double* y, double* rho_l, double* rho_v, int32_t* status);
int32_t gnx_pcsaft_mix_stability(gnx_handle* h, const double* params, int64_t B, const int64_t* mix_comp,
                                 const double* mix_kij, const double* mix_eab, int64_t M, int32_t nc, const int64_t* owner,
                                 const int64_t* trial, const double* T, const double* P, const double* z, int64_t n,
                                 double* tpd, double* w, double* rho_w, double* rho_z, int32_t* status);
int32_t gnx_pcsaft_mix_lle(gnx_handle* h, const double* params, int64_t B, const int64_t* mix_comp,
                           const double* mix_kij, const double* mix_eab, int64_t M, int32_t nc, const int64_t* owner,
                           const double* T, const double* P, const double* z, const double* w0, int64_t n, double* beta,
                           double* x, double* y, double* rho_x, double* rho_y, int32_t* status);

enum { GNX_POOL_ADD = 0, GNX_POOL_MEAN = 1, GNX_POOL_MAX = 2 };
int32_t gnx_segment_pool_fwd(gnx_handle* h, const float* x, const int32_t* ptr, int64_t B, int32_t H, int32_t mode,
                             float* out);
int32_t gnx_segment_pool_bwd(gnx_handle* h, const float* dout, const float* x, const float* out, const int32_t* ptr,
                             int64_t B, int32_t H, int32_t mode, float* dx);

size_t gnx_batchnorm_workspace_bytes(int64_t M, int32_t H);
int32_t gnx_batchnorm_fwd(gnx_handle* h, const float* x, int64_t M, int32_t H, const float* gamma, const float* beta,
                          float* running_mean, float* running_var, int64_t* num_batches_tracked, float momentum,
                          float eps, int32_t training, int32_t relu, float* y, float* save_mean, float* save_rstd,
                          void* ws, size_t ws_bytes);
int32_t gnx_batchnorm_bwd(gnx_handle* h, const float* dy, const float* x, const float* y, int64_t M, int32_t H,
                          const float* gamma, const float* save_mean, const float* save_rstd, int32_t relu,
                          float* dx, float* dgamma, float* dbeta, void* ws, size_t ws_bytes);
int32_t gnx_batchnorm_bwd_x(gnx_handle* h, const float* dy, const float* x, int64_t M, int32_t H, const float* gamma,
                            const float* beta, const float* save_mean, const float* save_rstd, int32_t relu, float* dx,
                            float* dgamma, float* dbeta, void* ws, size_t ws_bytes);

int32_t gnx_dropout(gnx_handle* h, const float* x, int64_t n, float p, uint64_t seed, uint64_t offset, float* y);

int32_t gnx_huber_ape(gnx_handle* h, const float* pred, const float* target, int64_t count, float delta, float* out2,
                      float* dpred);

int32_t gnx_adamw_amsgrad(gnx_handle* h, float* p, const float* g, float* m, float* v, float* vmax, int64_t n, float lr,
                          float beta1, float beta2, float eps, float weight_decay, int64_t step);
int32_t gnx_sgd(gnx_handle* h, float* p, const float* g, int64_t n, float lr);

#define GNX_PNA_MAX_LAYERS 8
#define GNX_PNA_MAX_TOWERS 8
enum {
  GNX_PNA_BWD_DEFER_SMALL = 1,
  GNX_PNA_BWD_LAST_OF_PASS = 2
};
typedef struct {
  int64_t N, E;
  int32_t T, F, pre_layers, post_layers, R, D;
  float avg_deg_log;
  int32_t merged;
  int32_t acc_first;
  int32_t use_side_streams;
  int32_t n_h, n_z;
  const int32_t *rowptr, *colptr, *cpos, *code, *code_pos, *dperm, *tiles, *ntiles, *chunks, *nchunks;
  int64_t max_tiles, max_chunks;
  const float *x, *BE, *EE, *A;
  const float* hs[GNX_PNA_MAX_LAYERS];
  const float* zs[GNX_PNA_MAX_LAYERS];
  const float* weff[GNX_PNA_MAX_TOWERS];
  const float* Wm;
  const float* const* params;
  float* const* grads;
  const float* dout;
  float* gbuf[GNX_PNA_MAX_LAYERS];
  float* dA;
  float* gebuf[GNX_PNA_MAX_LAYERS];
  float *dP, *dQ;
  float *dTe, *dEE;
  float *dWm, *dbm;
  float* dWeff;
  void* ws;
  size_t ws_bytes;
  float* acc_buf;
  float* dx;
  int32_t flags;
  int32_t etile_w;
  const int32_t* etile_info;
} gnx_pna_bwd_args;
size_t gnx_pna_conv_bwd_workspace_bytes(int32_t T, int32_t F, int32_t D);
int32_t gnx_pna_conv_bwd(gnx_handle* h, const gnx_pna_bwd_args* args);

typedef struct {
  int32_t L, T, F, pre_layers, post_layers, R, D, merged, use_side_streams, _pad;
  const float* BE;
  float* acc_buf;
  const float* ones;
  const float* avg_deg_log;
  const float* const* params;
  float* const* grads;
  const float* const* EE;
  float* const* dTe;
  float* const* dEE;
  const float* const* dWm;
  const float* const* dbm;
  const float* const* dWeff;
} gnx_pna_finish_args;
int32_t gnx_pna_stack_finish(gnx_handle* h, const gnx_pna_finish_args* args);
int32_t gnx_pna_weight_only_all(gnx_handle* h, int32_t L, const float* BE, int32_t R, int32_t T, int32_t F,
                                int32_t pre_layers, int32_t post_layers, int32_t D, const float* avg_deg_log,
                                const float* const* params, int32_t merged, float* const* EE, float* const* Te,
                                float* const* weff, float* const* Wm, float* const* bm);

int32_t gnx_pna_weight_only(gnx_handle* h, const float* BE, int32_t R, int32_t T, int32_t F, int32_t pre_layers,
                            int32_t post_layers, int32_t D, float avg_deg_log, const float* const* params, int32_t merged,
                            float* EE, float* Te, float* const* weff, float* Wm, float* bm);
typedef struct {
  int64_t N, E;
  int32_t T, F, pre_layers, post_layers, D, merged;
  const int32_t *rowptr, *src, *dst, *code, *dperm, *tiles, *ntiles;
  int64_t max_tiles;
  const float *x, *Te;
  const float* weff[GNX_PNA_MAX_TOWERS];
  const float *Wm, *bm;
  const float* const* params;
  float *P, *Q, *A;
  float* hs[GNX_PNA_MAX_LAYERS];
  float* zs[GNX_PNA_MAX_LAYERS];
  void* ws;
  size_t ws_bytes;
  float* out;
  const int32_t* etile_info;
  int32_t etile_w;
  int32_t tile_rows;
} gnx_pna_fwd_args;
int32_t gnx_pna_conv_fwd(gnx_handle* h, const gnx_pna_fwd_args* args);

typedef struct {
  uint64_t image_bytes;
  int32_t classes, Npad, Kpad;
  int32_t koff[5];
  int32_t frag;
  int32_t bt;
} gnx_gemm_image;
typedef struct {
  void* post0[GNX_PNA_MAX_TOWERS];
  void* dA[GNX_PNA_MAX_TOWERS];
  void* dx[GNX_PNA_MAX_TOWERS];
  gnx_gemm_image post0_rec[GNX_PNA_MAX_TOWERS], dA_rec[GNX_PNA_MAX_TOWERS], dx_rec[GNX_PNA_MAX_TOWERS];
} gnx_pna_layer_images;
size_t gnx_pna_split_all_bytes(gnx_handle* h, int32_t L, int32_t T, int32_t F, int32_t pre_layers, int32_t post_layers,
                               int32_t D, int64_t N, int32_t tile_rows);
int32_t gnx_pna_split_all(gnx_handle* h, int32_t L, int32_t T, int32_t F, int32_t pre_layers, int32_t post_layers, int32_t D,
                          int64_t N, int32_t tile_rows, const float* const* params, const float* const* weff, void* slab,
                          size_t slab_bytes, gnx_pna_layer_images* out);
int32_t gnx_gemm_split_counts(gnx_handle* h, int64_t* per_call, int64_t* batched);
int32_t gnx_pna_conv_fwd_images(gnx_handle* h, const gnx_pna_fwd_args* args, const gnx_pna_layer_images* images);
int32_t gnx_pna_conv_bwd_images(gnx_handle* h, const gnx_pna_bwd_args* args, const gnx_pna_layer_images* images);

int32_t gnx_fill(gnx_handle* h, float* p, int64_t n, float v);
int32_t gnx_scale(gnx_handle* h, float* p, int64_t n, float v);
int32_t gnx_axpy(gnx_handle* h, float* y, const float* x, int64_t n, float a);

int32_t gnx_side_begin(gnx_handle* h);
int32_t gnx_side_stream(gnx_handle* h, void** hip_stream);
int32_t gnx_side_end(gnx_handle* h);
int32_t gnx_side_join(gnx_handle* h);
int32_t gnx_side_stream_n(gnx_handle* h, int32_t which, void** hip_stream);
int32_t gnx_side_begin_n(gnx_handle* h, int32_t which);
int32_t gnx_side_join_n(gnx_handle* h, int32_t which);
int32_t gnx_clip_rows(gnx_handle* h, const float* x, int64_t M, int32_t P, const float* lo, const float* hi, float* y);

#ifdef __cplusplus
}
#endif
#endif
```

Measured before the change: 677,200 graphs/s.

## Fuse PNA dA GEMM with aggregation backward into one kernel

Adds a fused kernel that computes the dA product (split-bf16 MFMA GEMM against the effective weights) for a tile of rows and immediately applies the PNA mean/min/max/std aggregation backward to scatter gradients onto messages. The dA intermediate no longer needs a round trip through global memory and one launch per tower disappears. The aggregation backward body is moved into a shared header so both paths use the same code. The kernel adds register and LDS pressure, and it falls back to the unfused path when the plan declines.

```diff
diff --git a/gnnepcsaft_amd/_lib.py b/gnnepcsaft_amd/_lib.py
--- a/gnnepcsaft_amd/_lib.py
+++ b/gnnepcsaft_amd/_lib.py
@@ -11,7 +11,7 @@
 ABI_VERSION = 7
 GNX_OK, GNX_E_INVALID, GNX_E_HIP, GNX_E_RANGE, GNX_E_WORKSPACE = 0, -1, -2, -3, -4
 OPT_GEMM_SPLIT, OPT_WGRAD_WGS, OPT_EMBED_BWD_MFMA, OPT_STD_BWD_CENTERED, OPT_GEMM_PIPE, OPT_WGRAD_PIPE, OPT_GEMM_AS, \
-    OPT_GEMM_WS_FAST, OPT_GEMM_TILE_ROWS, OPT_GEMM_MID = range(10)
+    OPT_GEMM_WS_FAST, OPT_GEMM_TILE_ROWS, OPT_GEMM_MID, OPT_DA_AGG_FUSED = range(11)
 GEMM_RELU, GEMM_ACCUMULATE, GEMM_B_TRANS, GEMM_SPLIT_ONLY, GEMM_PRESPLIT = 1, 2, 4, 8, 16
 GEMM_KERNEL_NAMES = ("none", "k_gemm<vec>", "k_gemm<generic>", "k_gemm_ws", "k_gemm_ws3", "k_gemm_ws3<fast,8>",
                      "k_gemm_ws3<fast,4>", "k_gemm3", "k_gemm3p<96>", "k_gemm3p<128>", "k_gemm_as3", "k_gemm_mid",
@@ -250,6 +250,8 @@
     "gnx_gemm_split_counts": (_i32, [_vp, C.POINTER(_i64), C.POINTER(_i64)]),
     "gnx_pna_conv_fwd_images": (_i32, [_vp, C.POINTER(PnaFwdArgs), C.POINTER(PnaLayerImages)]),
     "gnx_pna_conv_bwd_images": (_i32, [_vp, C.POINTER(PnaBwdArgs), C.POINTER(PnaLayerImages)]),
+    "gnx_pna_da_aggregate_bwd": (_i32, [_vp, _vp, _i32, _i32, _i32, _i32, _vp, _vp, _vp, _vp, _i64, _i64, _vp, _vp, _vp, _vp,
+                                        _i64, _vp, C.POINTER(GemmImage), _vp, _sz, C.POINTER(_i32)]),
     "gnx_pna_weight_only_all": (_i32, [_vp, _i32, _vp, _i32, _i32, _i32, _i32, _i32, _i32, C.POINTER(_f32), C.POINTER(_vp),
                                        _i32, C.POINTER(_vp), C.POINTER(_vp), C.POINTER(_vp), C.POINTER(_vp), C.POINTER(_vp)]),
     "gnx_pna_stack_finish": (_i32, [_vp, C.POINTER(PnaFinishArgs)]),
diff --git a/gnnepcsaft_amd/csrc/gnx_aggregate.hip b/gnnepcsaft_amd/csrc/gnx_aggregate.hip
--- a/gnnepcsaft_amd/csrc/gnx_aggregate.hip
+++ b/gnnepcsaft_amd/csrc/gnx_aggregate.hip
@@ -1,4 +1,5 @@
 #include "gnx_common.hpp"
+#include "gnx_pna_agg_item.hpp"
 
 #include <cmath>
 #include <cstdlib>
@@ -17,33 +18,8 @@
   typedef float type;
 };
 
-template <int VEC>
-__device__ __forceinline__ void vload(float (&r)[VEC], const float* p) {
-  if constexpr (VEC == 4) {
-    f32x4 v = *reinterpret_cast<const f32x4*>(p);
-    r[0] = v.x;
-    r[1] = v.y;
-    r[2] = v.z;
-    r[3] = v.w;
-  } else {
-    r[0] = p[0];
-  }
-}
-template <int VEC>
-__device__ __forceinline__ void vstore(float* p, const float (&r)[VEC]) {
-  if constexpr (VEC == 4) {
-    f32x4 v = {r[0], r[1], r[2], r[3]};
-    *reinterpret_cast<f32x4*>(p) = v;
-  } else {
-    p[0] = r[0];
-  }
-}
-
 __device__ __forceinline__ float relu_keep_nan(float r) { return (r < 0.f) ? 0.f : r; }
 __device__ __forceinline__ float max_keep_nan(float s, float a) { return (a > s || a != a) ? a : s; }
-
-#define STD_VAR_MIN 1e-5f
-#define STD_MASK_AT 0.0031622776601683794f
 
 template <int VEC>
 __global__ void __launch_bounds__(256) k_pna_agg_fwd(const float* __restrict__ m, const int* __restrict__ rowptr,
@@ -149,139 +125,7 @@
   vload<VEC>(gmn, dA + ao + F);
   vload<VEC>(gmx, dA + ao + 2 * F);
   vload<VEC>(gsd, dA + ao + 3 * F);
-  float s[VEC], s2[VEC], mn[VEC], mx[VEC];
-#pragma unroll
-  for (int v = 0; v < VEC; ++v) {
-    s[v] = 0.f;
-    s2[v] = 0.f;
-    mn[v] = INFINITY;
-    mx[v] = -INFINITY;
-  }
-  if (p1 - p0 <= 4) {
-    const int deg = p1 - p0;
-    float a[4][VEC];
-#pragma unroll
-    for (int e = 0; e < 4; ++e) vload<VEC>(a[e], m + (int64_t)(p0 + (e < deg ? e : 0)) * H + c);
-#pragma unroll
-    for (int e = 0; e < 4; ++e)
-      if (e < deg) {
-#pragma unroll
-        for (int v = 0; v < VEC; ++v) {
-          s[v] = __fadd_rn(s[v], a[e][v]);
-          s2[v] = __fadd_rn(s2[v], __fmul_rn(a[e][v], a[e][v]));
-          mn[v] = fminf(mn[v], a[e][v]);
-          mx[v] = fmaxf(mx[v], a[e][v]);
-        }
-      }
-    const float cnt = (float)deg;
-    float mean[VEC], sd[VEC], nmn[VEC], nmx[VEC], c2[VEC];
-#pragma unroll
-    for (int v = 0; v < VEC; ++v) {
-      c2[v] = 0.f;
-      mean[v] = __fdiv_rn(s[v], cnt);
-      float mean2 = __fdiv_rn(s2[v], cnt);
-      float var = __fsub_rn(mean2, __fmul_rn(mean[v], mean[v]));
-      float o = __fsqrt_rn(fmaxf(var, STD_VAR_MIN));
-      sd[v] = (o <= STD_MASK_AT) ? 0.f : o;
-      nmn[v] = (mn[v] == 0.f) ? 1.f : 0.f;
-      nmx[v] = (mx[v] == 0.f) ? 1.f : 0.f;
-    }
-#pragma unroll
-    for (int e = 0; e < 4; ++e)
-      if (e < deg) {
-#pragma unroll
-        for (int v = 0; v < VEC; ++v) {
-          nmn[v] += (a[e][v] == mn[v]) ? 1.f : 0.f;
-          nmx[v] += (a[e][v] == mx[v]) ? 1.f : 0.f;
-          const float dv = a[e][v] - mean[v];
-          c2[v] = fmaf(dv, dv, c2[v]);
-        }
-      }
-    float k_mean[VEC], k_mn[VEC], k_mx[VEC], k_sd[VEC];
-#pragma unroll
-    for (int v = 0; v < VEC; ++v) {
-      k_mean[v] = gmean[v] / cnt;
-      k_mn[v] = gmn[v] / nmn[v];
-      k_mx[v] = gmx[v] / nmx[v];
-      const float sdiv = (centered && c2[v] > 0.f) ? sqrtf(c2[v] / cnt) : sd[v];
-      k_sd[v] = (sd[v] > 0.f) ? gsd[v] / (cnt * sdiv) : 0.f;
-    }
-    float* dp = dm + (int64_t)p0 * H + c;
-#pragma unroll
-    for (int e = 0; e < 4; ++e)
-      if (e < deg) {
-        float o[VEC];
-#pragma unroll
-        for (int v = 0; v < VEC; ++v) {
-          float r = k_mean[v] + k_sd[v] * (a[e][v] - mean[v]);
-          r += (a[e][v] == mn[v]) ? k_mn[v] : 0.f;
-          r += (a[e][v] == mx[v]) ? k_mx[v] : 0.f;
-          o[v] = r;
-        }
-        vstore<VEC>(dp + (int64_t)e * H, o);
-      }
-    return;
-  }
-  const float* mp = m + (int64_t)p0 * H + c;
-  for (int p = p0; p < p1; ++p, mp += H) {
-    float a[VEC];
-    vload<VEC>(a, mp);
-#pragma unroll
-    for (int v = 0; v < VEC; ++v) {
-      s[v] = __fadd_rn(s[v], a[v]);
-      s2[v] = __fadd_rn(s2[v], __fmul_rn(a[v], a[v]));
-      mn[v] = fminf(mn[v], a[v]);
-      mx[v] = fmaxf(mx[v], a[v]);
-    }
-  }
-  const float cnt = (float)(p1 - p0);
-  float mean[VEC], sd[VEC], nmn[VEC], nmx[VEC], c2[VEC];
-#pragma unroll
-  for (int v = 0; v < VEC; ++v) {
-    c2[v] = 0.f;
-    mean[v] = __fdiv_rn(s[v], cnt);
-    float mean2 = __fdiv_rn(s2[v], cnt);
-    float var = __fsub_rn(mean2, __fmul_rn(mean[v], mean[v]));
-    float o = __fsqrt_rn(fmaxf(var, STD_VAR_MIN));
-    sd[v] = (o <= STD_MASK_AT) ? 0.f : o;
-    nmn[v] = (mn[v] == 0.f) ? 1.f : 0.f;
-    nmx[v] = (mx[v] == 0.f) ? 1.f : 0.f;
-  }
-  mp = m + (int64_t)p0 * H + c;
-  for (int p = p0; p < p1; ++p, mp += H) {
-    float a[VEC];
-    vload<VEC>(a, mp);
-#pragma unroll
-    for (int v = 0; v < VEC; ++v) {
-      nmn[v] += (a[v] == mn[v]) ? 1.f : 0.f;
-      nmx[v] += (a[v] == mx[v]) ? 1.f : 0.f;
-      const float dv = a[v] - mean[v];
-      c2[v] = fmaf(dv, dv, c2[v]);
-    }
-  }
-  float k_mean[VEC], k_mn[VEC], k_mx[VEC], k_sd[VEC];
-#pragma unroll
-  for (int v = 0; v < VEC; ++v) {
-    k_mean[v] = gmean[v] / cnt;
-    k_mn[v] = gmn[v] / nmn[v];
-    k_mx[v] = gmx[v] / nmx[v];
-    const float sdiv = (centered && c2[v] > 0.f) ? sqrtf(c2[v] / cnt) : sd[v];
-    k_sd[v] = (sd[v] > 0.f) ? gsd[v] / (cnt * sdiv) : 0.f;
-  }
-  mp = m + (int64_t)p0 * H + c;
-  float* dp = dm + (int64_t)p0 * H + c;
-  for (int p = p0; p < p1; ++p, mp += H, dp += H) {
-    float a[VEC], o[VEC];
-    vload<VEC>(a, mp);
-#pragma unroll
-    for (int v = 0; v < VEC; ++v) {
-      float r = k_mean[v] + k_sd[v] * (a[v] - mean[v]);
-      r += (a[v] == mn[v]) ? k_mn[v] : 0.f;
-      r += (a[v] == mx[v]) ? k_mx[v] : 0.f;
-      o[v] = r;
-    }
-    vstore<VEC>(dp, o);
-  }
+  pna_agg_bwd_item<VEC>(gmean, gmn, gmx, gsd, p0, p1, m + c, dm + c, H, centered);
 }
 
 extern "C" int32_t gnx_pna_aggregate_bwd(gnx_handle* h, const float* dA, const float* m, const float* A,
diff --git a/gnnepcsaft_amd/csrc/gnx_api.hip b/gnnepcsaft_amd/csrc/gnx_api.hip
--- a/gnnepcsaft_amd/csrc/gnx_api.hip
+++ b/gnnepcsaft_amd/csrc/gnx_api.hip
@@ -45,7 +45,8 @@
               {GNX_OPT_EMBED_BWD_MFMA, "GNX_EMBED_BWD_MFMA", 1}, {GNX_OPT_STD_BWD_CENTERED, "GNX_STD_BWD_CENTERED", 1},
               {GNX_OPT_GEMM_PIPE, "GNX_GEMM_PIPE", 1},           {GNX_OPT_WGRAD_PIPE, "GNX_WGRAD_PIPE", 1},
               {GNX_OPT_GEMM_AS, "GNX_GEMM_AS", 1},               {GNX_OPT_GEMM_WS_FAST, "GNX_GEMM_WS_FAST", 2},
-              {GNX_OPT_GEMM_TILE_ROWS, "GNX_GEMM_TILE_ROWS", 0}, {GNX_OPT_GEMM_MID, "GNX_GEMM_MID", 1}};
+              {GNX_OPT_GEMM_TILE_ROWS, "GNX_GEMM_TILE_ROWS", 0}, {GNX_OPT_GEMM_MID, "GNX_GEMM_MID", 1},
+              {GNX_OPT_DA_AGG_FUSED, "GNX_DA_AGG_FUSED", 1}};
   for (const auto& o : opts) {
     const char* e = getenv(o.env);
     h->opt[o.id] = e ? atoi(e) : o.def;
diff --git a/gnnepcsaft_amd/csrc/gnx_gemm.hip b/gnnepcsaft_amd/csrc/gnx_gemm.hip
--- a/gnnepcsaft_amd/csrc/gnx_gemm.hip
+++ b/gnnepcsaft_amd/csrc/gnx_gemm.hip
@@ -1,4 +1,5 @@
 #include "gnx_gemm_plan.hpp"
+#include "gnx_pna_agg_item.hpp"
 #include "gnx_split.hpp"
 
 #include <cstdlib>
@@ -1494,6 +1495,178 @@
     as_stamp_buf[(size_t)blockIdx.x * 8 + 6] = clock64();
   }
 #endif
+}
+
+#define DAF_BM 32
+#define DAF_PIECE (DAF_BM * AS_LDA)
+#define DAF_LDS (3 * DAF_PIECE + DAF_BM * 4)
+
+struct daf_args {
+  const float* m;
+  const int* rowptr;
+  float* ge;
+  int H;
+  int centered;
+};
+
+__global__ void __launch_bounds__(256, 2) k_pna_dA_agg_bwd(gemm_args g, daf_args x) {
+  extern __shared__ __attribute__((aligned(16))) unsigned char lds_daf[];
+  unsigned char* const A3 = lds_daf;
+  int* const rown = reinterpret_cast<int*>(lds_daf + 3 * DAF_PIECE);
+
+  const int tid = threadIdx.x;
+  const int lane = tid & 63;
+  const int wave = tid >> 6;
+  const int li = lane & 31, lh = lane >> 5;
+  constexpr int NT = 4;
+
+  const int t = blockIdx.x >> 2, part = blockIdx.x & 3;
+  if (t >= g.ntiles[0]) return;
+  const int p0 = g.tile_info[3 * t] + DAF_BM * part;
+  int pr = g.tile_info[3 * t + 1] - DAF_BM * part;
+  const int cls = g.tile_info[3 * t + 2];
+  if (pr <= 0) return;
+  pr = pr < DAF_BM ? pr : DAF_BM;
+
+  const seg_dev& s = g.seg[0];
+  const int lr = tid >> 5, k4 = (tid & 31) * 4;
+  f32x4 ra[4];
+#pragma unroll
+  for (int q = 0; q < 4; ++q) {
+    const int r = lr + 8 * q;
+    const int row = g.row_index[p0 + (r < pr ? r : pr - 1)];
+    ra[q] = *reinterpret_cast<const f32x4*>(s.a + (int64_t)row * s.lda + k4);
+  }
+  if (tid < DAF_BM) rown[tid] = g.row_index[p0 + (tid < pr ? tid : pr - 1)];
+
+  constexpr int total_kt = NT * 4;
+  const __bf16* const bbase = g.bsplit + ((int64_t)cls * NT * 4 * 3) * (BN * BK) + (wave * 64 + lane) * 8;
+  bf16x8 bq[2][2][3];
+  auto load_b = [&](int slot, int sl, int j) {
+    const __bf16* p = bbase + (int64_t)(j < total_kt ? j : total_kt - 1) * (3 * BN * BK);
+#pragma unroll
+    for (int pc = 0; pc < 3; ++pc) bq[slot][sl][pc] = *reinterpret_cast<const bf16x8*>(p + ((sl * 3 + pc) * 4 * 64) * 8);
+  };
+  load_b(0, 0, 0);
+  load_b(0, 1, 0);
+
+  typedef __attribute__((ext_vector_type(2))) float f32x2;
+#pragma unroll
+  for (int q = 0; q < 4; q += 2) {
+    float xa[8];
+#pragma unroll
+    for (int j = 0; j < 4; ++j) {
+      xa[j] = ra[q][j];
+      xa[4 + j] = ra[q + 1][j];
+    }
+    bf16x8 pc[3];
+    split3(xa, pc[0], pc[1], pc[2]);
+#pragma unroll
+    for (int p = 0; p < 3; ++p) {
+      const f32x4 w = *reinterpret_cast<const f32x4*>(&pc[p]);
+      unsigned char* qa = A3 + p * DAF_PIECE + (lr + 8 * q) * AS_LDA + k4 * 2;
+      *reinterpret_cast<f32x2*>(qa) = f32x2{w.x, w.y};
+      *reinterpret_cast<f32x2*>(qa + 8 * AS_LDA) = f32x2{w.z, w.w};
+    }
+  }
+  load_b(1, 0, 1);
+  load_b(1, 1, 1);
+  __syncthreads();
+
+  const int qj = li & 3;
+  const int lc = wave * 32 + (li >> 2) * 4;
+  int e0[4], e1[4];
+#pragma unroll
+  for (int gq = 0; gq < 4; ++gq) {
+    const int r = 8 * gq + 4 * lh + qj;
+    const int node = rown[r];
+    e0[gq] = x.rowptr[node];
+    e1[gq] = r < pr ? x.rowptr[node + 1] : e0[gq];
+  }
+#pragma unroll
+  for (int gq = 0; gq < 4; ++gq) asm volatile("" ::"v"(e0[gq]), "v"(e1[gq]));
+
+  int afrag = li * AS_LDA + 16 * lh;
+  bf16x8 af[2][3];
+  auto read_a = [&](int slot, int off, int ks) {
+    const unsigned char* base = A3 + off;
+#pragma unroll
+    for (int p = 0; p < 3; ++p) af[slot][p] = *reinterpret_cast<const bf16x8*>(base + p * DAF_PIECE + ks * 32);
+  };
+  read_a(0, afrag, 0);
+
+  const f32x4 bv = *reinterpret_cast<const f32x4*>(c_zero4);
+  const float floor_v = g.relu ? 0.f : -__builtin_inff();
+  asm volatile("" ::"v"(bv));
+  auto quad_swap = [&](float& a, float& b, auto CTRL, bool hi) {
+    const float send = hi ? a : b;
+    const float got = __builtin_bit_cast(float, __builtin_amdgcn_mov_dpp(__builtin_bit_cast(int, send), decltype(CTRL)::value, 0xf, 0xf, true));
+    a = hi ? got : a;
+    b = hi ? b : got;
+  };
+  using XOR1 = std::integral_constant<int, 0xB1>;
+  using XOR2 = std::integral_constant<int, 0x4E>;
+
+  const float* const mc = x.m + lc;
+  float am[4][4][4];
+  auto load_messages = [&]() {
+#pragma unroll
+    for (int gq = 0; gq < 4; ++gq) {
+      const int deg = e1[gq] - e0[gq];
+#pragma unroll
+      for (int e = 0; e < 4; ++e) vload<4>(am[gq][e], mc + (deg > 0 ? (e0[gq] + (e < deg ? e : 0)) * x.H : 0));
+    }
+  };
+
+  f32x4 kept[NT][4];
+#pragma unroll
+  for (int nt = 0; nt < NT; ++nt) {
+    asm volatile("" : "+v"(afrag));
+    f32x16 acc;
+#pragma unroll
+    for (int r = 0; r < 16; ++r) acc[r] = 0.f;
+#pragma unroll
+    for (int ks = 0; ks < 8; ++ks) {
+      const int kt = ks >> 1, sl = ks & 1;
+      read_a((ks + 1) & 1, afrag, (ks + 1) & 7);
+      __builtin_amdgcn_sched_barrier(0);
+      mfma_3x3(acc, af[ks & 1], bq[kt & 1][sl]);
+      load_b(kt & 1, sl, nt * 4 + kt + 2);
+      __builtin_amdgcn_sched_barrier(0);
+    }
+#pragma unroll
+    for (int gq = 0; gq < 4; ++gq) {
+      float c0 = acc[4 * gq], c1 = acc[4 * gq + 1], c2 = acc[4 * gq + 2], c3 = acc[4 * gq + 3];
+      quad_swap(c0, c1, XOR1{}, (qj & 1) != 0);
+      quad_swap(c2, c3, XOR1{}, (qj & 1) != 0);
+      quad_swap(c0, c2, XOR2{}, (qj & 2) != 0);
+      quad_swap(c1, c3, XOR2{}, (qj & 2) != 0);
+      f32x4 v = {c0 + bv.x, c1 + bv.y, c2 + bv.z, c3 + bv.w};
+#pragma unroll
+      for (int e = 0; e < 4; ++e) v[e] = fmaxf(v[e], floor_v);
+      kept[nt][gq] = v;
+    }
+  }
+
+  load_messages();
+  float* const gec = x.ge + lc;
+#pragma unroll
+  for (int gq = 0; gq < 4; ++gq) {
+    const int deg = e1[gq] - e0[gq];
+    if (deg <= 0) continue;
+    float gmean[4], gmn[4], gmx[4], gsd[4];
+#pragma unroll
+    for (int e = 0; e < 4; ++e) {
+      gmean[e] = kept[0][gq][e];
+      gmn[e] = kept[1][gq][e];
+      gmx[e] = kept[2][gq][e];
+      gsd[e] = kept[3][gq][e];
+    }
+    if (deg <= 4)
+      pna_agg_bwd_item_loaded<4>(gmean, gmn, gmx, gsd, deg, am[gq], gec + (int64_t)e0[gq] * x.H, x.H, x.centered);
+    else
+      pna_agg_bwd_item_loop<4>(gmean, gmn, gmx, gsd, e0[gq], e1[gq], mc, gec, x.H, x.centered);
+  }
 }
 
 #define MID_T 16
@@ -1941,6 +2114,63 @@
                      tile_info, ntiles, max_tiles, ws, ws_bytes);
 }
 
+static_assert(PLAN_DAF_BM == DAF_BM && PLAN_DAF_LDS == DAF_LDS, "plan / k_pna_dA_agg_bwd");
+
+extern "C" int32_t gnx_pna_da_aggregate_bwd(gnx_handle* h, const float* weff_t, int32_t T, int32_t F, int32_t D, int32_t t,
+                                            const float* g, const float* dA, const float* m, const int32_t* rowptr, int64_t N,
+                                            int64_t E, float* ge, const int32_t* dperm, const int32_t* tiles,
+                                            const int32_t* ntiles, int64_t max_tiles, void* image, const gnx_gemm_image* rec,
+                                            void* ws, size_t ws_bytes, int32_t* fused) {
+  GNX_CHECK_ARG(h && fused, "gnx_pna_da_aggregate_bwd: NULL argument");
+  *fused = 0;
+  GNX_CHECK_ARG(T >= 1 && F >= 1 && D >= 1 && D <= 4096 && t >= 0 && t < T && N >= 0 && E >= 0,
+                "gnx_pna_da_aggregate_bwd: bad shape T=%d F=%d D=%d t=%d N=%lld E=%lld", T, F, D, t, (long long)N, (long long)E);
+  GNX_CHECK_ARG(weff_t && g && dA && rowptr && dperm && tiles && ntiles && max_tiles > 0, "gnx_pna_da_aggregate_bwd: NULL argument");
+  GNX_CHECK_ARG(E == 0 || (m && ge), "gnx_pna_da_aggregate_bwd: NULL messages");
+  if (N == 0 || E == 0) return GNX_OK;
+  const int64_t H = (int64_t)T * F;
+  const pna_product q = pna_dA_product(weff_t, T, F, D, t, g, const_cast<float*>(dA));
+  int32_t extra = 0;
+  void* img = ws;
+  size_t img_bytes = ws_bytes;
+  if (image != nullptr && rec != nullptr && rec->image_bytes > 0) {
+    const gemm_plan p = pna_product_plan(q, N, GNX_GEMM_PRESPLIT, image, max_tiles, h->opt, h->num_cus);
+    if (p.images && gemm_image_equal(gemm_image_of(p), *rec)) {
+      extra = GNX_GEMM_PRESPLIT;
+      img = image;
+      img_bytes = (size_t)rec->image_bytes;
+    }
+  }
+  const pna_dA_agg_plan f = pna_dA_agg_plan_of(q, N, E, H, m, ge, extra, img, max_tiles, h->opt, h->num_cus);
+  if (!f.fused) return GNX_OK;
+  const gemm_plan& p = f.product;
+  if (img_bytes < p.image_bytes) {
+    gnx_set_error("gnx_pna_da_aggregate_bwd: workspace of %zu bytes, the split weight images need %zu", img_bytes, p.image_bytes);
+    return GNX_E_WORKSPACE;
+  }
+  GNX_CHECK_ARG(aligned16(img), "gnx_pna_da_aggregate_bwd: workspace must be 16-byte aligned");
+  if (p.run_split) {
+    const int32_t st = gemm_launch(h, q.nseg, q.seg, q.stride, q.classes, N, q.N, nullptr, nullptr, 0, q.C, q.ldc, GNX_GEMM_SPLIT_ONLY,
+                                   dperm, tiles, ntiles, max_tiles, img, img_bytes);
+    if (st != GNX_OK) return st;
+  }
+  gemm_args ga = {{},    1,     N,      q.N,    nullptr, nullptr,
+                  0,     q.C,   q.ldc,  0,      dperm,   tiles,
+                  ntiles, p.ny, reinterpret_cast<__bf16*>(img), p.Npad, p.Kpad, {}, p.Kpad / BK};
+  for (int s = 0; s < MAX_SEGS; ++s) {
+    ga.seg[s] = seg_dev{nullptr, nullptr, nullptr, 0, 0, 0, 0, 0, 0};
+    ga.koff[s] = p.koff[s];
+  }
+  const gnx_gemm_seg& in = q.seg[0];
+  ga.seg[0] = seg_dev{in.a, nullptr, in.b, in.lda, in.ldb, q.stride[0], in.k, plan_vec_a(in), plan_vec_b(in, q.stride[0])};
+  const daf_args x = {m + (int64_t)t * F, rowptr, ge + (int64_t)t * F, (int)H, h->opt[GNX_OPT_STD_BWD_CENTERED]};
+  gnx_prof_scope prof(h, GNX_K_PNA_AGG_BWD, f.bytes, f.flops, f.mfma, true);
+  GNX_LAUNCH_TIMED(prof, k_pna_dA_agg_bwd, dim3(f.grid_x), dim3(256), f.lds, h->stream, ga, x);
+  GNX_LAUNCH_CHECK();
+  *fused = 1;
+  return GNX_OK;
+}
+
 extern "C" int32_t gnx_gemm_grouped_rows(gnx_handle* h, int32_t nseg, const gnx_gemm_seg* segs, const int64_t* cls_strides,
                                          int32_t num_classes, int64_t M, int32_t N, const float* bias, const float* mask,
                                          int64_t ldmask, float* C, int64_t ldc, int32_t flags, const int32_t* row_index,
diff --git a/gnnepcsaft_amd/csrc/gnx_gemm_plan.hpp b/gnnepcsaft_amd/csrc/gnx_gemm_plan.hpp
--- a/gnnepcsaft_amd/csrc/gnx_gemm_plan.hpp
+++ b/gnnepcsaft_amd/csrc/gnx_gemm_plan.hpp
@@ -330,3 +330,35 @@
   if (nprobs) *nprobs = n;
   return off;
 }
+
+constexpr int PLAN_DAF_BM = 32;
+constexpr size_t PLAN_DAF_LDS = 3 * PLAN_DAF_BM * 272 + PLAN_DAF_BM * 4;
+
+struct pna_dA_agg_plan {
+  bool fused = false;
+  gemm_plan product;
+  unsigned grid_x = 0;
+  size_t lds = 0;
+  double bytes = 0.0, flops = 0.0, mfma = 0.0;
+};
+
+static inline pna_dA_agg_plan pna_dA_agg_plan_of(const pna_product& q, int64_t N, int64_t E, int64_t H, const float* m,
+                                                 const float* ge, int32_t extra_flags, const void* ws, int64_t max_tiles,
+                                                 const int* opt, int num_cus) {
+  pna_dA_agg_plan f;
+  f.product = pna_product_plan(q, N, extra_flags, ws, max_tiles, opt, num_cus);
+  const gemm_plan& p = f.product;
+  const int F = q.seg[0].k;
+  f.fused = opt[GNX_OPT_DA_AGG_FUSED] != 0 && p.kernel == GNX_GEMM_KERNEL_AS3 && p.images && !p.stop_after_split && q.grouped &&
+            max_tiles > 0 && F == PLAN_BN && q.N == 4 * PLAN_BN && p.epi == PLAN_EPI_PLAIN && q.bias == nullptr &&
+            (q.flags & GNX_GEMM_RELU) == 0 && m != nullptr && ge != nullptr && plan_aligned16(m) && plan_aligned16(ge) &&
+            H % 4 == 0 && H >= F && (double)(E + 1) * (double)H < 2147483648.0 && (double)N * (double)q.seg[0].lda < 2147483648.0 &&
+            max_tiles * (PLAN_BM / PLAN_DAF_BM) < 2147483648LL;
+  if (!f.fused) return f;
+  f.grid_x = (unsigned)(max_tiles * (PLAN_BM / PLAN_DAF_BM));
+  f.lds = PLAN_DAF_LDS;
+  f.bytes = 4.0 * N * F + 8.0 * E * F + 4.0 * E + 8.0 * N;
+  f.flops = p.flops;
+  f.mfma = p.mfma;
+  return f;
+}
diff --git a/gnnepcsaft_amd/csrc/gnx_layer.hip b/gnnepcsaft_amd/csrc/gnx_layer.hip
--- a/gnnepcsaft_amd/csrc/gnx_layer.hip
+++ b/gnnepcsaft_amd/csrc/gnx_layer.hip
@@ -147,6 +147,14 @@
     }
     g = a->gbuf[++gi];
   }
+  int ei = 0;
+  float* ge = a->gebuf[ei];
+  const float* m_last = a->hs[a->n_h - 1];
+  bool fused_agg = true;
+  auto dA_product = [&](int t) -> int32_t {
+    return run_with_image(h, pna_dA_product(a->weff[t], T, F, D, t, g, a->dA), N, ct, im ? im->dA[t] : nullptr,
+                          im ? &im->dA_rec[t] : nullptr, a->ws, a->ws_bytes);
+  };
   for (int t = 0; t < T; ++t) {
     const int k = pidx(t, false, 0);
     const float* gt = g + t * F;
@@ -164,13 +172,19 @@
       class_wgrads.push_back(class_wgrad);
     else
       GNX_TRY(class_wgrad());
-    GNX_TRY(run_with_image(h, pna_dA_product(a->weff[t], T, F, D, t, g, a->dA), N, ct, im ? im->dA[t] : nullptr,
-                           im ? &im->dA_rec[t] : nullptr, a->ws, a->ws_bytes));
+    if (fused_agg) {
+      int32_t took = 0;
+      GNX_TRY(gnx_pna_da_aggregate_bwd(h, a->weff[t], T, F, D, t, g, a->dA, m_last, a->rowptr, N, E, ge, a->dperm, a->tiles,
+                                       a->ntiles, a->max_tiles, im ? im->dA[t] : nullptr, im ? &im->dA_rec[t] : nullptr, a->ws,
+                                       a->ws_bytes, &took));
+      fused_agg = took != 0;
+      if (!fused_agg)
+        for (int u = 0; u < t; ++u) GNX_TRY(dA_product(u));
+    }
+    if (!fused_agg) GNX_TRY(dA_product(t));
   }
   const float* g_post0 = g;
-  int ei = 0;
-  float* ge = a->gebuf[ei];
-  GNX_TRY(gnx_pna_aggregate_bwd(h, a->dA, a->hs[a->n_h - 1], a->A, a->rowptr, N, E, T, F, ge));
+  if (!fused_agg) GNX_TRY(gnx_pna_aggregate_bwd(h, a->dA, m_last, a->A, a->rowptr, N, E, T, F, ge));
   for (auto& fn : class_wgrads) GNX_TRY(on_side(h, 0, side, fn));
   bool fused_bwd = pre == 2 && a->etile_info != nullptr && E > 0 && F % 4 == 0 && F <= 128 &&
                    R <= 64 && a16(ge) && a16(a->hs[0]) && a16(a->gebuf[1]) && a16(a->dP) && a16(a->dTe);
diff --git a/gnnepcsaft_amd/csrc/gnx_pna_agg_item.hpp b/gnnepcsaft_amd/csrc/gnx_pna_agg_item.hpp
--- /dev/null
+++ b/gnnepcsaft_amd/csrc/gnx_pna_agg_item.hpp
@@ -0,0 +1,189 @@
+#pragma once
+#include "gnx_common.hpp"
+
+#include <cmath>
+
+template <int VEC>
+__device__ __forceinline__ void vload(float (&r)[VEC], const float* p) {
+  if constexpr (VEC == 4) {
+    f32x4 v = *reinterpret_cast<const f32x4*>(p);
+    r[0] = v.x;
+    r[1] = v.y;
+    r[2] = v.z;
+    r[3] = v.w;
+  } else {
+    r[0] = p[0];
+  }
+}
+template <int VEC>
+__device__ __forceinline__ void vstore(float* p, const float (&r)[VEC]) {
+  if constexpr (VEC == 4) {
+    f32x4 v = {r[0], r[1], r[2], r[3]};
+    *reinterpret_cast<f32x4*>(p) = v;
+  } else {
+    p[0] = r[0];
+  }
+}
+
+#define STD_VAR_MIN 1e-5f
+#define STD_MASK_AT 0.0031622776601683794f
+
+template <int VEC>
+__device__ __forceinline__ void pna_agg_bwd_item_loaded(const float (&gmean)[VEC], const float (&gmn)[VEC],
+                                                        const float (&gmx)[VEC], const float (&gsd)[VEC], int deg,
+                                                        const float (&a)[4][VEC], float* __restrict__ dp, int H, int centered) {
+  float s[VEC], s2[VEC], mn[VEC], mx[VEC];
+#pragma unroll
+  for (int v = 0; v < VEC; ++v) {
+    s[v] = 0.f;
+    s2[v] = 0.f;
+    mn[v] = INFINITY;
+    mx[v] = -INFINITY;
+  }
+#pragma unroll
+  for (int e = 0; e < 4; ++e)
+    if (e < deg) {
+#pragma unroll
+      for (int v = 0; v < VEC; ++v) {
+        s[v] = __fadd_rn(s[v], a[e][v]);
+        s2[v] = __fadd_rn(s2[v], __fmul_rn(a[e][v], a[e][v]));
+        mn[v] = fminf(mn[v], a[e][v]);
+        mx[v] = fmaxf(mx[v], a[e][v]);
+      }
+    }
+  const float cnt = (float)deg;
+  float mean[VEC], sd[VEC], nmn[VEC], nmx[VEC], c2[VEC];
+#pragma unroll
+  for (int v = 0; v < VEC; ++v) {
+    c2[v] = 0.f;
+    mean[v] = __fdiv_rn(s[v], cnt);
+    float mean2 = __fdiv_rn(s2[v], cnt);
+    float var = __fsub_rn(mean2, __fmul_rn(mean[v], mean[v]));
+    float o = __fsqrt_rn(fmaxf(var, STD_VAR_MIN));
+    sd[v] = (o <= STD_MASK_AT) ? 0.f : o;
+    nmn[v] = (mn[v] == 0.f) ? 1.f : 0.f;
+    nmx[v] = (mx[v] == 0.f) ? 1.f : 0.f;
+  }
+#pragma unroll
+  for (int e = 0; e < 4; ++e)
+    if (e < deg) {
+#pragma unroll
+      for (int v = 0; v < VEC; ++v) {
+        nmn[v] += (a[e][v] == mn[v]) ? 1.f : 0.f;
+        nmx[v] += (a[e][v] == mx[v]) ? 1.f : 0.f;
+        const float dv = a[e][v] - mean[v];
+        c2[v] = fmaf(dv, dv, c2[v]);
+      }
+    }
+  float k_mean[VEC], k_mn[VEC], k_mx[VEC], k_sd[VEC];
+#pragma unroll
+  for (int v = 0; v < VEC; ++v) {
+    k_mean[v] = gmean[v] / cnt;
+    k_mn[v] = gmn[v] / nmn[v];
+    k_mx[v] = gmx[v] / nmx[v];
+    const float sdiv = (centered && c2[v] > 0.f) ? sqrtf(c2[v] / cnt) : sd[v];
+    k_sd[v] = (sd[v] > 0.f) ? gsd[v] / (cnt * sdiv) : 0.f;
+  }
+#pragma unroll
+  for (int e = 0; e < 4; ++e)
+    if (e < deg) {
+      float o[VEC];
+#pragma unroll
+      for (int v = 0; v < VEC; ++v) {
+        float r = k_mean[v] + k_sd[v] * (a[e][v] - mean[v]);
+        r += (a[e][v] == mn[v]) ? k_mn[v] : 0.f;
+        r += (a[e][v] == mx[v]) ? k_mx[v] : 0.f;
+        o[v] = r;
+      }
+      vstore<VEC>(dp + (int64_t)e * H, o);
+    }
+}
+
+template <int VEC>
+__device__ __forceinline__ void pna_agg_bwd_item_loop(const float (&gmean)[VEC], const float (&gmn)[VEC], const float (&gmx)[VEC],
+                                                      const float (&gsd)[VEC], int p0, int p1, const float* __restrict__ mc,
+                                                      float* __restrict__ dmc, int H, int centered) {
+  float s[VEC], s2[VEC], mn[VEC], mx[VEC];
+#pragma unroll
+  for (int v = 0; v < VEC; ++v) {
+    s[v] = 0.f;
+    s2[v] = 0.f;
+    mn[v] = INFINITY;
+    mx[v] = -INFINITY;
+  }
+  const float* mp = mc + (int64_t)p0 * H;
+  for (int p = p0; p < p1; ++p, mp += H) {
+    float a[VEC];
+    vload<VEC>(a, mp);
+#pragma unroll
+    for (int v = 0; v < VEC; ++v) {
+      s[v] = __fadd_rn(s[v], a[v]);
+      s2[v] = __fadd_rn(s2[v], __fmul_rn(a[v], a[v]));
+      mn[v] = fminf(mn[v], a[v]);
+      mx[v] = fmaxf(mx[v], a[v]);
+    }
+  }
+  const float cnt = (float)(p1 - p0);
+  float mean[VEC], sd[VEC], nmn[VEC], nmx[VEC], c2[VEC];
+#pragma unroll
+  for (int v = 0; v < VEC; ++v) {
+    c2[v] = 0.f;
+    mean[v] = __fdiv_rn(s[v], cnt);
+    float mean2 = __fdiv_rn(s2[v], cnt);
+    float var = __fsub_rn(mean2, __fmul_rn(mean[v], mean[v]));
+    float o = __fsqrt_rn(fmaxf(var, STD_VAR_MIN));
+    sd[v] = (o <= STD_MASK_AT) ? 0.f : o;
+    nmn[v] = (mn[v] == 0.f) ? 1.f : 0.f;
+    nmx[v] = (mx[v] == 0.f) ? 1.f : 0.f;
+  }
+  mp = mc + (int64_t)p0 * H;
+  for (int p = p0; p < p1; ++p, mp += H) {
+    float a[VEC];
+    vload<VEC>(a, mp);
+#pragma unroll
+    for (int v = 0; v < VEC; ++v) {
+      nmn[v] += (a[v] == mn[v]) ? 1.f : 0.f;
+      nmx[v] += (a[v] == mx[v]) ? 1.f : 0.f;
+      const float dv = a[v] - mean[v];
+      c2[v] = fmaf(dv, dv, c2[v]);
+    }
+  }
+  float k_mean[VEC], k_mn[VEC], k_mx[VEC], k_sd[VEC];
+#pragma unroll
+  for (int v = 0; v < VEC; ++v) {
+    k_mean[v] = gmean[v] / cnt;
+    k_mn[v] = gmn[v] / nmn[v];
+    k_mx[v] = gmx[v] / nmx[v];
+    const float sdiv = (centered && c2[v] > 0.f) ? sqrtf(c2[v] / cnt) : sd[v];
+    k_sd[v] = (sd[v] > 0.f) ? gsd[v] / (cnt * sdiv) : 0.f;
+  }
+  mp = mc + (int64_t)p0 * H;
+  float* dp = dmc + (int64_t)p0 * H;
+  for (int p = p0; p < p1; ++p, mp += H, dp += H) {
+    float a[VEC], o[VEC];
+    vload<VEC>(a, mp);
+#pragma unroll
+    for (int v = 0; v < VEC; ++v) {
+      float r = k_mean[v] + k_sd[v] * (a[v] - mean[v]);
+      r += (a[v] == mn[v]) ? k_mn[v] : 0.f;
+      r += (a[v] == mx[v]) ? k_mx[v] : 0.f;
+      o[v] = r;
+    }
+    vstore<VEC>(dp, o);
+  }
+}
+
+template <int VEC>
+__device__ __forceinline__ void pna_agg_bwd_item(const float (&gmean)[VEC], const float (&gmn)[VEC], const float (&gmx)[VEC],
+                                                 const float (&gsd)[VEC], int p0, int p1, const float* __restrict__ mc,
+                                                 float* __restrict__ dmc, int H, int centered) {
+  const int deg = p1 - p0;
+  if (deg <= 4) {
+    float a[4][VEC];
+#pragma unroll
+    for (int e = 0; e < 4; ++e) vload<VEC>(a[e], mc + (int64_t)(p0 + (e < deg ? e : 0)) * H);
+    pna_agg_bwd_item_loaded<VEC>(gmean, gmn, gmx, gsd, deg, a, dmc + (int64_t)p0 * H, H, centered);
+    return;
+  }
+  pna_agg_bwd_item_loop<VEC>(gmean, gmn, gmx, gsd, p0, p1, mc, dmc, H, centered);
+}
diff --git a/gnnepcsaft_amd/ops.py b/gnnepcsaft_amd/ops.py
--- a/gnnepcsaft_amd/ops.py
+++ b/gnnepcsaft_amd/ops.py
@@ -859,6 +859,38 @@
     return dm
 
 
+def pna_dA_aggregate_bwd(gout: torch.Tensor, weffs: Sequence[torch.Tensor], m: torch.Tensor, A: torch.Tensor, g: GraphPack,
+                         dc: DegreeClasses, T: int, F: int, *, dA: Optional[torch.Tensor] = None,
+                         dm: Optional[torch.Tensor] = None, forward_tiles: bool = False) -> Tuple[torch.Tensor, bool]:
+    N = gout.size(0)
+    if dA is None:
+        dA = torch.empty(N, T * 4 * F, dtype=torch.float32, device=m.device)
+    if dm is None:
+        dm = torch.empty_like(m)
+    lib, h = _lib.load(), handle(m.device)
+    nbytes = lib.gnx_pna_conv_bwd_workspace_bytes(T, F, dc.D)
+    ws = torch.empty(max(nbytes, 1), dtype=torch.uint8, device=m.device)
+    if forward_tiles:
+        table = (dc.dperm.data_ptr(), dc.tiles_p.data_ptr(), dc.ntiles_p.data_ptr(), dc.max_tiles_p)
+    else:
+        table = (dc.dperm.data_ptr(), dc.tiles.data_ptr(), dc.ntiles.data_ptr(), dc.max_tiles)
+    took = C.c_int32(0)
+    for t in range(T):
+        check(lib.gnx_pna_da_aggregate_bwd(h, weffs[t].data_ptr(), T, F, dc.D, t, gout.data_ptr(), dA.data_ptr(), m.data_ptr(),
+                                           g.rowptr.data_ptr(), N, g.E, dm.data_ptr(), *table, None, None, ws.data_ptr(), nbytes,
+                                           C.byref(took)))
+        if not took.value:
+            break
+    else:
+        return dm, True
+    for t in range(T):
+        gemm_grouped([(gout[:, t * F:(t + 1) * F], None, weffs[t][0], 4 * F * F)], dA[:, t * 4 * F:(t + 1) * 4 * F], dc,
+                     b_trans=False, forward_tiles=forward_tiles)
+    check(lib.gnx_pna_aggregate_bwd(h, dA.data_ptr(), m.data_ptr(), A.data_ptr(), g.rowptr.data_ptr(), N, g.E, T, F,
+                                    dm.data_ptr()))
+    return dm, False
+
+
 def gine_aggregate_fwd(x: torch.Tensor, Le: torch.Tensor, g: GraphPack, eps: float) -> torch.Tensor:
     out = torch.empty_like(x)
     check(_lib.load().gnx_gine_aggregate_fwd(handle(x.device), x.data_ptr(), Le.data_ptr(), g.rowptr.data_ptr(),
diff --git a/include/gnx.h b/include/gnx.h
--- a/include/gnx.h
+++ b/include/gnx.h
@@ -37,7 +37,8 @@
   GNX_OPT_GEMM_WS_FAST = 7,
   GNX_OPT_GEMM_TILE_ROWS = 8,
   GNX_OPT_GEMM_MID = 9,
-  GNX_OPT_COUNT = 10
+  GNX_OPT_DA_AGG_FUSED = 10,
+  GNX_OPT_COUNT = 11
 };
 int32_t gnx_set_option(gnx_handle* h, int32_t opt, int32_t value);
 int32_t gnx_get_option(gnx_handle* h, int32_t opt, int32_t* value);
@@ -499,6 +500,11 @@
 int32_t gnx_pna_conv_fwd_images(gnx_handle* h, const gnx_pna_fwd_args* args, const gnx_pna_layer_images* images);
 int32_t gnx_pna_conv_bwd_images(gnx_handle* h, const gnx_pna_bwd_args* args, const gnx_pna_layer_images* images);
 
+int32_t gnx_pna_da_aggregate_bwd(gnx_handle* h, const float* weff_t, int32_t T, int32_t F, int32_t D, int32_t t, const float* g,
+                                 const float* dA, const float* m, const int32_t* rowptr, int64_t N, int64_t E, float* ge,
+                                 const int32_t* dperm, const int32_t* tiles, const int32_t* ntiles, int64_t max_tiles,
+                                 void* image, const gnx_gemm_image* rec, void* ws, size_t ws_bytes, int32_t* fused);
+
 int32_t gnx_fill(gnx_handle* h, float* p, int64_t n, float v);
 int32_t gnx_scale(gnx_handle* h, float* p, int64_t n, float v);
 int32_t gnx_axpy(gnx_handle* h, float* y, const float* x, int64_t n, float a);
```

New measurement: 687,000 graphs/s (median of 6 runs). 1.01x the previous value.
